# openxrlab/xrnerf

Measured on AMD Instinct MI355X. Metric: training rays/s, Instant-NGP Lego (configs/instant_ngp/nerf_blender_local01.py), synthetic 800x800 rays, higher is better.
Workload: dtype f32

## Files before the change

include/xrnerf_mi355.h:

```cpp
#ifndef XRNERF_MI355_H
#define XRNERF_MI355_H

#include <stddef.h>
#include <stdint.h>

#ifdef __cplusplus
extern "C" {
#endif

#define XR_OK 0
#define XR_EINVAL (-22)
#define XR_ENOMEM (-12)
#define XR_EHIP (-5)

#define XR_NERF_STEPS 1024u
#define XR_NERF_CASCADES 8u
#define XR_NERF_GRIDSIZE 128u
#define XR_GRID_CELLS (128u * 128u * 128u)

enum { XR_ACT_NONE = 0, XR_ACT_RELU = 1, XR_ACT_LOGISTIC = 2, XR_ACT_EXPONENTIAL = 3 };

const char* xr_last_error(void);
int xr_version(void);

void xr_pcg32_host_state(uint64_t seed, uint64_t ncalls, uint64_t* state_host, uint64_t* inc_host);

size_t xr_rays_sampler_workspace_bytes(uint32_t n_rays, uint32_t n_series );
int xr_rays_sampler(const float* rays_o, const float* rays_d, const uint8_t* bitfield, uint32_t n_rays,
                    float aabb0, float aabb1, float near_distance, float cone_angle, uint32_t max_samples,
                    uint64_t rng_state, uint64_t rng_inc, float* coords_out, int32_t* rays_index,
                    int32_t* rays_numsteps, uint32_t* counter2, float* xyz_planes, uint32_t plane_stride,
                    uint32_t rng_chunk, uint32_t rng_ray0, uint32_t flags, void* workspace, size_t workspace_bytes, void* stream);
#define XR_K1_WIDE 1u
int xr_rays_sampler_series(const float* rays_o, const float* rays_d, uint32_t ray_stride, const uint8_t* bitfield, uint32_t n_rays,
                           uint32_t n_series, float aabb0, float aabb1, float near_distance, float cone_angle, uint32_t max_samples,
                           uint64_t rng_state, uint64_t rng_inc, float* coords_out, size_t coords_stride, int32_t* rays_index,
                           int32_t* rays_numsteps, uint32_t* counter2, float* xyz_planes, uint32_t plane_stride, void* workspace,
                           size_t workspace_bytes, void* stream);

int xr_compacted_coord(const float* coords_in, const int32_t* numsteps_in, uint32_t n_rays,
                       uint32_t max_compacted, float* coords_out, int32_t* numsteps_out,
                       uint32_t* rays_counter, uint32_t* numstep_counter, void* workspace,
                       size_t workspace_bytes, void* stream);

int xr_clip_numsteps(const int32_t* numsteps_in, const uint32_t* counter2, uint32_t n_rays, uint32_t n_series, uint32_t ray_stride,
                     uint32_t max_compacted, int32_t* numsteps_out, uint32_t* n_valid_dev, void* stream);

int xr_calc_rgb_forward(const float* network_output , const float* coords ,
                        const int32_t* rays_numsteps, const int32_t* rays_numsteps_compacted,
                        const float* bg_color , uint32_t n_rays, int rgb_activation,
                        int density_activation, float* rgb_output , void* stream);
int xr_calc_rgb_backward(const float* network_output, const int32_t* rays_numsteps_compacted,
                         const float* coords, const float* grad_rgb ,
                         const float* rgb_output ,
                         const float* density_grid_mean , uint32_t n_rays,
                         int rgb_activation, int density_activation, float* dloss_doutput ,
                         void* stream);

int xr_composite_train(const float* network_output, const float* coords, const int32_t* rays_numsteps,
                       const int32_t* rays_numsteps_compacted, const float* bg_color, const float* target,
                       const float* alpha_mask, const float* density_grid_mean, uint32_t n_rays, int rgb_activation,
                       int density_activation, float delta, float scale, float* rgb_output, float* loss_mse_out,
                       float* dloss_doutput, uint32_t* live_seg_count, void* stream);
int xr_train_loss_scalars(const float* rgb, const float* target, const float* alpha_mask, uint32_t n_rays, float delta,
                          float scale, float* loss_mse_out, void* stream);
int xr_calc_rgb_inference(const float* network_output, const float* coords, const int32_t* rays_numsteps,
                          float bg_r, float bg_g, float bg_b, uint32_t n_rays, int rgb_activation,
                          int density_activation, float* rgb_output, float* alpha_output, void* stream);

int xr_render_slice_select(const int32_t* rays_numsteps, const float* T, uint32_t n_rays, uint32_t s0, uint32_t s1,
                           float eps, uint32_t* rows_out, int32_t* ray_offset_out, uint32_t* count_out, void* stream);
int xr_render_slice_composite(const float* raw_slice , const float* coords, const int32_t* rays_numsteps,
                              const int32_t* ray_offset, uint32_t n_rays, uint32_t s0, uint32_t s1, int rgb_activation,
                              int density_activation, float* T, float* rgb_acc, void* stream);

int xr_generate_grid_samples(const float* density_grid, uint32_t ema_step, uint32_t n_elements, uint32_t n_cascades ,
                             float thresh, float aabb0, float aabb1, uint64_t rng_state, uint64_t rng_inc,
                             float* positions, uint32_t pos_row_stride, uint32_t pos_comp_stride, int32_t* indices , void* stream);
int xr_mark_untrained_density_grid(const float* focal_lengths , const float* xforms ,
                                   uint32_t n_elements, uint32_t n_images, int resolution0, int resolution1,
                                   float* density_grid, void* stream);
int xr_splat_grid_samples(const float* mlp_out, const int32_t* indices, uint32_t padded_output_width,
                          uint32_t n_samples, float* density_grid_tmp, void* stream);
int xr_ema_grid_samples(const float* density_grid_tmp, uint32_t n_elements, float decay, float* density_grid,
                        void* stream);
size_t xr_update_bitfield_workspace_bytes(void);
int xr_update_bitfield(const float* density_grid, float* density_grid_mean, uint8_t* bitfield, void* workspace,
                       size_t workspace_bytes, void* stream);
int xr_ema_update_bitfield(const float* density_grid_tmp, uint32_t n_elements, float decay, float* density_grid,
                           float* density_grid_mean, uint8_t* bitfield, void* workspace, size_t workspace_bytes, void* stream);
int xr_bitfield_from_mean(const float* density_grid, const float* density_grid_mean, uint8_t* bitfield,
                          void* stream);

void xr_hashgrid_meta(int n_levels, int log2_hashmap_size, int base_resolution, double per_level_scale,
                      float* scale_host, uint32_t* resolution_host, uint32_t* offset_host );
int xr_hashgrid_fwd(const float* table, const float* x, uint32_t x_stride, uint32_t x_comp_stride, uint32_t n, const uint32_t* n_dev,
                    const uint32_t* rows, int n_levels, const float* scale_host, const uint32_t* resolution_host,
                    const uint32_t* offset_host, float* enc_t, uint32_t ld, void* stream);
size_t xr_hashgrid_bwd_workspace_bytes(uint32_t n, int n_levels, const uint32_t* resolution_host,
                                       const uint32_t* offset_host);
#define XR_SCATTER_OVERWRITE 1
int xr_hashgrid_bwd(const float* x, uint32_t x_stride, const float* denc_t, uint32_t ld, uint32_t n,
                    const uint32_t* n_dev, const uint32_t* rows, int n_levels, const float* scale_host, const uint32_t* resolution_host,
                    const uint32_t* offset_host, float* grad_table, void* workspace, size_t workspace_bytes, int flags,
                    void* stream);
int xr_set_helper_stream(void* stream, void* fork_event, void* join_event);
int xr_sh4(const float* dirs, uint32_t dir_stride, uint32_t n, float* out, void* stream);

#define XR_MLP_F32 0
#define XR_MLP_F16 1
#define XR_MLP_BF16X3 2
#define XR_MLP_F16X2 3
int xr_set_mlp_range_word(uint32_t* word);
int xr_nerf_mlp_fwd(int arithmetic, const float* enc_t, uint32_t ld, const float* dirs, uint32_t dir_stride, uint32_t n,
                    const uint32_t* n_dev, const uint32_t* rows , const float* w_density, const float* w_color, int n_hidden_density, int n_hidden_color,
                    float pad_value, float* raw , void* stream);
size_t xr_nerf_mlp_bwd_workspace_bytes(uint32_t n, int n_hidden_density, int n_hidden_color);
int xr_nerf_mlp_bwd(int arithmetic, const float* enc_t, uint32_t ld, const float* dirs, uint32_t dir_stride, uint32_t n,
                    const uint32_t* n_dev, const float* w_density, const float* w_color, int n_hidden_density, int n_hidden_color,
                    float pad_value, const float* draw , float* denc_t, float* grad_w_density,
                    float* grad_w_color, void* workspace, size_t workspace_bytes, const uint32_t* live_rows,
                    const uint32_t* n_live, void* stream);
#define XR_LIVE_SEGMENT_ROWS 1024u
#define XR_LIVE_ROWS_SEGMENTS(n) (((n) + XR_LIVE_SEGMENT_ROWS - 1u) / XR_LIVE_SEGMENT_ROWS)
int xr_nerf_mlp_bwd_list_slots(void* workspace, size_t workspace_bytes, uint32_t n, uint32_t** live_rows, uint32_t** seg_count,
                               uint32_t** n_live);
int xr_live_rows(const float* dloss_doutput, uint32_t n, const uint32_t* n_dev, uint32_t* seg_count, uint32_t* live_rows,
                 uint32_t* n_live, float* zero_denc_t, uint32_t ld, int seg_counts_ready, void* stream);

typedef struct xr_adam_fuse {
    float* param; float* m; float* v; float* ema;
    int step;
    float lr, beta1, beta2, eps, weight_decay, ema_momentum, grad_scale;
    uint64_t n;
} xr_adam_fuse;
int xr_hashgrid_bwd_adam(const float* x, uint32_t x_stride, const float* denc_t, uint32_t ld, uint32_t n, const uint32_t* n_dev,
                         const uint32_t* rows, int n_levels, const float* scale_host, const uint32_t* resolution_host,
                         const uint32_t* offset_host, void* workspace, size_t workspace_bytes, const xr_adam_fuse* adam,
                         void* stream);

int xr_nerf_density_splat(int mlp_mode, const float* enc_t, uint32_t ld, uint32_t n, const float* w_density, int n_hidden_density,
                          int n_hidden_color, const int32_t* indices, float* density_grid_tmp, void* stream);

int xr_ngp_train_step(const float* table, const float* w_density, const float* w_color, int n_hidden_density, int n_hidden_color,
                      float pad_value, int mlp_mode, int n_levels, const float* scale_host, const uint32_t* resolution_host,
                      const uint32_t* offset_host, const float* coords, uint32_t n_rows, const uint32_t* n_dev,
                      const int32_t* rays_numsteps, const int32_t* rays_numsteps_compacted, uint32_t n_rays, const float* bg_color,
                      const float* target, const float* alpha_mask, const float* density_grid_mean, int rgb_activation,
                      int density_activation, float huber_delta, float loss_scale, float* enc_t, uint32_t ld, float* raw,
                      float* draw, float* denc_t, float* rgb_out, float* zero_block, size_t zero_floats, float* grad_w_density,
                      float* grad_w_color, float* loss_mse, uint32_t* live_seg_count, float* grad_table, size_t table_floats, int zero_draw,
                      void* ws_mlp_bwd, size_t ws_mlp_bwd_bytes, void* ws_scatter, size_t ws_scatter_bytes, int scatter_level0,
                      const float* xyz_planes, uint32_t plane_stride, const xr_adam_fuse* table_adam, const xr_adam_fuse* w_density_adam,
                      const xr_adam_fuse* w_color_adam, const char* timed_entry, void* timing_begin, void* timing_end, void* stream);
void* xr_timing_event_create(void);
int xr_event_record(void* event, void* stream);
int xr_timing_event_destroy(void* event);
int xr_timing_event_elapsed_ms(void* begin, void* end, float* ms);

#define XR_NGP_WINDOW 16
typedef struct xr_ngp_window {
    float *rays_o, *rays_d, *target, *alpha, *bg; int32_t* img_ids;
    int32_t *rays_index, *rays_numsteps, *numsteps_clipped;
    uint32_t ray_stride;
    float* coords; size_t coords_stride;
    float* xyz_planes; uint32_t plane_stride;
    uint32_t *counter2, *n_valid;
} xr_ngp_window;
int xr_ngp_window_march(const xr_ngp_window* window, uint32_t first_chunk, uint32_t n_chunks, uint32_t batches_ready, uint32_t n_rays,
                        const float* rays_rgb_rows, uint64_t n_table_rays, uint64_t* cur_ray, uint64_t batch_seed, uint64_t batch_call_index,
                        const uint8_t* bitfield, float aabb0, float aabb1, float near_distance, float cone_angle, uint32_t max_samples,
                        uint64_t k1_call_index, uint32_t max_compacted, void* workspace, size_t workspace_bytes,
                        uint32_t* counter_host_pinned, void* stream);
int xr_make_batch_series(const float* rays_rgb_rows, const uint64_t* row0_host, uint32_t n, uint32_t n_series, uint32_t ray_stride,
                         uint64_t rng_state, uint64_t rng_inc, float* rays_o, float* rays_d, float* target, float* alpha, float* bg,
                         int32_t* img_ids, void* stream);

typedef struct xr_ngp_step_set {
    float *enc_t, *raw, *draw, *denc_t, *rgb_out, *zero_block; size_t zero_floats;
    float *grad_w_density, *grad_w_color, *loss_mse; uint32_t* live_seg_count;
    float* grad_table;
} xr_ngp_step_set;
typedef struct xr_grad_exchange {
    int (*all_reduce)(void* ctx, float* buf, size_t n, void* stream);
    int (*reduce_scatter)(void* ctx, const float* send, float* recv, size_t n_recv, void* stream);
    int (*all_gather)(void* ctx, const float* send, float* recv, size_t n_send, void* stream);
    int (*finish)(void* ctx, void* stream);
    void* ctx; int world_size, rank;
} xr_grad_exchange;
typedef struct xr_ngp_loop_desc {
    float *table, *w_density, *w_color; int n_hidden_density, n_hidden_color; float pad_value; int mlp_mode;
    int n_levels; const float* scale_host; const uint32_t *resolution_host, *offset_host;
    xr_adam_fuse adam_table, adam_w_density, adam_w_color;
    const float* density_grid_mean; int rgb_activation, density_activation; float huber_delta, loss_scale;
    uint32_t n_rows, ld;
    xr_ngp_window window; xr_ngp_step_set step[2];
    void* ws_mlp_bwd; size_t ws_mlp_bwd_bytes; void* ws_scatter; size_t ws_scatter_bytes;
    void* stream;
    const xr_grad_exchange* exchange; int dp_mode; int split_level;
    float *shard_grad, *table_padded; uint64_t shard_floats;
} xr_ngp_loop_desc;
typedef struct xr_ngp_loop_state {
    uint64_t iter;
    uint32_t step_turn;
    int32_t adam_step;
    uint32_t last_step_set;
} xr_ngp_loop_state;
int xr_ngp_loop_run(const xr_ngp_loop_desc* desc, xr_ngp_loop_state* state, uint32_t k, uint32_t n_rays, const float* lr,
                    const float* ema_momentum, const char* timed_entry, void* const* timing_events, void* const* iter_events);
int xr_rccl_unique_id(const char* librccl_path, void* id128);
void* xr_rccl_create(const char* librccl_path, const void* id128, int world_size, int rank);
int xr_rccl_destroy(void* handle);
int xr_rccl_exchange(void* handle, xr_grad_exchange* out);
int xr_rccl_exposed_ms(void* handle, int timing_on, float* mean_ms , float* max_ms, int* count);

int xr_mlp_fwd(const float* x, long row_stride, long col_stride, int n_in, float pad_value, uint32_t n, const float* w,
               int n_hidden, float* y, void* stream);
size_t xr_mlp_bwd_workspace_bytes(int n_hidden);
int xr_mlp_bwd(const float* x, long row_stride, long col_stride, int n_in, float pad_value, uint32_t n, const float* w,
               int n_hidden, const float* dy, float* dx, float* grad_w, void* workspace, size_t workspace_bytes,
               void* stream);

int xr_gen_rays(const float* pose43_host, int H, int W, float fx, float fy, float cx, float cy, int row0,
                int nrows, float* rays_o, float* rays_d, void* stream);
int xr_huber_loss_grad(const float* rgb, const float* target, const float* alpha, uint32_t n_elems, float delta, float scale,
                       float* grad, float* loss_out, void* stream);
int xr_scale_multi(int n_tensors, float* const* tensors, const size_t* n, const float* scale_dev, float host_factor,
                   void* stream);
int xr_adam_step_multi(int n_tensors, float* const* p_host, const float* const* g_host, float* const* m_host,
                       float* const* v_host, float* const* ema_host, const size_t* n_host, int step, float lr,
                       float beta1, float beta2, float eps, float weight_decay, float ema_momentum, float grad_scale,
                       void* stream);

int xr_mip_zvals(const float* near, const float* far, uint32_t n_rays, uint32_t n_z, int lindisp,
                 const float* z_rand, float* z_out, void* stream);
uint32_t xr_mip_encode_channels(int min_deg, int max_deg, int min_deg_view, int max_deg_view, int append_identity);
int xr_mip_encode(const float* rays_o, const float* rays_d, const float* viewdirs, const float* radii ,
                  const float* z_vals , uint32_t n_rays, uint32_t n_z, int min_deg, int max_deg,
                  int min_deg_view, int max_deg_view, int append_identity, int ray_shape, float* out, uint32_t ld,
                  void* stream);
int xr_mip_encode_gaussians(const float* means, const float* covs, const float* viewdirs, uint32_t n_rays,
                            uint32_t n_samples, int min_deg, int max_deg, int min_deg_view, int max_deg_view,
                            int append_identity, float* out, uint32_t ld, void* stream);
int xr_mip_render_forward(const float* raw, const float* z_vals, const float* rays_d, uint32_t n_rays, uint32_t n_z,
                          float density_bias, float rgb_padding, int white_bkgd, int density_activation, float* rgb,
                          float* distance, float* acc, float* weights, void* stream);
int xr_mip_render_backward(const float* raw, const float* z_vals, const float* rays_d, const float* grad_rgb,
                           uint32_t n_rays, uint32_t n_z, float density_bias, float rgb_padding, int white_bkgd,
                           int density_activation, float* grad_raw, void* stream);
int xr_mip_resample(const float* z_vals, const float* weights , const float* rand,
                    float resample_padding, uint32_t n_rays, uint32_t n_z, float* z_out, void* stream);

uint32_t xr_kilo_param_floats(int pos_freqs, int dir_freqs, int n_hidden);
size_t xr_kilo_workspace_bytes(uint64_t n_samples_total, uint32_t num_networks);
int xr_kilo_mlp_forward(const float* pts, const float* rays_o, const float* rays_d, const float* z_vals,
                        const float* viewdirs, uint32_t n_rays, uint32_t n_samples, const float* gmin_host,
                        const float* gmax_host, const int32_t* fixed_res_host, const int32_t* occ_res_host,
                        const uint8_t* occupancy, const float* domain_mins, const float* domain_maxs, const float* params,
                        uint32_t param_stride, uint32_t num_networks, int pos_freqs, int dir_freqs, int n_hidden,
                        float* raw, uint32_t* counts_out, void* workspace, size_t workspace_bytes, void* stream);
int xr_kilo_mlp_backward(const float* pts, const float* rays_o, const float* rays_d, const float* z_vals,
                         const float* viewdirs, uint32_t n_rays, uint32_t n_samples, const float* gmin_host,
                         const float* gmax_host, const int32_t* fixed_res_host, const int32_t* occ_res_host,
                         const uint8_t* occupancy, const float* domain_mins, const float* domain_maxs, const float* params,
                         uint32_t param_stride, uint32_t num_networks, int pos_freqs, int dir_freqs, int n_hidden,
                         const float* draw, float* grad_params, int reuse_assignment, void* workspace, size_t workspace_bytes, void* stream);
int xr_kilo_pack_params(const float* const* tensors_host, uint32_t num_networks, int pos_freqs, int dir_freqs, int n_hidden, float* blocks,
                        uint32_t param_stride, void* stream);
int xr_kilo_unpack_grads(float* blocks, uint32_t param_stride, uint32_t num_networks, int pos_freqs, int dir_freqs, int n_hidden,
                         float* const* grads_host, int clear_blocks, void* stream);
size_t xr_kilo_render_workspace_bytes(uint32_t n_rays, uint32_t n_samples, uint32_t num_networks);
int xr_kilo_render_rays(const float* rays_o, const float* rays_d, const float* viewdirs, const float* near,
                        const float* far, uint32_t n_rays, uint32_t n_samples, int lindisp, const float* gmin_host,
                        const float* gmax_host, const int32_t* fixed_res_host, const int32_t* occ_res_host,
                        const uint8_t* occupancy, const float* domain_mins, const float* domain_maxs, const float* params,
                        uint32_t param_stride, uint32_t num_networks, int pos_freqs, int dir_freqs, int n_hidden,
                        int white_bkgd, float* rgb, float* disp, float* acc, void* workspace, size_t workspace_bytes,
                        void* stream);
int xr_nerf_render_forward(const float* raw, const float* z_vals, const float* rays_d, uint32_t n_rays,
                           uint32_t n_samples, int white_bkgd, float* rgb, float* disp, float* acc, float* weights,
                           void* stream);

int xr_linear_forward(const float* x, uint32_t ldx, const float* w, const float* bias, uint32_t M, uint32_t N, uint32_t K, int relu,
                      float* y, uint32_t ldy, void* stream);
int xr_linear_backward_input(const float* dy, uint32_t lddy, const float* mask_src, const float* w, int w_transposed, uint32_t M, uint32_t N,
                             uint32_t K, float* dx, void* stream);
int xr_linear_arithmetic(int mode);
uint32_t xr_linear_backward_splits(uint32_t M, uint32_t N, uint32_t K);
int xr_linear_backward_weight(const float* dy, uint32_t lddy, const float* mask_src, const float* x, uint32_t ldx, uint32_t M, uint32_t N,
                              uint32_t K, uint32_t splits, float* dw_partials, float* db_partials, size_t part_stride, void* stream);
int xr_linear_backward_bias(const float* dy, const float* mask_src, uint32_t M, uint32_t N, uint32_t splits,
                            float* db_partials, void* stream);
int xr_sum_partials(const float* partials, uint32_t n_partials, size_t stride, uint32_t n, float* out, void* stream);

int xr_kilo_student_step(const float* examples, uint32_t ex_stride, const float* teacher_raw, const float* domain_mins,
                         const float* domain_maxs, float* params, uint32_t param_stride, uint32_t num_networks, uint32_t batch,
                         int pos_freqs, int dir_freqs, int n_hidden, float alpha_distance, float* loss, float* grad,
                         float* adam_m, float* adam_v, int adam_step, float lr, float beta1, float beta2, float eps, void* stream);
int xr_kilo_student_forward(const float* examples, uint32_t ex_stride, uint32_t n_examples, const float* domain_mins,
                            const float* domain_maxs, const float* params, uint32_t param_stride, uint32_t num_networks,
                            int pos_freqs, int dir_freqs, int n_hidden, int render, float alpha_distance, float* out, void* stream);
int xr_kilo_distill_examples(uint64_t seed, uint64_t iteration, uint64_t pool_size, const float* domain_mins, const float* domain_maxs,
                             uint32_t num_networks, uint32_t batch, uint32_t ex_stride, float* examples, void* stream);
int xr_kilo_occupancy_points(const float* gmin_host, const float* gmax_host, const int32_t* res_host, const int32_t* sub_host,
                             uint64_t voxel_begin, uint32_t n_voxels, float* points, void* stream);
int xr_kilo_occupancy_reduce(const float* raw, uint32_t raw_stride, uint32_t samples_per_voxel, float threshold, uint32_t n_voxels,
                             uint8_t* occupancy, void* stream);

#ifdef __cplusplus
}
#endif
#include "xrnerf_mi355_bungee.h"
#endif
```

xrnerf_amd/_lib.py:

```python
import ctypes as C
import os

HERE = os.path.dirname(os.path.abspath(__file__))
LIB_PATH = os.environ.get('XRNERF_LIB') or os.path.join(HERE, 'libxrnerf_mi355.so')

_vp, _u32, _i32, _f, _u64, _sz, _d = C.c_void_p, C.c_uint32, C.c_int, C.c_float, C.c_uint64, C.c_size_t, C.c_double

class AdamFuse(C.Structure):
    _fields_ = [('param', C.c_void_p), ('m', C.c_void_p), ('v', C.c_void_p), ('ema', C.c_void_p), ('step', C.c_int),
                ('lr', C.c_float), ('beta1', C.c_float), ('beta2', C.c_float), ('eps', C.c_float), ('weight_decay', C.c_float),
                ('ema_momentum', C.c_float), ('grad_scale', C.c_float), ('n', C.c_uint64)]


class Window(C.Structure):
    _fields_ = [(k, C.c_void_p) for k in ('rays_o', 'rays_d', 'target', 'alpha', 'bg', 'img_ids', 'rays_index', 'rays_numsteps',
                                          'numsteps_clipped')] + \
               [('ray_stride', C.c_uint32), ('coords', C.c_void_p), ('coords_stride', C.c_size_t), ('xyz_planes', C.c_void_p),
                ('plane_stride', C.c_uint32), ('counter2', C.c_void_p), ('n_valid', C.c_void_p)]


class StepSet(C.Structure):
    _fields_ = [(k, C.c_void_p) for k in ('enc_t', 'raw', 'draw', 'denc_t', 'rgb_out', 'zero_block')] + [('zero_floats', C.c_size_t)] + \
               [(k, C.c_void_p) for k in ('grad_w_density', 'grad_w_color', 'loss_mse', 'live_seg_count', 'grad_table')]


WINDOW = 16
LIVE_SEGMENT_ROWS = 1024

EX_ALL_REDUCE = C.CFUNCTYPE(C.c_int, C.c_void_p, C.c_void_p, C.c_size_t, C.c_void_p)
EX_SCATTER_GATHER = C.CFUNCTYPE(C.c_int, C.c_void_p, C.c_void_p, C.c_void_p, C.c_size_t, C.c_void_p)
EX_FINISH = C.CFUNCTYPE(C.c_int, C.c_void_p, C.c_void_p)


class GradExchange(C.Structure):
    _fields_ = [('all_reduce', EX_ALL_REDUCE), ('reduce_scatter', EX_SCATTER_GATHER), ('all_gather', EX_SCATTER_GATHER),
                ('finish', EX_FINISH), ('ctx', C.c_void_p), ('world_size', C.c_int), ('rank', C.c_int)]


class LoopDesc(C.Structure):
    _fields_ = [('table', C.c_void_p), ('w_density', C.c_void_p), ('w_color', C.c_void_p), ('n_hidden_density', C.c_int),
                ('n_hidden_color', C.c_int), ('pad_value', C.c_float), ('mlp_mode', C.c_int), ('n_levels', C.c_int),
                ('scale_host', C.c_void_p), ('resolution_host', C.c_void_p), ('offset_host', C.c_void_p),
                ('adam_table', AdamFuse), ('adam_w_density', AdamFuse), ('adam_w_color', AdamFuse),
                ('density_grid_mean', C.c_void_p), ('rgb_activation', C.c_int), ('density_activation', C.c_int),
                ('huber_delta', C.c_float), ('loss_scale', C.c_float), ('n_rows', C.c_uint32), ('ld', C.c_uint32),
                ('window', Window), ('step', StepSet * 2),
                ('ws_mlp_bwd', C.c_void_p), ('ws_mlp_bwd_bytes', C.c_size_t), ('ws_scatter', C.c_void_p), ('ws_scatter_bytes', C.c_size_t),
                ('stream', C.c_void_p),
                ('exchange', C.POINTER(GradExchange)), ('dp_mode', C.c_int), ('split_level', C.c_int),
                ('shard_grad', C.c_void_p), ('table_padded', C.c_void_p), ('shard_floats', C.c_uint64)]


class LoopState(C.Structure):
    _fields_ = [('iter', C.c_uint64), ('step_turn', C.c_uint32), ('adam_step', C.c_int32), ('last_step_set', C.c_uint32)]


SIGNATURES = {
    'xr_last_error': (C.c_char_p, []),
    'xr_version': (_i32, []),
    'xr_event_record': (_i32, [_vp, _vp]),
    'xr_timing_event_create': (_vp, []),
    'xr_timing_event_destroy': (_i32, [_vp]),
    'xr_timing_event_elapsed_ms': (_i32, [_vp, _vp, _vp]),
    'xr_pcg32_host_state': (None, [_u64, _u64, _vp, _vp]),
    'xr_rays_sampler': (_i32, [_vp, _vp, _vp, _u32, _f, _f, _f, _f, _u32, _u64, _u64, _vp, _vp, _vp, _vp, _vp, _u32, _u32, _u32, _u32, _vp, _sz, _vp]),
    'xr_compacted_coord': (_i32, [_vp, _vp, _u32, _u32, _vp, _vp, _vp, _vp, _vp, _sz, _vp]),
    'xr_rays_sampler_workspace_bytes': (_sz, [_u32, _u32]),
    'xr_rays_sampler_series': (_i32, [_vp, _vp, _u32, _vp, _u32, _u32, _f, _f, _f, _f, _u32, _u64, _u64, _vp, _sz, _vp, _vp, _vp, _vp, _u32, _vp,
                                      _sz, _vp]),
    'xr_clip_numsteps': (_i32, [_vp, _vp, _u32, _u32, _u32, _u32, _vp, _vp, _vp]),
    'xr_make_batch_series': (_i32, [_vp, _vp, _u32, _u32, _u32, _u64, _u64, _vp, _vp, _vp, _vp, _vp, _vp, _vp]),
    'xr_ngp_window_march': (_i32, [_vp, _u32, _u32, _u32, _u32, _vp, _u64, _vp, _u64, _u64, _vp, _f, _f, _f, _f, _u32, _u64, _u32, _vp, _sz,
                                   _vp, _vp]),
    'xr_render_slice_select': (_i32, [_vp, _vp, _u32, _u32, _u32, _f, _vp, _vp, _vp, _vp]),
    'xr_render_slice_composite': (_i32, [_vp, _vp, _vp, _vp, _u32, _u32, _u32, _i32, _i32, _vp, _vp, _vp]),
    'xr_calc_rgb_forward': (_i32, [_vp, _vp, _vp, _vp, _vp, _u32, _i32, _i32, _vp, _vp]),
    'xr_calc_rgb_backward': (_i32, [_vp, _vp, _vp, _vp, _vp, _vp, _u32, _i32, _i32, _vp, _vp]),
    'xr_hashgrid_bwd_adam': (_i32, [_vp, _u32, _vp, _u32, _u32, _vp, _vp, _i32, _vp, _vp, _vp, _vp, _sz, _vp, _vp]),
    'xr_train_loss_scalars': (_i32, [_vp, _vp, _vp, _u32, _f, _f, _vp, _vp]),
    'xr_composite_train': (_i32, [_vp, _vp, _vp, _vp, _vp, _vp, _vp, _vp, _u32, _i32, _i32, _f, _f, _vp, _vp, _vp, _vp, _vp]),
    'xr_calc_rgb_inference': (_i32, [_vp, _vp, _vp, _f, _f, _f, _u32, _i32, _i32, _vp, _vp, _vp]),
    'xr_generate_grid_samples': (_i32, [_vp, _u32, _u32, _u32, _f, _f, _f, _u64, _u64, _vp, _u32, _u32, _vp, _vp]),
    'xr_mark_untrained_density_grid': (_i32, [_vp, _vp, _u32, _u32, _i32, _i32, _vp, _vp]),
    'xr_splat_grid_samples': (_i32, [_vp, _vp, _u32, _u32, _vp, _vp]),
    'xr_ema_grid_samples': (_i32, [_vp, _u32, _f, _vp, _vp]),
    'xr_update_bitfield_workspace_bytes': (_sz, []),
    'xr_update_bitfield': (_i32, [_vp, _vp, _vp, _vp, _sz, _vp]),
    'xr_ema_update_bitfield': (_i32, [_vp, _u32, _f, _vp, _vp, _vp, _vp, _sz, _vp]),
    'xr_bitfield_from_mean': (_i32, [_vp, _vp, _vp, _vp]),
    'xr_hashgrid_meta': (None, [_i32, _i32, _i32, _d, _vp, _vp, _vp]),
    'xr_hashgrid_fwd': (_i32, [_vp, _vp, _u32, _u32, _u32, _vp, _vp, _i32, _vp, _vp, _vp, _vp, _u32, _vp]),
    'xr_hashgrid_bwd_workspace_bytes': (_sz, [_u32, _i32, _vp, _vp]),
    'xr_hashgrid_bwd': (_i32, [_vp, _u32, _vp, _u32, _u32, _vp, _vp, _i32, _vp, _vp, _vp, _vp, _vp, _sz, _i32, _vp]),
    'xr_set_helper_stream': (_i32, [_vp, _vp, _vp]),
    'xr_set_mlp_range_word': (_i32, [_vp]),
    'xr_sh4': (_i32, [_vp, _u32, _u32, _vp, _vp]),
    'xr_nerf_mlp_fwd': (_i32, [_i32, _vp, _u32, _vp, _u32, _u32, _vp, _vp, _vp, _vp, _i32, _i32, _f, _vp, _vp]),
    'xr_nerf_mlp_bwd_workspace_bytes': (_sz, [_u32, _i32, _i32]),
    'xr_ngp_train_step': (_i32, [_vp, _vp, _vp, _i32, _i32, _f, _i32, _i32, _vp, _vp, _vp, _vp, _u32, _vp, _vp, _vp, _u32, _vp, _vp, _vp,
                                 _vp, _i32, _i32, _f, _f, _vp, _u32, _vp, _vp, _vp, _vp, _vp, _sz, _vp, _vp, _vp, _vp, _vp, _sz, _i32, _vp, _sz,
                                 _vp, _sz, _i32, _vp, _u32, _vp, _vp, _vp, C.c_char_p, _vp, _vp, _vp]),
    'xr_ngp_loop_run': (_i32, [_vp, _vp, _u32, _u32, _vp, _vp, C.c_char_p, _vp, _vp]),
    'xr_rccl_unique_id': (_i32, [C.c_char_p, _vp]),
    'xr_rccl_create': (_vp, [C.c_char_p, _vp, _i32, _i32]),
    'xr_rccl_destroy': (_i32, [_vp]),
    'xr_rccl_exchange': (_i32, [_vp, _vp]),
    'xr_rccl_exposed_ms': (_i32, [_vp, _i32, _vp, _vp, _vp]),
    'xr_nerf_mlp_bwd': (_i32, [_i32, _vp, _u32, _vp, _u32, _u32, _vp, _vp, _vp, _i32, _i32, _f, _vp, _vp, _vp, _vp, _vp, _sz, _vp, _vp, _vp]),
    'xr_live_rows': (_i32, [_vp, _u32, _vp, _vp, _vp, _vp, _vp, _u32, _i32, _vp]),
    'xr_nerf_mlp_bwd_list_slots': (_i32, [_vp, _sz, _u32, _vp, _vp, _vp]),
    'xr_mlp_fwd': (_i32, [_vp, C.c_long, C.c_long, _i32, _f, _u32, _vp, _i32, _vp, _vp]),
    'xr_mlp_bwd_workspace_bytes': (_sz, [_i32]),
    'xr_mlp_bwd': (_i32, [_vp, C.c_long, C.c_long, _i32, _f, _u32, _vp, _i32, _vp, _vp, _vp, _vp, _sz, _vp]),
    'xr_gen_rays': (_i32, [_vp, _i32, _i32, _f, _f, _f, _f, _i32, _i32, _vp, _vp, _vp]),
    'xr_huber_loss_grad': (_i32, [_vp, _vp, _vp, _u32, _f, _f, _vp, _vp, _vp]),
    'xr_adam_step_multi': (_i32, [_i32, _vp, _vp, _vp, _vp, _vp, _vp, _i32, _f, _f, _f, _f, _f, _f, _f, _vp]),
    'xr_scale_multi': (_i32, [_i32, _vp, _vp, _vp, _f, _vp]),
    'xr_mip_zvals': (_i32, [_vp, _vp, _u32, _u32, _i32, _vp, _vp, _vp]),
    'xr_mip_encode_channels': (_u32, [_i32, _i32, _i32, _i32, _i32]),
    'xr_mip_encode': (_i32, [_vp, _vp, _vp, _vp, _vp, _u32, _u32, _i32, _i32, _i32, _i32, _i32, _i32, _vp, _u32, _vp]),
    'xr_mip_encode_gaussians': (_i32, [_vp, _vp, _vp, _u32, _u32, _i32, _i32, _i32, _i32, _i32, _vp, _u32, _vp]),
    'xr_mip_render_forward': (_i32, [_vp, _vp, _vp, _u32, _u32, _f, _f, _i32, _i32, _vp, _vp, _vp, _vp, _vp]),
    'xr_mip_render_backward': (_i32, [_vp, _vp, _vp, _vp, _u32, _u32, _f, _f, _i32, _i32, _vp, _vp]),
    'xr_mip_resample': (_i32, [_vp, _vp, _vp, _f, _u32, _u32, _vp, _vp]),
    'xr_kilo_param_floats': (_u32, [_i32, _i32, _i32]),
    'xr_kilo_workspace_bytes': (_sz, [_u64, _u32]),
    'xr_kilo_mlp_forward': (_i32, [_vp, _vp, _vp, _vp, _vp, _u32, _u32, _vp, _vp, _vp, _vp, _vp, _vp, _vp, _vp, _u32, _u32,
                                   _i32, _i32, _i32, _vp, _vp, _vp, _sz, _vp]),
    'xr_kilo_mlp_backward': (_i32, [_vp, _vp, _vp, _vp, _vp, _u32, _u32, _vp, _vp, _vp, _vp, _vp, _vp, _vp, _vp, _u32, _u32,
                                    _i32, _i32, _i32, _vp, _vp, _i32, _vp, _sz, _vp]),
    'xr_kilo_pack_params': (_i32, [_vp, _u32, _i32, _i32, _i32, _vp, _u32, _vp]),
    'xr_kilo_unpack_grads': (_i32, [_vp, _u32, _u32, _i32, _i32, _i32, _vp, _i32, _vp]),
    'xr_nerf_render_forward': (_i32, [_vp, _vp, _vp, _u32, _u32, _i32, _vp, _vp, _vp, _vp, _vp]),
    'xr_nerf_density_splat': (_i32, [_i32, _vp, _u32, _u32, _vp, _i32, _i32, _vp, _vp, _vp]),
    'xr_linear_forward': (_i32, [_vp, _u32, _vp, _vp, _u32, _u32, _u32, _i32, _vp, _u32, _vp]),
    'xr_linear_backward_input': (_i32, [_vp, _u32, _vp, _vp, _i32, _u32, _u32, _u32, _vp, _vp]),
    'xr_linear_backward_splits': (_u32, [_u32, _u32, _u32]),
    'xr_linear_arithmetic': (_i32, [_i32]),
    'xr_linear_backward_bias': (_i32, [_vp, _vp, _u32, _u32, _u32, _vp, _vp]),
    'xr_sum_partials': (_i32, [_vp, _u32, _sz, _u32, _vp, _vp]),
    'xr_linear_backward_weight': (_i32, [_vp, _u32, _vp, _vp, _u32, _u32, _u32, _u32, _u32, _vp, _vp, _sz, _vp]),
    'xr_kilo_render_workspace_bytes': (_sz, [_u32, _u32, _u32]),
    'xr_kilo_render_rays': (_i32, [_vp, _vp, _vp, _vp, _vp, _u32, _u32, _i32, _vp, _vp, _vp, _vp, _vp, _vp, _vp, _vp, _u32,
                                   _u32, _i32, _i32, _i32, _i32, _vp, _vp, _vp, _vp, _sz, _vp]),
    'xr_kilo_student_step': (_i32, [_vp, _u32, _vp, _vp, _vp, _vp, _u32, _u32, _u32, _i32, _i32, _i32, _f, _vp, _vp, _vp, _vp, _i32, _f, _f,
                                    _f, _f, _vp]),
    'xr_kilo_student_forward': (_i32, [_vp, _u32, _u32, _vp, _vp, _vp, _u32, _u32, _i32, _i32, _i32, _i32, _f, _vp, _vp]),
    'xr_kilo_distill_examples': (_i32, [_u64, _u64, _u64, _vp, _vp, _u32, _u32, _u32, _vp, _vp]),
    'xr_kilo_occupancy_points': (_i32, [_vp, _vp, _vp, _vp, _u64, _u32, _vp, _vp]),
    'xr_kilo_occupancy_reduce': (_i32, [_vp, _u32, _u32, _f, _u32, _vp, _vp]),
}

BUNGEE_SIGNATURES = {
    'xr_bungee_zvals': (_i32, [_vp, _vp, _vp, _vp, _u32, _u32, _i32, _vp, _f, _f, _f, _vp, _vp]),
    'xr_bungee_encode': (_i32, [_vp, _vp, _vp, _vp, _vp, _vp, _vp, _u32, _u32, _i32, _i32, _i32, _vp, _u32, _vp, _u32, _vp]),
    'xr_bungee_render_forward': (_i32, [_vp, _vp, _vp, _vp, _u32, _u32, _u32, _i32, _f, _f, _i32, _i32, _vp, _vp, _vp, _vp, _vp]),
    'xr_bungee_render_backward': (_i32, [_vp, _vp, _vp, _vp, _vp, _u32, _u32, _u32, _i32, _f, _f, _i32, _i32, _vp, _vp]),
}

VANILLA_SIGNATURES = {
    'xr_nerf_encode': (_i32, [_vp, _vp, _u64, _u32, _i32, _i32, _vp, _u32, _vp]),
    'xr_nerf_render_train_forward': (_i32, [_vp, _vp, _vp, _vp, _u32, _u32, _i32, _vp, _vp, _vp, _vp, _vp]),
    'xr_nerf_render_backward': (_i32, [_vp, _vp, _vp, _vp, _u32, _u32, _i32, _vp, _vp, _vp]),
    'xr_nerf_sample_pdf': (_i32, [_vp, _vp, _vp, _vp, _vp, _u32, _u32, _u32, _vp, _vp, _vp, _vp]),
}

ANINERF_SIGNATURES = {
    'xr_ani_closest': (_i32, [_vp, _vp, _vp, _vp, _u32, _u32, _f, _vp, _vp, _vp, _vp, _vp, _vp]),
    'xr_ani_select_workspace_bytes': (_sz, [_u32]),
    'xr_ani_select': (_i32, [_vp, _vp, _u32, _vp, _vp, _vp, _sz, _vp]),
    'xr_ani_blend_forward': (_i32, [_vp, _vp, _vp, _u32, _vp, _vp]),
    'xr_ani_blend_backward': (_i32, [_vp, _vp, _u32, _vp, _vp]),
    'xr_ani_skin_forward': (_i32, [_vp, _vp, _vp, _vp, _vp, _u32, _vp, _vp, _vp]),
    'xr_ani_skin_backward': (_i32, [_vp, _vp, _vp, _vp, _vp, _u32, _vp, _vp, _vp, _vp]),
    'xr_ani_encode_backward': (_i32, [_vp, _vp, _u32, _u32, _i32, _vp, _vp]),
}

NEURALBODY_SIGNATURES = {
    'xr_nb_layout': (_i32, [_u32, _i32, _i32, _i32, _vp]),
    'xr_nb_build_rows_workspace_bytes': (_sz, [_i32, _i32, _i32]),
    'xr_nb_build_rows': (_i32, [_vp, _u32, _i32, _i32, _i32, _vp, _vp, _vp, _vp, _vp, _sz, _vp]),
    'xr_nb_subm_table': (_i32, [_vp, _vp, _u32, _i32, _i32, _i32, _vp, _vp]),
    'xr_nb_down_tables': (_i32, [_vp, _vp, _u32, _vp, _vp, _u32, _i32, _i32, _i32, _vp, _vp, _vp]),
    'xr_nb_conv': (_i32, [_vp, _vp, _vp, _u32, _i32, _i32, _i32, _i32, _vp, _vp]),
    'xr_nb_conv_weight_grad_workspace_bytes': (_sz, [_u32, _i32, _i32]),
    'xr_nb_conv_weight_grad': (_i32, [_vp, _vp, _vp, _u32, _i32, _i32, _vp, _vp, _sz, _vp]),
    'xr_nb_sample_forward': (_i32, [_vp, _vp, _vp, _vp, _f, _i32, _i32, _i32, _vp, _vp, _u32, _vp, _u32, _vp]),
    'xr_nb_sample_backward_workspace_bytes': (_sz, [_vp]),
    'xr_nb_sample_backward': (_i32, [_vp, _vp, _vp, _vp, _f, _i32, _i32, _i32, _vp, _vp, _vp, _u32, _u32, _vp, _vp, _sz, _vp]),
}

_lib = None


class XrError(RuntimeError):
    pass


def load():
    global _lib
    if _lib is not None:
        return _lib
    from . import build as _build

    def is_stale():
        if not os.environ.get('XRNERF_LIB') and os.path.exists(LIB_PATH) and os.path.isdir(_build.CSRC):
            i = _build.info()
            return i.get('stamp') == 'missing' or not i.get('binary_is_the_stamped_build') or i.get('sources_match_the_stamped_build') is False
        return False

    stale = is_stale()
    if not os.path.exists(LIB_PATH) or stale:
        import fcntl
        import warnings

        def rebuild():
            try:
                _build.build(force=stale)
            except Exception as e:
                if not os.path.exists(LIB_PATH):
                    raise XrError('libxrnerf_mi355.so is missing and could not be built: %s. '
                                  'Run `python -m xrnerf_amd.build` (needs hipcc).' % e)
                warnings.warn('libxrnerf_mi355.so is not the stamped build of the sources beside it and could not be rebuilt (%s): '
                              'loading it as it is' % e)
        try:
            lock = open(LIB_PATH + '.lock', 'w')
        except OSError:
            lock = None
        if lock is None:
            rebuild()
        else:
            with lock:
                fcntl.flock(lock, fcntl.LOCK_EX)
                try:
                    stale = is_stale()
                    if not os.path.exists(LIB_PATH) or stale:
                        rebuild()
                finally:
                    fcntl.flock(lock, fcntl.LOCK_UN)
    lib = C.CDLL(LIB_PATH)
    for name, (res, args) in list(SIGNATURES.items()) + list(BUNGEE_SIGNATURES.items()) + list(VANILLA_SIGNATURES.items()) + \
            list(ANINERF_SIGNATURES.items()) + list(NEURALBODY_SIGNATURES.items()):
        fn = getattr(lib, name)
        fn.restype = res
        fn.argtypes = args
    _lib = lib
    return lib


def check(rc, what=''):
    if rc != 0:
        raise XrError('%s failed (%d): %s' % (what, rc, load().xr_last_error().decode()))
```

xrnerf_amd/csrc/xr_common.h:

```cpp
#pragma once
#include <hip/hip_runtime.h>
#include <cstdint>
#include <cstdio>
#include <cstring>
#include "../../include/xrnerf_mi355.h"
#ifndef XR_LDS_PTR
#define XR_LDS_PTR(T, p) ((T __attribute__((address_space(3)))*)(p))
#endif
extern "C" __attribute__((visibility("hidden"))) int xr_device_cus(void);

#define XR_WAVE 64

void xr_set_error(const char* fmt, ...);

#define XR_REQUIRE(cond, msg)                                   \
    do {                                                        \
        if (!(cond)) { xr_set_error("%s: %s", __func__, msg); return XR_EINVAL; } \
    } while (0)

#define XR_LAUNCH_CHECK()                                                            \
    do {                                                                             \
        hipError_t e_ = hipGetLastError();                                           \
        if (e_ != hipSuccess) { xr_set_error("%s: %s", __func__, hipGetErrorString(e_)); return XR_EHIP; } \
    } while (0)

#define XR_HIP(call)                                                                 \
    do {                                                                             \
        hipError_t e_ = (call);                                                      \
        if (e_ != hipSuccess) { xr_set_error("%s: %s", __func__, hipGetErrorString(e_)); return XR_EHIP; } \
    } while (0)

static inline uint32_t xr_div_up(uint64_t a, uint32_t b) { return (uint32_t)((a + b - 1) / b); }

#define XR_SQRT3 1.73205080757f
__host__ __device__ inline float xr_min_step() { return XR_SQRT3 / 1024.0f; }
__host__ __device__ inline float xr_max_step() { return XR_SQRT3 / 1024.0f * 128.0f * 1024.0f / 128.0f; }
__host__ __device__ inline float xr_max_warp_step() { return XR_SQRT3 / 1024.0f * 128.0f; }

struct xr_pcg32 {
    uint64_t state, inc;
    __host__ __device__ uint32_t next_uint() {
        uint64_t old = state;
        state = old * 0x5851f42d4c957f2dULL + inc;
        uint32_t xs = (uint32_t)(((old >> 18u) ^ old) >> 27u);
        uint32_t rot = (uint32_t)(old >> 59u);
        return (xs >> rot) | (xs << ((~rot + 1u) & 31));
    }
    __host__ __device__ float next_float() {
        uint32_t u = (next_uint() >> 9) | 0x3f800000u;
        float f;
#if defined(__HIP_DEVICE_COMPILE__)
        f = __uint_as_float(u);
#else
        memcpy(&f, &u, 4);
#endif
        return f - 1.0f;
    }
    __host__ __device__ void advance(uint64_t delta) {
        uint64_t cur_mult = 0x5851f42d4c957f2dULL, cur_plus = inc, acc_mult = 1u, acc_plus = 0u;
        while (delta > 0) {
            if (delta & 1) { acc_mult *= cur_mult; acc_plus = acc_plus * cur_mult + cur_plus; }
            cur_plus = (cur_mult + 1) * cur_plus;
            cur_mult *= cur_mult;
            delta >>= 1;
        }
        state = acc_mult * state + acc_plus;
    }
    __host__ __device__ void seed(uint64_t initstate, uint64_t initseq) {
        state = 0u; inc = (initseq << 1u) | 1u;
        next_uint(); state += initstate; next_uint();
    }
};

__host__ __device__ inline uint32_t xr_expand_bits(uint32_t v) {
    v = (v * 0x00010001u) & 0xFF0000FFu; v = (v * 0x00000101u) & 0x0F00F00Fu;
    v = (v * 0x00000011u) & 0xC30C30C3u; v = (v * 0x00000005u) & 0x49249249u;
    return v;
}
__host__ __device__ inline uint32_t xr_morton3d(uint32_t x, uint32_t y, uint32_t z) {
    return xr_expand_bits(x) | (xr_expand_bits(y) << 1) | (xr_expand_bits(z) << 2);
}
__host__ __device__ inline uint32_t xr_morton3d_invert(uint32_t x) {
    x = x & 0x49249249; x = (x | (x >> 2)) & 0xc30c30c3; x = (x | (x >> 4)) & 0x0f00f00f;
    x = (x | (x >> 8)) & 0xff0000ff; x = (x | (x >> 16)) & 0x0000ffff;
    return x;
}

__device__ inline float xr_clampf(float v, float lo, float hi) { return v < lo ? lo : (hi < v ? hi : v); }
__device__ inline float xr_logistic(float x) { return 1.0f / (1.0f + __expf(-x)); }
__device__ inline float xr_act_rgb(float v, int a) {
    switch (a) { case 0: return v; case 1: return v > 0.f ? v : 0.f; case 2: return xr_logistic(v);
                 default: return __expf(xr_clampf(v, -10.f, 10.f)); }
}
__device__ inline float xr_act_density(float v, int a) {
    switch (a) { case 0: return v; case 1: return v > 0.f ? v : 0.f; case 2: return xr_logistic(v);
                 default: return __expf(v); }
}
__device__ inline float xr_dact_rgb(float v, int a) {
    switch (a) { case 0: return 1.f; case 1: return v > 0.f ? 1.f : 0.f;
                 case 2: { float s = xr_logistic(v); return s * (1.f - s); }
                 default: return __expf(xr_clampf(v, -10.f, 10.f)); }
}
__device__ inline float xr_dact_density(float v, int a) {
    switch (a) { case 0: return 1.f; case 1: return v > 0.f ? 1.f : 0.f;
                 case 2: { float s = xr_logistic(v); return s * (1.f - s); }
                 default: return __expf(xr_clampf(v, -15.f, 15.f)); }
}
__host__ __device__ inline float xr_unwarp_dt(float dt) {
    return dt * (xr_max_warp_step() - xr_min_step()) + xr_min_step();
}

#define XR_LIVE_SEG 1024u

struct XrHelper { hipStream_t stream; hipEvent_t fork, join; };
const XrHelper* xr_internal_helper();
int xr_internal_hashgrid_bwd_adam_supported(uint32_t n, int n_levels, const float* scale_host, const uint32_t* resolution_host,
                                            const uint32_t* offset_host);
void xr_internal_defer_mlp_reduce(bool on);
int xr_internal_mlp_bwd_reduce(const void* workspace, uint32_t n, int n_hidden_density, int n_hidden_color, float* grad_w_density, float* grad_w_color, int overwrite, void* stream);
```

xrnerf_amd/csrc/xr_misc.hip:

```cpp
#include "xr_common.h"
#include "xr_adam.h"
#include <cstdlib>
#include <cstdarg>

static thread_local char g_err[512] = "";
void xr_set_error(const char* fmt, ...) {
    va_list ap; va_start(ap, fmt);
    vsnprintf(g_err, sizeof(g_err), fmt, ap);
    va_end(ap);
}
extern "C" const char* xr_last_error(void) { return g_err; }
extern "C" int xr_version(void) { return 123; }

extern "C" void xr_pcg32_host_state(uint64_t seed, uint64_t ncalls, uint64_t* state_host, uint64_t* inc_host) {
    xr_pcg32 r; r.seed(seed, 1u);
    r.advance(ncalls << 32);
    *state_host = r.state; *inc_host = r.inc;
}

struct Pose43 { float m[12]; };
__global__ __launch_bounds__(256) void k_gen_rays(Pose43 p, int W, float fx, float fy, float cx, float cy, int row0,
                                                   uint32_t n, float* __restrict__ rays_o, float* __restrict__ rays_d) {
    const uint32_t q = blockIdx.x * 256 + threadIdx.x;
    if (q >= n) return;
    const int r = q / W, c = q % W;
    const float i = (float)c + 0.5f, j = (float)(row0 + r) + 0.5f;
    const float dx = (i - cx) / fx, dy = (j - cy) / fy;
    float v[3];
#pragma unroll
    for (int k = 0; k < 3; ++k) {
        float a = __fmul_rn(p.m[k], dx);
        a = __fadd_rn(a, __fmul_rn(p.m[3 + k], dy));
        v[k] = __fadd_rn(a, p.m[6 + k]);
    }
    const float nrm = __fsqrt_rn(__fadd_rn(__fadd_rn(__fmul_rn(v[0], v[0]), __fmul_rn(v[1], v[1])), __fmul_rn(v[2], v[2])));
#pragma unroll
    for (int k = 0; k < 3; ++k) { rays_d[3 * (size_t)q + k] = v[k] / nrm; rays_o[3 * (size_t)q + k] = p.m[9 + k]; }
}
extern "C" int xr_gen_rays(const float* pose43_host, int H, int W, float fx, float fy, float cx, float cy, int row0,
                           int nrows, float* rays_o, float* rays_d, void* stream_) {
    XR_REQUIRE(pose43_host && rays_o && rays_d, "null pointer");
    XR_REQUIRE(H > 0 && W > 0 && row0 >= 0 && nrows > 0 && row0 + nrows <= H, "bad image window");
    Pose43 p; memcpy(p.m, pose43_host, sizeof(p.m));
    const uint32_t n = (uint32_t)nrows * (uint32_t)W;
    hipLaunchKernelGGL(k_gen_rays, dim3(xr_div_up(n, 256)), dim3(256), 0, (hipStream_t)stream_, p, W, fx, fy, cx, cy, row0, n,
                       rays_o, rays_d);
    XR_LAUNCH_CHECK();
    return XR_OK;
}

__global__ __launch_bounds__(256) void k_huber(const float* __restrict__ rgb, const float* __restrict__ target,
                                                const float* __restrict__ alpha, uint32_t n, float delta, float scale,
                                                float* __restrict__ grad, float* __restrict__ loss) {
    __shared__ float ws[4], ws2[4];
    float acc = 0.f, mse = 0.f;
    for (uint32_t i = blockIdx.x * 256 + threadIdx.x; i < n; i += gridDim.x * 256) {
        const float r = rgb[i] - target[i], a = fabsf(r);
        if (a > delta) { acc += a - 0.5f * delta; grad[i] = scale * (r > 0.f ? 1.f : -1.f); }
        else { acc += 0.5f / delta * a * a; grad[i] = scale * (r / delta); }
        if (alpha) { const float m = r * alpha[i / 3]; mse += m * m; }
    }
#pragma unroll
    for (int d = 32; d > 0; d >>= 1) { acc += __shfl_xor(acc, d, 64); mse += __shfl_xor(mse, d, 64); }
    if ((threadIdx.x & 63) == 0) { ws[threadIdx.x >> 6] = acc; ws2[threadIdx.x >> 6] = mse; }
    __syncthreads();
    if (threadIdx.x == 0) {
        atomicAdd(loss, scale * ((ws[0] + ws[1]) + (ws[2] + ws[3])));
        if (alpha) atomicAdd(loss + 1, (ws2[0] + ws2[1]) + (ws2[2] + ws2[3]));
    }
}
extern "C" int xr_huber_loss_grad(const float* rgb, const float* target, const float* alpha, uint32_t n_elems, float delta, float scale,
                                  float* grad, float* loss_out, void* stream_) {
    XR_REQUIRE(rgb && target && grad && loss_out && n_elems > 0, "bad argument");
    XR_REQUIRE(!alpha || n_elems % 3 == 0, "the masked error takes rgb triples");
    hipLaunchKernelGGL(k_huber, dim3(min(xr_div_up(n_elems, 256), 1024u)), dim3(256), 0, (hipStream_t)stream_, rgb, target, alpha, n_elems,
                       delta, scale, grad, loss_out);
    XR_LAUNCH_CHECK();
    return XR_OK;
}

struct XrBatchRows { uint64_t row0[XR_NGP_WINDOW]; };
__global__ __launch_bounds__(256) void k_make_batch(const float* __restrict__ rows, uint32_t n, xr_pcg32 rng,
                                                     float* __restrict__ rays_o, float* __restrict__ rays_d,
                                                     float* __restrict__ target, float* __restrict__ alpha,
                                                     float* __restrict__ bg, int32_t* __restrict__ img_ids, XrBatchRows at, uint32_t ray_stride) {
    const uint32_t i = blockIdx.x * 256 + threadIdx.x;
    if (i >= n) return;
    const float* r = rows + 11 * ((size_t)at.row0[blockIdx.y] + i);
    rng.advance(((uint64_t)blockIdx.y << 32) + 3ull * i);
    const size_t q = (size_t)blockIdx.y * ray_stride + i;
    const float a = r[9];
#pragma unroll
    for (int k = 0; k < 3; ++k) {
        rays_o[3 * q + k] = r[k];
        rays_d[3 * q + k] = r[3 + k];
        const float b = rng.next_float();
        bg[3 * q + k] = b;
        target[3 * q + k] = r[6 + k] * a + b * (1.f - a);
    }
    alpha[q] = a;
    img_ids[q] = (int32_t)r[10];
}
extern "C" int xr_make_batch_series(const float* rays_rgb_rows, const uint64_t* row0_host, uint32_t n, uint32_t n_series, uint32_t ray_stride,
                                    uint64_t rng_state, uint64_t rng_inc, float* rays_o, float* rays_d, float* target, float* alpha, float* bg,
                                    int32_t* img_ids, void* stream_) {
    XR_REQUIRE(rays_rgb_rows && row0_host && rays_o && rays_d && target && alpha && bg && img_ids && n > 0, "bad argument");
    XR_REQUIRE(n_series >= 1 && n_series <= (uint32_t)XR_NGP_WINDOW && ray_stride >= n, "bad series");
    xr_pcg32 rng{rng_state, rng_inc};
    XrBatchRows at = {};
    for (uint32_t c = 0; c < n_series; ++c) at.row0[c] = row0_host[c];
    hipLaunchKernelGGL(k_make_batch, dim3(xr_div_up(n, 256), n_series), dim3(256), 0, (hipStream_t)stream_, rays_rgb_rows, n, rng, rays_o,
                       rays_d, target, alpha, bg, img_ids, at, ray_stride);
    XR_LAUNCH_CHECK();
    return XR_OK;
}

struct AdamTensors { float* p[4]; const float* g[4]; float* m[4]; float* v[4]; float* ema[4]; unsigned long long n[4]; unsigned first_block[5]; };
typedef float am_f4 __attribute__((ext_vector_type(4)));
template <bool NT> __device__ __forceinline__ float4 am_ld(const float* p, size_t i) {
    if (NT) { const am_f4 r = __builtin_nontemporal_load(reinterpret_cast<const am_f4*>(p) + i); return make_float4(r.x, r.y, r.z, r.w); }
    return reinterpret_cast<const float4*>(p)[i];
}
template <bool NT> __device__ __forceinline__ void am_st(float* p, size_t i, const float4 v) {
    if (NT) { am_f4 r; r.x = v.x; r.y = v.y; r.z = v.z; r.w = v.w; __builtin_nontemporal_store(r, reinterpret_cast<am_f4*>(p) + i); }
    else reinterpret_cast<float4*>(p)[i] = v;
}
template <bool NT>
__global__ __launch_bounds__(256) void k_adam_multi(AdamTensors t, int nt, float b1, float b2, float step_size, float bc2s,
                                                     float eps, float wd, float mom, float gs) {
    int k = 0;
#pragma unroll
    for (int j = 1; j < 4; ++j) if (j < nt && blockIdx.x >= t.first_block[j]) k = j;
    const unsigned nblk = t.first_block[k + 1] - t.first_block[k], blk = blockIdx.x - t.first_block[k];
    float* __restrict__ p = t.p[k]; const float* __restrict__ g = t.g[k];
    float* __restrict__ m = t.m[k]; float* __restrict__ v = t.v[k]; float* __restrict__ ema = t.ema[k];
    const size_t n = t.n[k], n4 = n / 4;
    for (size_t i = blk * 256ull + threadIdx.x; i < n4; i += (size_t)nblk * 256) {
        float4 pp = ((float4*)p)[i], mm = am_ld<NT>(m, i), vv = am_ld<NT>(v, i);
        const float4 gg = am_ld<NT>(g, i);
        adam1(pp.x, gg.x, mm.x, vv.x, b1, b2, step_size, bc2s, eps, wd, gs);
        adam1(pp.y, gg.y, mm.y, vv.y, b1, b2, step_size, bc2s, eps, wd, gs);
        adam1(pp.z, gg.z, mm.z, vv.z, b1, b2, step_size, bc2s, eps, wd, gs);
        adam1(pp.w, gg.w, mm.w, vv.w, b1, b2, step_size, bc2s, eps, wd, gs);
        ((float4*)p)[i] = pp; am_st<NT>(m, i, mm); am_st<NT>(v, i, vv);
        if (ema) {
            float4 e = am_ld<NT>(ema, i);
            e.x = (1.f - mom) * e.x + mom * pp.x; e.y = (1.f - mom) * e.y + mom * pp.y;
            e.z = (1.f - mom) * e.z + mom * pp.z; e.w = (1.f - mom) * e.w + mom * pp.w;
            am_st<NT>(ema, i, e);
        }
    }
    if (blk == 0 && threadIdx.x < (n & 3)) {
        const size_t i = n4 * 4 + threadIdx.x;
        float pp = p[i], mm = m[i], vv = v[i];
        adam1(pp, g[i], mm, vv, b1, b2, step_size, bc2s, eps, wd, gs);
        p[i] = pp; m[i] = mm; v[i] = vv;
        if (ema) ema[i] = (1.f - mom) * ema[i] + mom * pp;
    }
}
extern "C" int xr_adam_step_multi(int n_tensors, float* const* p, const float* const* g, float* const* m, float* const* v,
                                  float* const* ema, const size_t* n, int step, float lr, float beta1, float beta2, float eps,
                                  float weight_decay, float ema_momentum, float grad_scale, void* stream_) {
    XR_REQUIRE(n_tensors >= 1 && n_tensors <= 4 && p && g && m && v && n && step >= 1, "bad argument");
    AdamTensors t; memset(&t, 0, sizeof(t));
    unsigned blocks = 0;
    for (int k = 0; k < n_tensors; ++k) {
        XR_REQUIRE(p[k] && g[k] && m[k] && v[k] && n[k] > 0, "null tensor");
        XR_REQUIRE((((uintptr_t)p[k] | (uintptr_t)g[k] | (uintptr_t)m[k] | (uintptr_t)v[k] | (uintptr_t)(ema ? ema[k] : nullptr)) & 15) == 0,
                   "buffers must be 16-byte aligned");
        t.p[k] = p[k]; t.g[k] = g[k]; t.m[k] = m[k]; t.v[k] = v[k]; t.ema[k] = ema ? ema[k] : nullptr; t.n[k] = n[k];
        t.first_block[k] = blocks;
        blocks += min(xr_div_up(n[k] / 4 + 1, 256), 2048u);
    }
    for (int k = n_tensors; k <= 4; ++k) t.first_block[k] = blocks;
    const float bc1 = 1.f - powf(beta1, (float)step), bc2 = 1.f - powf(beta2, (float)step);
#ifndef XR_ADAM_NT
#define XR_ADAM_NT 1
#endif
    hipLaunchKernelGGL(k_adam_multi<XR_ADAM_NT != 0>, dim3(blocks), dim3(256), 0, (hipStream_t)stream_, t, n_tensors, beta1, beta2, lr / bc1,
                       sqrtf(bc2), eps, weight_decay, ema_momentum, grad_scale);
    XR_LAUNCH_CHECK();
    return XR_OK;
}

struct ScaleTensors { float* p[4]; unsigned long long n[4]; };
__global__ __launch_bounds__(256) void k_scale_multi(ScaleTensors t, int nt, const float* __restrict__ scale_dev, float host_factor) {
    const float f = (scale_dev ? *scale_dev : 1.f) * host_factor;
    if (f == 1.f) return;
    for (int k = 0; k < nt; ++k) {
        float* __restrict__ p = t.p[k];
        const size_t n = t.n[k], n4 = n / 4;
        for (size_t i = blockIdx.x * 256ull + threadIdx.x; i < n4; i += (size_t)gridDim.x * 256) {
            float4 v = ((float4*)p)[i];
            v.x *= f; v.y *= f; v.z *= f; v.w *= f;
            ((float4*)p)[i] = v;
        }
        if (blockIdx.x == 0 && threadIdx.x < (n & 3)) p[n4 * 4 + threadIdx.x] *= f;
    }
}
extern "C" int xr_scale_multi(int n_tensors, float* const* p, const size_t* n, const float* scale_dev, float host_factor, void* stream_) {
    XR_REQUIRE(n_tensors >= 1 && n_tensors <= 4 && p && n, "bad argument");
    ScaleTensors t; memset(&t, 0, sizeof(t));
    for (int k = 0; k < n_tensors; ++k) {
        XR_REQUIRE(p[k] && ((uintptr_t)p[k] & 15) == 0, "tensors must be 16-byte aligned");
        t.p[k] = p[k]; t.n[k] = n[k];
    }
    hipLaunchKernelGGL(k_scale_multi, dim3(2048), dim3(256), 0, (hipStream_t)stream_, t, n_tensors, scale_dev, host_factor);
    XR_LAUNCH_CHECK();
    return XR_OK;
}
```

xrnerf_amd/csrc/xr_raymarch.hip:

```cpp
#include "xr_common.h"
#include "xr_aux.h"
#include <cfloat>
#include <cstdlib>

#define RM_BLOCK 256
#ifndef K1W_MAX_RAYS
#define K1W_MAX_RAYS 32768
#endif
#define K1_TL 128

__device__ inline uint32_t block_excl_scan(uint32_t v, uint32_t* total, uint32_t* lds4) {
    const int lane = threadIdx.x & 63, wid = threadIdx.x >> 6;
    uint32_t inc = v;
#pragma unroll
    for (int d = 1; d < 64; d <<= 1) {
        uint32_t o = __shfl_up(inc, d, 64);
        if (lane >= d) inc += o;
    }
    if (lane == 63) lds4[wid] = inc;
    __syncthreads();
    uint32_t woff = 0, tot = 0;
#pragma unroll
    for (int w = 0; w < RM_BLOCK / 64; ++w) {
        uint32_t t = lds4[w];
// ... 162 lines not shown
            }
        }
        if (done) break;
        const float tl = __shfl(t, K1W - 1, K1W);
        t0 = tl + rm_calc_dt(tl, cone);
    }
    if (li == 0) { cnt[ray] = j; start_t[ray] = startt; }
}
__global__ __launch_bounds__(RM_BLOCK) void k1_block_scan(uint32_t n_rays, const uint32_t* __restrict__ cnt, uint32_t* __restrict__ local_off,
                                                          uint32_t* __restrict__ block_tot) {
    __shared__ uint32_t lds4[4];
    const uint32_t i = blockIdx.x * RM_BLOCK + threadIdx.x;
    uint32_t tot;
    const uint32_t off = block_excl_scan(i < n_rays ? cnt[i] : 0u, &tot, lds4);
    if (i < n_rays) local_off[i] = off;
    if (threadIdx.x == 0) block_tot[blockIdx.x] = tot;
}

__global__ __launch_bounds__(1024) void k_scan_blocks(uint32_t nb, const uint32_t* __restrict__ block_tot,
                                                      uint32_t limit, uint32_t* __restrict__ block_base,
                                                      uint32_t* __restrict__ info) {
    __shared__ uint32_t wsum[16];
    __shared__ uint32_t s_running, s_cross;
    const int lane = threadIdx.x & 63, wid = threadIdx.x >> 6;
    if (threadIdx.x == 0) { s_running = 0; s_cross = nb; }
    __syncthreads();
    for (uint32_t c0 = 0; c0 < nb; c0 += 1024) {
        uint32_t b = c0 + threadIdx.x;
        uint32_t v = b < nb ? block_tot[b] : 0, inc = v;
#pragma unroll
        for (int d = 1; d < 64; d <<= 1) { uint32_t o = __shfl_up(inc, d, 64); if (lane >= d) inc += o; }
        if (lane == 63) wsum[wid] = inc;
        __syncthreads();
        uint32_t woff = 0, ctot = 0;
        for (int w = 0; w < 16; ++w) { uint32_t t = wsum[w]; if (w < wid) woff += t; ctot += t; }
        uint32_t base = s_running + woff + inc - v;
        if (b < nb) {
            block_base[b] = base;
            if ((uint64_t)base + v > (uint64_t)limit) atomicMin(&s_cross, b);
        }
        __syncthreads();
        if (threadIdx.x == 0) s_running += ctot;
        __syncthreads();
    }
    if (threadIdx.x == 0) { info[0] = s_running; info[1] = s_cross; }
}

__global__ __launch_bounds__(RM_BLOCK) void k1_write(
    uint32_t n_rays, float lo, float hi, const float* __restrict__ rays_o, const float* __restrict__ rays_d,
    const uint8_t* __restrict__ bitfield, float cone, uint32_t max_samples, const uint32_t* __restrict__ cnt,
    const uint32_t* __restrict__ local_off, const float* __restrict__ start_t,
    const uint32_t* __restrict__ block_base, const uint32_t* __restrict__ info, const uint32_t* __restrict__ block_tot,
    float* __restrict__ coords_out,
    int32_t* __restrict__ rays_index, int32_t* __restrict__ numsteps_out, uint32_t* __restrict__ counter2,
    const float* __restrict__ tlist, float* __restrict__ xyz_planes, uint32_t plane_stride, uint32_t ray_stride, size_t coords_stride) {
    __shared__ uint32_t lds4[4];
    const uint32_t b = blockIdx.x, i = b * RM_BLOCK + threadIdx.x;
    const uint32_t nb = gridDim.x;
    {
        const size_t c = blockIdx.y;
        rays_o += 3 * c * ray_stride; rays_d += 3 * c * ray_stride;
        rays_index += c * ray_stride; numsteps_out += 2 * c * ray_stride; counter2 += 2 * c;
        coords_out += 7 * c * coords_stride;
        if (xyz_planes) xyz_planes += 3 * c * (size_t)plane_stride;
        if (block_tot) block_tot += c * nb;
        cnt += c * nb * RM_BLOCK; local_off += c * nb * RM_BLOCK; start_t += c * nb * RM_BLOCK; tlist += c * nb * RM_BLOCK * (size_t)K1_TL;
    }
    uint32_t cross, bbase, grand;
    if (block_tot) {
        __shared__ uint32_t s_cross, s_bbase;
        if (threadIdx.x == 0) s_cross = nb;
        const uint32_t v = threadIdx.x < nb ? block_tot[threadIdx.x] : 0u;
        const uint32_t ex = block_excl_scan(v, &grand, lds4);
        if (threadIdx.x < nb && (uint64_t)ex + v > (uint64_t)max_samples) atomicMin(&s_cross, threadIdx.x);
        if (threadIdx.x == b) s_bbase = ex;
        __syncthreads();
        cross = s_cross; bbase = s_bbase;
    } else { cross = info[1]; bbase = block_base[b]; grand = info[0]; }
    uint32_t n = 0, base = 0; bool in = i < n_rays;
    if (in) { n = cnt[i]; base = bbase + local_off[i]; }
    bool valid = in && !((uint64_t)base + n > (uint64_t)max_samples);
    uint32_t vtot;
    uint32_t voff = block_excl_scan(valid ? 1u : 0u, &vtot, lds4);
    uint32_t valid_before = (b <= cross) ? b * RM_BLOCK : 0u;
    if (in) {
        if (!valid) {
            numsteps_out[2 * i] = 0; numsteps_out[2 * i + 1] = (int32_t)base; rays_index[i] = 0;
        } else {
            numsteps_out[2 * i] = (int32_t)n; numsteps_out[2 * i + 1] = (int32_t)base;
            rays_index[i] = n == 0 ? -1 : (int32_t)(valid_before + voff);
        }
    }
    if (threadIdx.x == 0) {
        if (b == 0) counter2[1] = grand;
        if (b == cross || (cross == nb && b == nb - 1)) counter2[0] = valid_before + vtot;
    }
    __shared__ uint32_t s_off[RM_BLOCK], s_n[RM_BLOCK];
    __shared__ float s_ray[RM_BLOCK][6];
    s_off[threadIdx.x] = in ? local_off[i] : 0xffffffffu;
    s_n[threadIdx.x] = valid ? n : 0u;
    if (in) {
#pragma unroll
        for (int k = 0; k < 3; ++k) { s_ray[threadIdx.x][k] = rays_o[3 * i + k]; s_ray[threadIdx.x][3 + k] = rays_d[3 * i + k]; }
    }
    __syncthreads();
    const uint32_t last = min((uint32_t)RM_BLOCK, n_rays - b * RM_BLOCK) - 1;
    const uint32_t btot = s_off[last] + cnt[b * RM_BLOCK + last];
    const float diag = hi - lo;
    for (uint32_t e = threadIdx.x; e < btot; e += RM_BLOCK) {
        uint32_t lo_r = 0, hi_r = last;
        while (lo_r < hi_r) {
            const uint32_t mid = (lo_r + hi_r + 1) >> 1;
            if (s_off[mid] <= e) lo_r = mid; else hi_r = mid - 1;
        }
        const uint32_t j = e - s_off[lo_r];
        if (j >= s_n[lo_r] || j >= K1_TL) continue;
        const float t = tlist[((size_t)b * RM_BLOCK + lo_r) * K1_TL + j];
        const float ox = s_ray[lo_r][0], oy = s_ray[lo_r][1], oz = s_ray[lo_r][2];
        const float dx = s_ray[lo_r][3], dy = s_ray[lo_r][4], dz = s_ray[lo_r][5];
        const float px = ox + t * dx, py = oy + t * dy, pz = oz + t * dz;
        const float dt = rm_calc_dt(t, cone);
        float* c = coords_out + 7 * ((size_t)bbase + e);
        c[0] = (px - lo) / diag; c[1] = (py - lo) / diag; c[2] = (pz - lo) / diag;
        c[3] = (dt - xr_min_step()) / (xr_max_warp_step() - xr_min_step());
        c[4] = (dx + 1.0f) * 0.5f; c[5] = (dy + 1.0f) * 0.5f; c[6] = (dz + 1.0f) * 0.5f;
        if (xyz_planes) {
            const size_t q = (size_t)bbase + e;
            xyz_planes[q] = c[0]; xyz_planes[plane_stride + q] = c[1]; xyz_planes[2 * (size_t)plane_stride + q] = c[2];
        }
    }
    if (!valid || n <= K1_TL) return;
    Ray r = rm_load_ray(rays_o, rays_d, i);
    const float wdx = (r.dx + 1.0f) * 0.5f, wdy = (r.dy + 1.0f) * 0.5f, wdz = (r.dz + 1.0f) * 0.5f;
    float t = tlist[(size_t)i * K1_TL + (K1_TL - 1)];
    t += rm_calc_dt(t, cone);
    uint32_t j = K1_TL;
    float* __restrict__ out = coords_out + 7 * (size_t)base;
    for (;;) {
        float px = r.ox + t * r.dx, py = r.oy + t * r.dy, pz = r.oz + t * r.dz;
        if (!(rm_contains(lo, hi, px, py, pz) && j < n)) break;
        float dt = rm_calc_dt(t, cone);
        int mip = rm_mip_from_dt(dt, px, py, pz);
        if (rm_occupied(px, py, pz, bitfield, mip)) {
            float* c = out + 7 * (size_t)j;
            c[0] = (px - lo) / diag; c[1] = (py - lo) / diag; c[2] = (pz - lo) / diag;
            c[3] = (dt - xr_min_step()) / (xr_max_warp_step() - xr_min_step());
            c[4] = wdx; c[5] = wdy; c[6] = wdz;
            if (xyz_planes) {
                const size_t q = (size_t)base + j;
                xyz_planes[q] = c[0]; xyz_planes[plane_stride + q] = c[1]; xyz_planes[2 * (size_t)plane_stride + q] = c[2];
            }
            ++j; t += dt;
        } else t = rm_advance(t, cone, px, py, pz, r, XR_NERF_GRIDSIZE >> mip);
    }
}

struct RmWorkspace { uint32_t *cnt, *local_off, *block_tot, *block_base, *info; float *start_t, *tlist; };
static size_t rm_ws_layout(uint32_t n_rays, char* base, RmWorkspace* w, uint32_t n_series = 1) {
    const size_t nb = (size_t)xr_div_up(n_rays, RM_BLOCK) * n_series;
    const size_t slots = n_series > 1 ? nb * RM_BLOCK : (size_t)n_rays;
    size_t off = 0;
    auto take = [&](size_t bytes) { size_t o = off; off += (bytes + 255) / 256 * 256; return base ? base + o : (char*)nullptr; };
    char* p0 = take(4ull * slots); char* p1 = take(4ull * slots); char* p2 = take(4ull * slots);
    char* p3 = take(4 * nb); char* p4 = take(4 * nb); char* p5 = take(16);
    char* p6 = take(4ull * slots * K1_TL);
    if (w) { w->tlist = (float*)p6; w->cnt = (uint32_t*)p0; w->local_off = (uint32_t*)p1; w->start_t = (float*)p2;
             w->block_tot = (uint32_t*)p3; w->block_base = (uint32_t*)p4; w->info = (uint32_t*)p5; }
    return off;
}

extern "C" size_t xr_rays_sampler_workspace_bytes(uint32_t n_rays, uint32_t n_series) {
    return rm_ws_layout(n_rays, nullptr, nullptr, n_series ? n_series : 1);
}

static int rm_launch(const float* rays_o, const float* rays_d, const uint8_t* bitfield, uint32_t n_rays, uint32_t n_series, uint32_t ray_stride,
                     float aabb0, float aabb1, float near_distance, float cone_angle, uint32_t max_samples, xr_pcg32 rng,
                     float* coords_out, size_t coords_stride, int32_t* rays_index, int32_t* rays_numsteps, uint32_t* counter2, float* xyz_planes,
                     uint32_t plane_stride, uint32_t rng_chunk, uint32_t rng_ray0, uint32_t flags, void* workspace, hipStream_t stream) {
    RmWorkspace w; rm_ws_layout(n_rays, (char*)workspace, &w, n_series);
    const uint32_t nb = xr_div_up(n_rays, RM_BLOCK);
#ifndef K1W_ALWAYS
#define K1W_ALWAYS 0
#endif
    if (n_series == 1 && ((flags & XR_K1_WIDE) != 0u || K1W_ALWAYS != 0) && (uint32_t)K1W_MAX_RAYS != 0u && n_rays <= (uint32_t)K1W_MAX_RAYS) {
        hipLaunchKernelGGL(k1_count_w, dim3(xr_div_up(n_rays * K1W, RM_BLOCK)), dim3(RM_BLOCK), 0, stream, n_rays, aabb0, aabb1, rays_o, rays_d,
                           bitfield, cone_angle, near_distance, rng, rng_chunk, rng_ray0, w.cnt, w.start_t, w.tlist);
        hipLaunchKernelGGL(k1_block_scan, dim3(nb), dim3(RM_BLOCK), 0, stream, n_rays, (const uint32_t*)w.cnt, w.local_off, w.block_tot);
    } else
        hipLaunchKernelGGL(k1_count, dim3(nb, n_series), dim3(RM_BLOCK), 0, stream, n_rays, aabb0, aabb1, rays_o, rays_d, bitfield,
                           cone_angle, near_distance, rng, rng_chunk, rng_ray0, w.cnt, w.local_off, w.start_t, w.block_tot, w.tlist, ray_stride);
#ifndef K1_INLINE_SCAN
#define K1_INLINE_SCAN 1
#endif
    const bool inline_scan = (K1_INLINE_SCAN || n_series > 1) && nb <= (uint32_t)RM_BLOCK;
    if (!inline_scan) hipLaunchKernelGGL(k_scan_blocks, dim3(1), dim3(1024), 0, stream, nb, w.block_tot, max_samples, w.block_base, w.info);
    hipLaunchKernelGGL(k1_write, dim3(nb, n_series), dim3(RM_BLOCK), 0, stream, n_rays, aabb0, aabb1, rays_o, rays_d, bitfield,
                       cone_angle, max_samples, w.cnt, w.local_off, w.start_t, w.block_base, w.info,
                       inline_scan ? (const uint32_t*)w.block_tot : (const uint32_t*)nullptr, coords_out,
                       rays_index, rays_numsteps, counter2, w.tlist, xyz_planes, plane_stride, ray_stride, coords_stride);
    XR_LAUNCH_CHECK();
    return XR_OK;
}

extern "C" int xr_rays_sampler(const float* rays_o, const float* rays_d, const uint8_t* bitfield, uint32_t n_rays,
                                float aabb0, float aabb1, float near_distance, float cone_angle, uint32_t max_samples,
                                uint64_t rng_state, uint64_t rng_inc, float* coords_out, int32_t* rays_index,
                                int32_t* rays_numsteps, uint32_t* counter2, float* xyz_planes, uint32_t plane_stride,
                                uint32_t rng_chunk, uint32_t rng_ray0, uint32_t flags, void* workspace, size_t workspace_bytes, void* stream_) {
    XR_REQUIRE((flags & ~XR_K1_WIDE) == 0, "unknown flag");
    XR_REQUIRE(rays_o && rays_d && bitfield && coords_out && rays_index && rays_numsteps && counter2, "null pointer");
    XR_REQUIRE(!xyz_planes || plane_stride >= max_samples, "a position plane holds max_samples values");
    XR_REQUIRE(n_rays > 0 && n_rays <= (1u << 28), "n_rays out of range");
    XR_REQUIRE(workspace && workspace_bytes >= xr_rays_sampler_workspace_bytes(n_rays, 1), "workspace too small");
    return rm_launch(rays_o, rays_d, bitfield, n_rays, 1, 0, aabb0, aabb1, near_distance, cone_angle, max_samples, xr_pcg32{rng_state, rng_inc},
                     coords_out, 0, rays_index, rays_numsteps, counter2, xyz_planes, plane_stride, rng_chunk, rng_ray0, flags, workspace,
                     (hipStream_t)stream_);
}

extern "C" int xr_rays_sampler_series(const float* rays_o, const float* rays_d, uint32_t ray_stride, const uint8_t* bitfield, uint32_t n_rays,
                                      uint32_t n_series, float aabb0, float aabb1, float near_distance, float cone_angle, uint32_t max_samples,
                                      uint64_t rng_state, uint64_t rng_inc, float* coords_out, size_t coords_stride, int32_t* rays_index,
                                      int32_t* rays_numsteps, uint32_t* counter2, float* xyz_planes, uint32_t plane_stride, void* workspace,
                                      size_t workspace_bytes, void* stream_) {
    XR_REQUIRE(rays_o && rays_d && bitfield && coords_out && rays_index && rays_numsteps && counter2, "null pointer");
    XR_REQUIRE(n_series >= 1 && n_series <= 65535u && n_rays > 0 && n_rays <= (1u << 28) && ray_stride >= n_rays, "bad series");
    XR_REQUIRE(coords_stride >= max_samples && (!xyz_planes || plane_stride >= max_samples), "a launch's buffers hold max_samples rows");
    XR_REQUIRE(workspace && workspace_bytes >= xr_rays_sampler_workspace_bytes(n_rays, n_series), "workspace too small");
    const uint32_t nb = xr_div_up(n_rays, RM_BLOCK);
    if (nb <= (uint32_t)RM_BLOCK || n_series == 1)
        return rm_launch(rays_o, rays_d, bitfield, n_rays, n_series, ray_stride, aabb0, aabb1, near_distance, cone_angle, max_samples,
                         xr_pcg32{rng_state, rng_inc}, coords_out, coords_stride, rays_index, rays_numsteps, counter2, xyz_planes, plane_stride,
                         0, 0, 0, workspace, (hipStream_t)stream_);
    xr_pcg32 rng{rng_state, rng_inc};
    for (uint32_t c = 0; c < n_series; ++c) {
        int rc = rm_launch(rays_o + 3 * (size_t)c * ray_stride, rays_d + 3 * (size_t)c * ray_stride, bitfield, n_rays, 1, 0, aabb0, aabb1, near_distance,
                           cone_angle, max_samples, rng, coords_out + 7 * c * coords_stride, 0, rays_index + (size_t)c * ray_stride,
                           rays_numsteps + 2 * (size_t)c * ray_stride, counter2 + 2 * c, xyz_planes ? xyz_planes + 3 * (size_t)c * plane_stride : nullptr,
                           plane_stride, 0, 0, 0, workspace, (hipStream_t)stream_);
        if (rc != XR_OK) return rc;
        rng.advance(1ull << 32);
    }
    return XR_OK;
}

__global__ __launch_bounds__(RM_BLOCK) void k2_count(uint32_t n_rays, const int32_t* __restrict__ numsteps_in,
                                                      uint32_t* __restrict__ local_off, uint32_t* __restrict__ block_tot) {
    __shared__ uint32_t lds4[4];
    const uint32_t i = blockIdx.x * RM_BLOCK + threadIdx.x;
    uint32_t n = i < n_rays ? (uint32_t)numsteps_in[2 * i] : 0u, tot;
    uint32_t off = block_excl_scan(n, &tot, lds4);
    if (i < n_rays) local_off[i] = off;
    if (threadIdx.x == 0) block_tot[blockIdx.x] = tot;
}
__global__ __launch_bounds__(RM_BLOCK) void k2_copy(uint32_t n_rays, uint32_t max_compacted,
                                                     const float* __restrict__ coords_in, const int32_t* __restrict__ numsteps_in,
                                                     const uint32_t* __restrict__ local_off, const uint32_t* __restrict__ block_base,
                                                     const uint32_t* __restrict__ info, float* __restrict__ coords_out,
                                                     int32_t* __restrict__ numsteps_out, uint32_t* __restrict__ rays_counter,
                                                     uint32_t* __restrict__ numstep_counter) {
    const uint32_t i = blockIdx.x * RM_BLOCK + threadIdx.x;
    const int lane = threadIdx.x & 63;
    uint32_t n = 0, base = 0, cbase = 0, nc = 0;
    if (i < n_rays) {
        n = (uint32_t)numsteps_in[2 * i]; base = (uint32_t)numsteps_in[2 * i + 1];
        cbase = block_base[blockIdx.x] + local_off[i];
        nc = min(max_compacted - min(max_compacted, cbase), n);
        numsteps_out[2 * i] = (int32_t)nc; numsteps_out[2 * i + 1] = (int32_t)cbase;
    }
    unsigned long long m = __ballot(nc > 0);
    if (lane == 0 && m) atomicAdd(rays_counter, (uint32_t)__popcll(m));
    if (i == 0) *numstep_counter = info[0];
    for (int s = 0; s < 64; ++s) {
        uint32_t rn = __shfl(nc, s, 64);
        if (rn == 0) continue;
        uint32_t rb = __shfl(base, s, 64), rc = __shfl(cbase, s, 64);
        const float* __restrict__ src = coords_in + 7 * (size_t)rb;
        float* __restrict__ dst = coords_out + 7 * (size_t)rc;
        for (uint32_t e = lane; e < 7 * rn; e += 64) dst[e] = src[e];
    }
}

extern "C" int xr_compacted_coord(const float* coords_in, const int32_t* numsteps_in, uint32_t n_rays,
                                  uint32_t max_compacted, float* coords_out, int32_t* numsteps_out,
                                  uint32_t* rays_counter, uint32_t* numstep_counter, void* workspace,
                                  size_t workspace_bytes, void* stream_) {
    hipStream_t stream = (hipStream_t)stream_;
    XR_REQUIRE(coords_in && numsteps_in && coords_out && numsteps_out && rays_counter && numstep_counter, "null pointer");
    XR_REQUIRE(n_rays > 0, "n_rays == 0");
    XR_REQUIRE(workspace && workspace_bytes >= xr_rays_sampler_workspace_bytes(n_rays, 1), "workspace too small");
    RmWorkspace w; rm_ws_layout(n_rays, (char*)workspace, &w);
    const uint32_t nb = xr_div_up(n_rays, RM_BLOCK);
    XR_HIP(hipMemsetAsync(rays_counter, 0, 4, stream));
    hipLaunchKernelGGL(k2_count, dim3(nb), dim3(RM_BLOCK), 0, stream, n_rays, numsteps_in, w.local_off, w.block_tot);
    hipLaunchKernelGGL(k_scan_blocks, dim3(1), dim3(1024), 0, stream, nb, w.block_tot, 0xffffffffu, w.block_base, w.info);
    hipLaunchKernelGGL(k2_copy, dim3(nb), dim3(RM_BLOCK), 0, stream, n_rays, max_compacted, coords_in, numsteps_in,
                       w.local_off, w.block_base, w.info, coords_out, numsteps_out, rays_counter, numstep_counter);
    XR_LAUNCH_CHECK();
    return XR_OK;
}

__global__ __launch_bounds__(RM_BLOCK) void k2_clip(uint32_t n_rays, uint32_t max_compacted, const int32_t* __restrict__ in,
                                                     const uint32_t* __restrict__ counter2, int32_t* __restrict__ out,
                                                     uint32_t* __restrict__ n_valid, uint32_t chunk_rows, uint32_t n_chunks,
                                                     uint32_t ray_stride) {
    const uint32_t i = blockIdx.x * RM_BLOCK + threadIdx.x;
    in += 2 * (size_t)blockIdx.y * ray_stride; out += 2 * (size_t)blockIdx.y * ray_stride;
    counter2 += 2 * blockIdx.y; n_valid += (size_t)(1 + n_chunks) * blockIdx.y;
    if (i == 0) {
        const uint32_t total = min(counter2[1], max_compacted);
        n_valid[0] = total;
        for (uint32_t c = 0; c < n_chunks; ++c)
            n_valid[1 + c] = min(chunk_rows, total - min(total, c * chunk_rows));
    }
    if (i >= n_rays) return;
    const uint32_t n = (uint32_t)in[2 * i], base = (uint32_t)in[2 * i + 1];
    out[2 * i] = (int32_t)min(max_compacted - min(max_compacted, base), n);
    out[2 * i + 1] = (int32_t)base;
}
extern "C" int xr_clip_numsteps(const int32_t* numsteps_in, const uint32_t* counter2, uint32_t n_rays, uint32_t n_series, uint32_t ray_stride,
                                       uint32_t max_compacted, int32_t* numsteps_out, uint32_t* n_valid_dev, void* stream_) {
    XR_REQUIRE(numsteps_in && counter2 && numsteps_out && n_valid_dev && n_rays > 0 && n_series >= 1 && n_series <= 65535u && ray_stride >= n_rays, "bad argument");
    hipLaunchKernelGGL(k2_clip, dim3(xr_div_up(n_rays, RM_BLOCK), n_series), dim3(RM_BLOCK), 0, (hipStream_t)stream_, n_rays, max_compacted,
                       numsteps_in, counter2, numsteps_out, n_valid_dev, max_compacted, 1u, ray_stride);
    XR_LAUNCH_CHECK();
    return XR_OK;
}

#define CG 16
#define CG_RC 4
__device__ inline void cg_chunk(uint32_t n, uint32_t sub, uint32_t* k0, uint32_t* k1) {
    const uint32_t chunk = (n + CG - 1) / CG;
    *k0 = min(n, sub * chunk); *k1 = min(n, (sub + 1) * chunk);
}
__device__ inline void cg_stitch(uint32_t sub, float T_loc, float cr, float cg, float cb, float* Tb, float* Cbr, float* Cbg,
                                 float* Cbb, float* Ttot, float* Cr, float* Cg, float* Cb) {
    float tb = 1.f, ar = 0.f, ag = 0.f, ab = 0.f, tt = 1.f, tr = 0.f, tg = 0.f, tbb = 0.f;
#pragma unroll
    for (int m = 0; m < CG; ++m) {
        const float tm = __shfl(T_loc, m, CG), rm = __shfl(cr, m, CG), gm = __shfl(cg, m, CG), bm = __shfl(cb, m, CG);
        if ((uint32_t)m == sub) { tb = tt; ar = tr; ag = tg; ab = tbb; }
        tr += tt * rm; tg += tt * gm; tbb += tt * bm;
        tt *= tm;
    }
    *Tb = tb; *Cbr = ar; *Cbg = ag; *Cbb = ab; *Ttot = tt; *Cr = tr; *Cg = tg; *Cb = tbb;
}

#define CG_LB 8
template <class F>
__device__ __forceinline__ void cg_long(const float4* __restrict__ raw, const float* __restrict__ coords, uint32_t base, uint32_t k0,
                                        uint32_t k1, F&& f) {
    for (uint32_t b = k0; b < k1; b += CG_LB) {
        float4 o[CG_LB]; float d[CG_LB];
        const uint32_t mm = min((uint32_t)CG_LB, k1 - b);
#pragma unroll
        for (uint32_t u = 0; u < CG_LB; ++u)
            if (u < mm) { o[u] = raw[base + b + u]; d[u] = coords[7 * (size_t)(base + b + u) + 3]; }
#pragma unroll
        for (uint32_t u = 0; u < CG_LB; ++u) if (u < mm) f(o[u], d[u], b + u);
    }
}

template <bool INFERENCE>
__global__ __launch_bounds__(RM_BLOCK) void k_composite_fwd(
    uint32_t n_rays, const float4* __restrict__ raw, const float* __restrict__ coords,
    const int32_t* __restrict__ numsteps, const int32_t* __restrict__ numsteps_c, const float* __restrict__ bg,
    float bg_r, float bg_g, float bg_b, int rgb_act, int density_act, float* __restrict__ rgb_out,
    float* __restrict__ alpha_out) {
    const uint32_t t = blockIdx.x * RM_BLOCK + threadIdx.x;
    const uint32_t i = t / CG, sub = t % CG;
    const bool in = i < n_rays;
    uint32_t n = 0, base = 0;
    if (in) { n = (uint32_t)numsteps_c[2 * i]; base = (uint32_t)numsteps_c[2 * i + 1]; }
    uint32_t k0, k1;
    cg_chunk(n, sub, &k0, &k1);
    float T = 1.f, cr = 0.f, cg = 0.f, cb = 0.f;
    const uint32_t m = k1 - k0;
    float4 oc[CG_RC]; float dc[CG_RC];
    if (m <= CG_RC) {
#pragma unroll
        for (uint32_t u = 0; u < CG_RC; ++u)
            if (u < m) { oc[u] = raw[base + k0 + u]; dc[u] = coords[7 * (size_t)(base + k0 + u) + 3]; }
    }
    auto step = [&](const float4 o, float dtw) {
        const float dt = xr_unwarp_dt(dtw);
        const float density = xr_act_density(o.w, density_act);
        const float alpha = 1.f - __expf(-density * dt);
        const float w = alpha * T;
        cr += w * xr_act_rgb(o.x, rgb_act); cg += w * xr_act_rgb(o.y, rgb_act); cb += w * xr_act_rgb(o.z, rgb_act);
        T *= (1.f - alpha);
    };
    if (m <= CG_RC) {
#pragma unroll
        for (uint32_t u = 0; u < CG_RC; ++u) if (u < m) step(oc[u], dc[u]);
    } else {
        cg_long(raw, coords, base, k0, k1, [&](const float4 o, float dtw, uint32_t) { step(o, dtw); });
    }
    float Tb, ar, ag, ab, Tt, Cr, Cg, Cb;
    cg_stitch(sub, T, cr, cg, cb, &Tb, &ar, &ag, &ab, &Tt, &Cr, &Cg, &Cb);
    if (!in || sub != 0) return;
    float br, bgc, bb;
    if (INFERENCE) { br = bg_r; bgc = bg_g; bb = bg_b; }
    else { br = bg[3 * i]; bgc = bg[3 * i + 1]; bb = bg[3 * i + 2]; }
    if (n == 0) {
        rgb_out[3 * i] = br; rgb_out[3 * i + 1] = bgc; rgb_out[3 * i + 2] = bb;
        if (INFERENCE) alpha_out[i] = 0.f;
        return;
    }
    const bool add_bg = INFERENCE ? true : (n == (uint32_t)numsteps[2 * i]);
    if (add_bg) { Cr += Tt * br; Cg += Tt * bgc; Cb += Tt * bb; }
    rgb_out[3 * i] = Cr; rgb_out[3 * i + 1] = Cg; rgb_out[3 * i + 2] = Cb;
    if (INFERENCE) alpha_out[i] = 1.f - Tt;
}

extern "C" int xr_calc_rgb_forward(const float* network_output, const float* coords, const int32_t* rays_numsteps,
                                   const int32_t* rays_numsteps_compacted, const float* bg_color, uint32_t n_rays,
                                   int rgb_activation, int density_activation, float* rgb_output, void* stream_) {
    XR_REQUIRE(network_output && coords && rays_numsteps && rays_numsteps_compacted && bg_color && rgb_output, "null pointer");
    XR_REQUIRE(((uintptr_t)network_output & 15) == 0, "network_output must be 16-byte aligned");
    XR_REQUIRE(n_rays > 0, "n_rays == 0");
    hipLaunchKernelGGL(k_composite_fwd<false>, dim3(xr_div_up((uint64_t)n_rays * CG, RM_BLOCK)), dim3(RM_BLOCK), 0, (hipStream_t)stream_,
                       n_rays, (const float4*)network_output, coords, rays_numsteps, rays_numsteps_compacted, bg_color,
                       0.f, 0.f, 0.f, rgb_activation, density_activation, rgb_output, (float*)nullptr);
    XR_LAUNCH_CHECK();
    return XR_OK;
}

extern "C" int xr_calc_rgb_inference(const float* network_output, const float* coords, const int32_t* rays_numsteps,
                                     float bg_r, float bg_g, float bg_b, uint32_t n_rays, int rgb_activation,
                                     int density_activation, float* rgb_output, float* alpha_output, void* stream_) {
    XR_REQUIRE(network_output && coords && rays_numsteps && rgb_output && alpha_output, "null pointer");
    XR_REQUIRE(((uintptr_t)network_output & 15) == 0, "network_output must be 16-byte aligned");
    XR_REQUIRE(n_rays > 0, "n_rays == 0");
    hipLaunchKernelGGL(k_composite_fwd<true>, dim3(xr_div_up((uint64_t)n_rays * CG, RM_BLOCK)), dim3(RM_BLOCK), 0, (hipStream_t)stream_,
                       n_rays, (const float4*)network_output, coords, rays_numsteps, rays_numsteps, (const float*)nullptr,
                       bg_r, bg_g, bg_b, rgb_activation, density_activation, rgb_output, alpha_output);
    XR_LAUNCH_CHECK();
    return XR_OK;
}

__global__ __launch_bounds__(RM_BLOCK) void k_slice_select(uint32_t n_rays, const int32_t* __restrict__ numsteps,
                                                            const float* __restrict__ T, float eps, uint32_t s0, uint32_t s1,
                                                            uint32_t* __restrict__ rows, int32_t* __restrict__ ray_off,
                                                            uint32_t* __restrict__ count) {
    const uint32_t i = blockIdx.x * RM_BLOCK + threadIdx.x;
    const int lane = threadIdx.x & 63;
    uint32_t cnt = 0, base = 0;
    if (i < n_rays) {
        const uint32_t n = (uint32_t)numsteps[2 * i];
        base = (uint32_t)numsteps[2 * i + 1];
        if (n > s0 && T[i] > eps) cnt = min(n, s1) - s0;
    }
    uint32_t inc = cnt;
#pragma unroll
    for (int d = 1; d < 64; d <<= 1) { uint32_t o = __shfl_up(inc, d, 64); if (lane >= d) inc += o; }
    const uint32_t wave_total = __shfl(inc, 63, 64);
    uint32_t wave_base = 0;
    if (lane == 63 && wave_total) wave_base = atomicAdd(count, wave_total);
    wave_base = __shfl(wave_base, 63, 64);
    if (i >= n_rays) return;
    if (cnt == 0) { ray_off[i] = -1; return; }
    const uint32_t off = wave_base + inc - cnt;
    ray_off[i] = (int32_t)off;
    for (uint32_t j = 0; j < cnt; ++j) rows[off + j] = base + s0 + j;
}
__global__ __launch_bounds__(RM_BLOCK) void k_slice_composite(uint32_t n_rays, const float4* __restrict__ raw_s,
                                                               const float* __restrict__ coords, const int32_t* __restrict__ numsteps,
                                                               const int32_t* __restrict__ ray_off, uint32_t s0, uint32_t s1,
                                                               int rgb_act, int density_act, float* __restrict__ T,
                                                               float* __restrict__ rgb_acc) {
    const uint32_t i = blockIdx.x * RM_BLOCK + threadIdx.x;
    if (i >= n_rays) return;
    const int32_t off = ray_off[i];
    if (off < 0) return;
    const uint32_t n = (uint32_t)numsteps[2 * i], base = (uint32_t)numsteps[2 * i + 1];
    const uint32_t cnt = min(n, s1) - s0;
    float t = T[i], cr = rgb_acc[3 * i], cg = rgb_acc[3 * i + 1], cb = rgb_acc[3 * i + 2];
    for (uint32_t j = 0; j < cnt; ++j) {
        const float4 o = raw_s[(uint32_t)off + j];
        const float dt = xr_unwarp_dt(coords[7 * (size_t)(base + s0 + j) + 3]);
        const float alpha = 1.f - __expf(-xr_act_density(o.w, density_act) * dt);
        const float w = alpha * t;
        cr += w * xr_act_rgb(o.x, rgb_act); cg += w * xr_act_rgb(o.y, rgb_act); cb += w * xr_act_rgb(o.z, rgb_act);
        t *= (1.f - alpha);
    }
    T[i] = t; rgb_acc[3 * i] = cr; rgb_acc[3 * i + 1] = cg; rgb_acc[3 * i + 2] = cb;
}
extern "C" int xr_render_slice_select(const int32_t* rays_numsteps, const float* T, uint32_t n_rays, uint32_t s0, uint32_t s1,
                                      float eps, uint32_t* rows_out, int32_t* ray_offset_out, uint32_t* count_out, void* stream_) {
    XR_REQUIRE(rays_numsteps && T && rows_out && ray_offset_out && count_out && n_rays > 0 && s1 > s0, "bad argument");
    XR_HIP(hipMemsetAsync(count_out, 0, 4, (hipStream_t)stream_));
    hipLaunchKernelGGL(k_slice_select, dim3(xr_div_up(n_rays, RM_BLOCK)), dim3(RM_BLOCK), 0, (hipStream_t)stream_, n_rays,
                       rays_numsteps, T, eps, s0, s1, rows_out, ray_offset_out, count_out);
    XR_LAUNCH_CHECK();
    return XR_OK;
}
extern "C" int xr_render_slice_composite(const float* raw_slice, const float* coords, const int32_t* rays_numsteps,
                                         const int32_t* ray_offset, uint32_t n_rays, uint32_t s0, uint32_t s1, int rgb_activation,
                                         int density_activation, float* T, float* rgb_acc, void* stream_) {
    XR_REQUIRE(raw_slice && coords && rays_numsteps && ray_offset && T && rgb_acc && n_rays > 0, "bad argument");
    XR_REQUIRE(((uintptr_t)raw_slice & 15) == 0, "raw must be 16-byte aligned");
    hipLaunchKernelGGL(k_slice_composite, dim3(xr_div_up(n_rays, RM_BLOCK)), dim3(RM_BLOCK), 0, (hipStream_t)stream_, n_rays,
                       (const float4*)raw_slice, coords, rays_numsteps, ray_offset, s0, s1, rgb_activation, density_activation,
                       T, rgb_acc);
    XR_LAUNCH_CHECK();
    return XR_OK;
}

__global__ __launch_bounds__(RM_BLOCK) void k_composite_bwd(
    uint32_t n_rays, const float4* __restrict__ raw, const int32_t* __restrict__ numsteps_c,
    const float* __restrict__ coords, const float* __restrict__ grad_rgb, const float* __restrict__ rgb_final,
    const float* __restrict__ density_grid_mean, int rgb_act, int density_act, float4* __restrict__ dout) {
    const uint32_t t = blockIdx.x * RM_BLOCK + threadIdx.x;
    const uint32_t i = t / CG, sub = t % CG;
    const bool in = i < n_rays;
    float loss_scale = 128.f; loss_scale /= (float)n_rays;
    const float l2 = rgb_act == XR_ACT_EXPONENTIAL ? 1e-4f : 0.0f;
    const float l1 = density_grid_mean[0] < 0.01f ? 1e-4f : 0.0f;
    uint32_t n = 0, base = 0;
    if (in) { n = (uint32_t)numsteps_c[2 * i]; base = (uint32_t)numsteps_c[2 * i + 1]; }
    uint32_t k0, k1;
    cg_chunk(n, sub, &k0, &k1);
    float T = 1.f, cr = 0.f, cg = 0.f, cb = 0.f;
    const uint32_t m = k1 - k0;
    float4 oc[CG_RC]; float dc[CG_RC];
    float gr = 0.f, gg = 0.f, gb = 0.f, fr = 0.f, fg = 0.f, fb = 0.f;
    if (in) {
        gr = grad_rgb[3 * i]; gg = grad_rgb[3 * i + 1]; gb = grad_rgb[3 * i + 2];
        fr = rgb_final[3 * i]; fg = rgb_final[3 * i + 1]; fb = rgb_final[3 * i + 2];
    }
    if (m <= CG_RC) {
#pragma unroll
        for (uint32_t u = 0; u < CG_RC; ++u)
            if (u < m) { oc[u] = raw[base + k0 + u]; dc[u] = coords[7 * (size_t)(base + k0 + u) + 3]; }
    }
    auto pass1 = [&](const float4 o, float dtw) {
        const float dt = xr_unwarp_dt(dtw);
        const float alpha = 1.f - __expf(-xr_act_density(o.w, density_act) * dt);
        const float w = alpha * T;
        cr += w * xr_act_rgb(o.x, rgb_act); cg += w * xr_act_rgb(o.y, rgb_act); cb += w * xr_act_rgb(o.z, rgb_act);
        T *= (1.f - alpha);
    };
    if (m <= CG_RC) {
#pragma unroll
        for (uint32_t u = 0; u < CG_RC; ++u) if (u < m) pass1(oc[u], dc[u]);
    } else {
        cg_long(raw, coords, base, k0, k1, [&](const float4 o, float dtw, uint32_t) { pass1(o, dtw); });
    }
    float Tb, ar, ag, ab, Tt, Cr, Cg, Cb;
    cg_stitch(sub, T, cr, cg, cb, &Tb, &ar, &ag, &ab, &Tt, &Cr, &Cg, &Cb);
    if (!in || k0 >= k1) return;
    T = Tb; cr = ar; cg = ag; cb = ab;
    auto pass2 = [&](const float4 o, float dtw, uint32_t k) {
        const float r = xr_act_rgb(o.x, rgb_act), g = xr_act_rgb(o.y, rgb_act), b = xr_act_rgb(o.z, rgb_act);
        const float dt = xr_unwarp_dt(dtw);
        const float density = xr_act_density(o.w, density_act);
        const float alpha = 1.f - __expf(-density * dt);
        const float w = alpha * T;
        cr += w * r; cg += w * g; cb += w * b;
        T *= (1.f - alpha);
        const float sr = fr - cr, sg = fg - cg, sb = fb - cb;
        float4 d;
        d.x = loss_scale * ((w * gr) * xr_dact_rgb(o.x, rgb_act) + fmaxf(0.0f, l2 * o.x));
        d.y = loss_scale * ((w * gg) * xr_dact_rgb(o.y, rgb_act) + fmaxf(0.0f, l2 * o.y));
        d.z = loss_scale * ((w * gb) * xr_dact_rgb(o.z, rgb_act) + fmaxf(0.0f, l2 * o.z));
        const float dot = gr * (T * r - sr) + gg * (T * g - sg) + gb * (T * b - sb);
        d.w = loss_scale * (xr_dact_density(o.w, density_act) * (dt * dot)) + (o.w < 0.f ? -l1 : 0.0f);
        dout[base + k] = d;
    };
    if (m <= CG_RC) {
#pragma unroll
        for (uint32_t u = 0; u < CG_RC; ++u) if (u < m) pass2(oc[u], dc[u], k0 + u);
    } else {
        cg_long(raw, coords, base, k0, k1, pass2);
    }
}

extern "C" int xr_calc_rgb_backward(const float* network_output, const int32_t* rays_numsteps_compacted,
                                    const float* coords, const float* grad_rgb, const float* rgb_output,
                                    const float* density_grid_mean, uint32_t n_rays, int rgb_activation,
                                    int density_activation, float* dloss_doutput, void* stream_) {
    XR_REQUIRE(network_output && rays_numsteps_compacted && coords && grad_rgb && rgb_output && density_grid_mean &&
               dloss_doutput, "null pointer");
    XR_REQUIRE((((uintptr_t)network_output | (uintptr_t)dloss_doutput) & 15) == 0, "raw/grad buffers must be 16-byte aligned");
    XR_REQUIRE(n_rays > 0, "n_rays == 0");
    hipLaunchKernelGGL(k_composite_bwd, dim3(xr_div_up((uint64_t)n_rays * CG, RM_BLOCK)), dim3(RM_BLOCK), 0, (hipStream_t)stream_,
                       n_rays, (const float4*)network_output, rays_numsteps_compacted, coords, grad_rgb, rgb_output,
                       density_grid_mean, rgb_activation, density_activation, (float4*)dloss_doutput);
    XR_LAUNCH_CHECK();
    return XR_OK;
}

#define CT_BLOCK 1024
#define CT_SEGS 68
#define CT_CAP 6144u
#define CT_MARK 0x7fc0a5a5u
#define CT_LDS_BYTES (CT_CAP * 20u)
__global__ __launch_bounds__(CT_BLOCK) void k_composite_train(
    uint32_t n_rays, const float4* __restrict__ raw, const float* __restrict__ coords, const int32_t* __restrict__ numsteps,
    const int32_t* __restrict__ numsteps_c, const float* __restrict__ bg, const float* __restrict__ target,
    const float* __restrict__ alpha_mask, const float* __restrict__ density_grid_mean, int rgb_act, int density_act, float delta,
    float scale, float* __restrict__ rgb_out, float* __restrict__ loss_mse, float4* __restrict__ dout,
    uint32_t* __restrict__ live_seg_count, int stage) {
    extern __shared__ __attribute__((aligned(16))) float4 ct_rows[];
    __shared__ float ws[CT_BLOCK / 64], ws2[CT_BLOCK / 64];
    __shared__ uint32_t seg_hist[CT_SEGS], seg_first, row_lo, row_hi;
    if (live_seg_count && threadIdx.x < CT_SEGS) seg_hist[threadIdx.x] = 0;
    if (threadIdx.x == 0) { row_lo = 0xffffffffu; row_hi = 0u; }
    const uint32_t t = blockIdx.x * CT_BLOCK + threadIdx.x;
    const uint32_t i = t / CG, sub = t % CG;
    const bool in = i < n_rays;
    float loss_scale = 128.f; loss_scale /= (float)n_rays;
    const float l2 = rgb_act == XR_ACT_EXPONENTIAL ? 1e-4f : 0.0f;
    const float l1 = density_grid_mean[0] < 0.01f ? 1e-4f : 0.0f;
    uint32_t n = 0, base = 0, n_full = 0;
    float br = 0.f, bgc = 0.f, bb = 0.f, tr = 0.f, tg = 0.f, tb = 0.f, am = 0.f;
    if (in) {
        n = (uint32_t)numsteps_c[2 * i]; base = (uint32_t)numsteps_c[2 * i + 1]; n_full = (uint32_t)numsteps[2 * i];
        br = bg[3 * i]; bgc = bg[3 * i + 1]; bb = bg[3 * i + 2];
        tr = target[3 * i]; tg = target[3 * i + 1]; tb = target[3 * i + 2];
        am = alpha_mask[i];
    }
    __syncthreads();
    if (stage && in && sub == 0 && n > 0) { atomicMin(&row_lo, base); atomicMax(&row_hi, base + n); }
    __syncthreads();
    const uint32_t lo = row_lo, hi = row_hi;
    const bool staged = stage && hi > lo && hi - lo <= CT_CAP;
    float* const ct_dt = reinterpret_cast<float*>(ct_rows + CT_CAP);
    if (staged) {
        for (uint32_t r = threadIdx.x; r < hi - lo; r += CT_BLOCK) {
            ct_rows[r] = raw[lo + r];
            ct_dt[r] = coords[7 * (size_t)(lo + r) + 3];
        }
        __syncthreads();
    }
    uint32_t k0, k1;
    cg_chunk(n, sub, &k0, &k1);
    float T = 1.f, cr = 0.f, cg = 0.f, cb = 0.f;
    const uint32_t m = k1 - k0;
    const uint32_t slot0 = base - lo;
    float4 oc[CG_RC]; float dc[CG_RC];
    if (m <= CG_RC) {
#pragma unroll
        for (uint32_t u = 0; u < CG_RC; ++u)
            if (u < m) {
                if (staged) { oc[u] = ct_rows[slot0 + k0 + u]; dc[u] = ct_dt[slot0 + k0 + u]; }
                else { oc[u] = raw[base + k0 + u]; dc[u] = coords[7 * (size_t)(base + k0 + u) + 3]; }
            }
    }
    auto long_chunk = [&](auto&& f) {
        if (staged) { for (uint32_t k = k0; k < k1; ++k) f(ct_rows[slot0 + k], ct_dt[slot0 + k], k); }
        else cg_long(raw, coords, base, k0, k1, f);
    };
    auto pass1 = [&](const float4 o, float dtw, uint32_t) {
        const float dt = xr_unwarp_dt(dtw);
        const float alpha = 1.f - __expf(-xr_act_density(o.w, density_act) * dt);
        const float w = alpha * T;
        cr += w * xr_act_rgb(o.x, rgb_act); cg += w * xr_act_rgb(o.y, rgb_act); cb += w * xr_act_rgb(o.z, rgb_act);
        T *= (1.f - alpha);
    };
    if (m <= CG_RC) {
#pragma unroll
        for (uint32_t u = 0; u < CG_RC; ++u) if (u < m) pass1(oc[u], dc[u], 0u);
    } else {
        long_chunk(pass1);
    }
    float Tb, ar, ag, ab, Tt, Cr, Cg, Cb;
    cg_stitch(sub, T, cr, cg, cb, &Tb, &ar, &ag, &ab, &Tt, &Cr, &Cg, &Cb);
    float fr, fg, fb;
    if (n == 0) { fr = br; fg = bgc; fb = bb; }
    else { fr = Cr; fg = Cg; fb = Cb; if (n == n_full) { fr += Tt * br; fg += Tt * bgc; fb += Tt * bb; } }
    float gr, gg, gb, acc = 0.f, mse = 0.f;
    {
        const float d3[3] = {fr - tr, fg - tg, fb - tb};
        float g3[3];
#pragma unroll
        for (int c = 0; c < 3; ++c) {
            const float a = fabsf(d3[c]);
            if (a > delta) { acc += a - 0.5f * delta; g3[c] = scale * (d3[c] > 0.f ? 1.f : -1.f); }
            else { acc += 0.5f / delta * a * a; g3[c] = scale * (d3[c] / delta); }
            const float mm = d3[c] * am; mse += mm * mm;
        }
        gr = g3[0]; gg = g3[1]; gb = g3[2];
    }
    if (!(in && sub == 0)) { acc = 0.f; mse = 0.f; }
    else { rgb_out[3 * i] = fr; rgb_out[3 * i + 1] = fg; rgb_out[3 * i + 2] = fb; }
#pragma unroll
    for (int d = 32; d > 0; d >>= 1) { acc += __shfl_xor(acc, d, 64); mse += __shfl_xor(mse, d, 64); }
    if ((threadIdx.x & 63) == 0) { ws[threadIdx.x >> 6] = acc; ws2[threadIdx.x >> 6] = mse; }
    if (threadIdx.x == 0) seg_first = base / XR_LIVE_SEG;
    __syncthreads();
    if (threadIdx.x == 0) {
        float a = 0.f, b = 0.f;
#pragma unroll
        for (int w = 0; w < CT_BLOCK / 64; ++w) { a += ws[w]; b += ws2[w]; }
        if (loss_mse && a != 0.f) atomicAdd(loss_mse, scale * a);
        if (loss_mse && b != 0.f) atomicAdd(loss_mse + 1, b);
    }
    if (in && k0 < k1) {
        T = Tb; cr = ar; cg = ag; cb = ab;
        auto pass2 = [&](const float4 o, float dtw, uint32_t k) {
            const float r = xr_act_rgb(o.x, rgb_act), g = xr_act_rgb(o.y, rgb_act), b = xr_act_rgb(o.z, rgb_act);
            const float dt = xr_unwarp_dt(dtw);
            const float density = xr_act_density(o.w, density_act);
            const float alpha = 1.f - __expf(-density * dt);
            const float w = alpha * T;
            cr += w * r; cg += w * g; cb += w * b;
            T *= (1.f - alpha);
            const float sr = fr - cr, sg = fg - cg, sb = fb - cb;
            float4 d;
            d.x = loss_scale * ((w * gr) * xr_dact_rgb(o.x, rgb_act) + fmaxf(0.0f, l2 * o.x));
            d.y = loss_scale * ((w * gg) * xr_dact_rgb(o.y, rgb_act) + fmaxf(0.0f, l2 * o.y));
            d.z = loss_scale * ((w * gb) * xr_dact_rgb(o.z, rgb_act) + fmaxf(0.0f, l2 * o.z));
            const float dot = gr * (T * r - sr) + gg * (T * g - sg) + gb * (T * b - sb);
            d.w = loss_scale * (xr_dact_density(o.w, density_act) * (dt * dot)) + (o.w < 0.f ? -l1 : 0.0f);
            if (staged) { ct_rows[slot0 + k] = d; ct_dt[slot0 + k] = __uint_as_float(CT_MARK); }
            else dout[base + k] = d;
            if (live_seg_count && (d.x != 0.f || d.y != 0.f || d.z != 0.f || d.w != 0.f)) {
                const uint32_t sg_ = (base + k) / XR_LIVE_SEG, rel = sg_ - seg_first;
                if (rel < CT_SEGS) atomicAdd(&seg_hist[rel], 1u); else atomicAdd(&live_seg_count[sg_], 1u);
            }
        };
        if (m <= CG_RC) {
#pragma unroll
            for (uint32_t u = 0; u < CG_RC; ++u) if (u < m) pass2(oc[u], dc[u], k0 + u);
        } else {
            long_chunk(pass2);
        }
    }
    if (!live_seg_count && !staged) return;
    __syncthreads();
    if (live_seg_count && threadIdx.x < CT_SEGS && seg_hist[threadIdx.x])
        atomicAdd(&live_seg_count[seg_first + threadIdx.x], seg_hist[threadIdx.x]);
    if (staged)
        for (uint32_t r = threadIdx.x; r < hi - lo; r += CT_BLOCK)
            if (__float_as_uint(ct_dt[r]) == CT_MARK) dout[lo + r] = ct_rows[r];
}

#define CW_RAYS 4
#define CW_RC 2
#define CW_SEGS 8
__global__ __launch_bounds__(64 * CW_RAYS) void k_composite_train_w(
    uint32_t n_rays, const float4* __restrict__ raw, const float* __restrict__ coords, const int32_t* __restrict__ numsteps,
    const int32_t* __restrict__ numsteps_c, const float* __restrict__ bg, const float* __restrict__ target,
    const float* __restrict__ density_grid_mean, int rgb_act, int density_act, float delta, float scale,
    float* __restrict__ rgb_out, float4* __restrict__ dout, uint32_t* __restrict__ live_seg_count) {
    __shared__ uint32_t seg_hist[CW_SEGS], seg_first;
    const uint32_t lane = threadIdx.x & 63, i = blockIdx.x * CW_RAYS + (threadIdx.x >> 6);
    const bool in = i < n_rays;
    if (live_seg_count) {
        if (threadIdx.x < CW_SEGS) seg_hist[threadIdx.x] = 0;
        if (threadIdx.x == 0) seg_first = (uint32_t)numsteps_c[2 * i + 1] / XR_LIVE_SEG;
        __syncthreads();
    }
    float loss_scale = 128.f; loss_scale /= (float)n_rays;
    const float l2 = rgb_act == XR_ACT_EXPONENTIAL ? 1e-4f : 0.0f;
    const float l1 = density_grid_mean[0] < 0.01f ? 1e-4f : 0.0f;
    uint32_t n = 0, base = 0, n_full = 0;
    if (in) { n = (uint32_t)numsteps_c[2 * i]; base = (uint32_t)numsteps_c[2 * i + 1]; n_full = (uint32_t)numsteps[2 * i]; }
    if (n > 0) {
        const uint32_t chunk = (n + 63) / 64;
        const uint32_t k0 = min(n, lane * chunk), k1 = min(n, (lane + 1) * chunk), m = k1 - k0;
        float4 oc[CW_RC]; float dc[CW_RC];
        if (chunk <= CW_RC) {
#pragma unroll
            for (uint32_t u = 0; u < CW_RC; ++u)
                if (u < m) { oc[u] = raw[base + k0 + u]; dc[u] = coords[7 * (size_t)(base + k0 + u) + 3]; }
        }
        const float br = bg[3 * i], bgc = bg[3 * i + 1], bb = bg[3 * i + 2];
        const float tr = target[3 * i], tg = target[3 * i + 1], tb = target[3 * i + 2];
        float T = 1.f, cr = 0.f, cg = 0.f, cb = 0.f;
        auto pass1 = [&](const float4 o, float dtw, uint32_t) {
            const float dt = xr_unwarp_dt(dtw);
            const float alpha = 1.f - __expf(-xr_act_density(o.w, density_act) * dt);
            const float w = alpha * T;
            cr += w * xr_act_rgb(o.x, rgb_act); cg += w * xr_act_rgb(o.y, rgb_act); cb += w * xr_act_rgb(o.z, rgb_act);
            T *= (1.f - alpha);
        };
        if (chunk <= CW_RC) {
#pragma unroll
            for (uint32_t u = 0; u < CW_RC; ++u) if (u < m) pass1(oc[u], dc[u], 0u);
        } else {
            cg_long(raw, coords, base, k0, k1, pass1);
        }
        float Tb1, ar1, ag1, ab1, Tg, Cgr, Cgg, Cgb;
        cg_stitch(lane & 15, T, cr, cg, cb, &Tb1, &ar1, &ag1, &ab1, &Tg, &Cgr, &Cgg, &Cgb);
        float GT = 1.f, Gr = 0.f, Gg = 0.f, Gb = 0.f, Tb = 1.f, ar = 0.f, ag = 0.f, ab = 0.f;
#pragma unroll
        for (int h = 0; h < 4; ++h) {
            const float th = __shfl(Tg, 16 * h, 64), rh = __shfl(Cgr, 16 * h, 64), gh = __shfl(Cgg, 16 * h, 64), bh = __shfl(Cgb, 16 * h, 64);
            if ((int)(lane >> 4) == h) { Tb = GT * Tb1; ar = Gr + GT * ar1; ag = Gg + GT * ag1; ab = Gb + GT * ab1; }
            Gr += GT * rh; Gg += GT * gh; Gb += GT * bh;
            GT *= th;
        }
        const float Tt = GT;
        float fr = Gr, fg = Gg, fb = Gb;
        if (n == n_full) { fr += Tt * br; fg += Tt * bgc; fb += Tt * bb; }
        if (lane == 0) { rgb_out[3 * i] = fr; rgb_out[3 * i + 1] = fg; rgb_out[3 * i + 2] = fb; }
        float g3[3];
        {
            const float d3[3] = {fr - tr, fg - tg, fb - tb};
#pragma unroll
            for (int c = 0; c < 3; ++c) g3[c] = fabsf(d3[c]) > delta ? scale * (d3[c] > 0.f ? 1.f : -1.f) : scale * (d3[c] / delta);
        }
        const float gr = g3[0], gg = g3[1], gb = g3[2];
        if (k0 < k1) {
            T = Tb; cr = ar; cg = ag; cb = ab;
            uint32_t live_lo = 0, live_hi = 0;
            const uint32_t seg_lo = (base + k0) / XR_LIVE_SEG;
            auto pass2 = [&](const float4 o, float dtw, uint32_t k) {
                const float r = xr_act_rgb(o.x, rgb_act), g = xr_act_rgb(o.y, rgb_act), b = xr_act_rgb(o.z, rgb_act);
                const float dt = xr_unwarp_dt(dtw);
                const float density = xr_act_density(o.w, density_act);
                const float alpha = 1.f - __expf(-density * dt);
                const float w = alpha * T;
                cr += w * r; cg += w * g; cb += w * b;
                T *= (1.f - alpha);
                const float ur = fr - cr, ug = fg - cg, ub = fb - cb;
                float4 d;
                d.x = loss_scale * ((w * gr) * xr_dact_rgb(o.x, rgb_act) + fmaxf(0.0f, l2 * o.x));
                d.y = loss_scale * ((w * gg) * xr_dact_rgb(o.y, rgb_act) + fmaxf(0.0f, l2 * o.y));
                d.z = loss_scale * ((w * gb) * xr_dact_rgb(o.z, rgb_act) + fmaxf(0.0f, l2 * o.z));
                const float dot = gr * (T * r - ur) + gg * (T * g - ug) + gb * (T * b - ub);
                d.w = loss_scale * (xr_dact_density(o.w, density_act) * (dt * dot)) + (o.w < 0.f ? -l1 : 0.0f);
                dout[base + k] = d;
                if (d.x != 0.f || d.y != 0.f || d.z != 0.f || d.w != 0.f) {
                    if ((base + k) / XR_LIVE_SEG == seg_lo) ++live_lo; else ++live_hi;
                }
            };
            if (chunk <= CW_RC) {
#pragma unroll
                for (uint32_t u = 0; u < CW_RC; ++u) if (u < m) pass2(oc[u], dc[u], k0 + u);
            } else {
                cg_long(raw, coords, base, k0, k1, pass2);
            }
            if (live_seg_count) {
                const uint32_t rel = seg_lo - seg_first;
                if (live_lo) { if (rel < CW_SEGS) atomicAdd(&seg_hist[rel], live_lo); else atomicAdd(&live_seg_count[seg_lo], live_lo); }
                if (live_hi) { if (rel + 1 < CW_SEGS) atomicAdd(&seg_hist[rel + 1], live_hi); else atomicAdd(&live_seg_count[seg_lo + 1], live_hi); }
            }
        }
    } else if (in && lane == 0) {
        rgb_out[3 * i] = bg[3 * i]; rgb_out[3 * i + 1] = bg[3 * i + 1]; rgb_out[3 * i + 2] = bg[3 * i + 2];
    }
    if (!live_seg_count) return;
    __syncthreads();
    if (threadIdx.x < CW_SEGS && seg_hist[threadIdx.x]) atomicAdd(&live_seg_count[seg_first + threadIdx.x], seg_hist[threadIdx.x]);
}

#define LS_THREADS XR_AUX_LS_VTHREADS
__global__ __launch_bounds__(LS_THREADS) void k_train_loss_scalars(const float* __restrict__ rgb, const float* __restrict__ target,
                                                                  const float* __restrict__ alpha_mask, uint32_t n_rays, float delta,
                                                                  float scale, float* __restrict__ out) {
    __shared__ float ws[LS_THREADS / 64], ws2[LS_THREADS / 64];
    xr_aux_loss_block<LS_THREADS>(rgb, target, alpha_mask, n_rays, delta, scale, out, ws, ws2);
}
extern "C" int xr_train_loss_scalars(const float* rgb, const float* target, const float* alpha_mask, uint32_t n_rays, float delta,
                                     float scale, float* loss_mse_out, void* stream_) {
    XR_REQUIRE(rgb && target && alpha_mask && loss_mse_out && n_rays > 0, "bad argument");
    hipLaunchKernelGGL(k_train_loss_scalars, dim3(1), dim3(LS_THREADS), 0, (hipStream_t)stream_, rgb, target, alpha_mask, n_rays, delta,
                       scale, loss_mse_out);
    XR_LAUNCH_CHECK();
    return XR_OK;
}

extern "C" int xr_composite_train(const float* network_output, const float* coords, const int32_t* rays_numsteps,
                                   const int32_t* rays_numsteps_compacted, const float* bg_color, const float* target,
                                   const float* alpha_mask, const float* density_grid_mean, uint32_t n_rays, int rgb_activation,
                                   int density_activation, float delta, float scale, float* rgb_output, float* loss_mse_out,
                                   float* dloss_doutput, uint32_t* live_seg_count, void* stream_) {
    XR_REQUIRE(network_output && coords && rays_numsteps && rays_numsteps_compacted && bg_color && target && alpha_mask &&
               density_grid_mean && rgb_output && dloss_doutput, "null pointer");
    XR_REQUIRE((((uintptr_t)network_output | (uintptr_t)dloss_doutput) & 15) == 0, "raw/grad buffers must be 16-byte aligned");
    XR_REQUIRE(n_rays > 0, "n_rays == 0");
#ifndef XR_CT_WAVE
#define XR_CT_WAVE 1
#endif
#ifndef XR_CT_STAGE
#define XR_CT_STAGE 1
#endif
    if (!loss_mse_out && XR_CT_WAVE) {
        hipLaunchKernelGGL(k_composite_train_w, dim3(xr_div_up(n_rays, CW_RAYS)), dim3(64 * CW_RAYS), 0, (hipStream_t)stream_, n_rays,
                           (const float4*)network_output, coords, rays_numsteps, rays_numsteps_compacted, bg_color, target,
                           density_grid_mean, rgb_activation, density_activation, delta, scale, rgb_output, (float4*)dloss_doutput,
                           live_seg_count);
        XR_LAUNCH_CHECK();
        return XR_OK;
    }
    const int stage = XR_CT_STAGE;
    static thread_local bool attr_set = false;
    if (!attr_set) {
        XR_HIP(hipFuncSetAttribute((const void*)k_composite_train, hipFuncAttributeMaxDynamicSharedMemorySize, (int)CT_LDS_BYTES));
        attr_set = true;
    }
    hipLaunchKernelGGL(k_composite_train, dim3(xr_div_up((uint64_t)n_rays * CG, CT_BLOCK)), dim3(CT_BLOCK), CT_LDS_BYTES, (hipStream_t)stream_,
                       n_rays, (const float4*)network_output, coords, rays_numsteps, rays_numsteps_compacted, bg_color, target,
                       alpha_mask, density_grid_mean, rgb_activation, density_activation, delta, scale, rgb_output, loss_mse_out,
                       (float4*)dloss_doutput, live_seg_count, stage);
    XR_LAUNCH_CHECK();
    return XR_OK;
}
```

xrnerf_amd/csrc/xr_step.hip:

```cpp
#include "xr_common.h"
#include "xr_aux.h"
#include <cstdlib>
#include <initializer_list>

extern "C" void* xr_timing_event_create(void) {
    hipEvent_t e = nullptr;
    return hipEventCreate(&e) == hipSuccess ? (void*)e : nullptr;
}
extern "C" int xr_timing_event_destroy(void* e) { return e && hipEventDestroy((hipEvent_t)e) != hipSuccess ? XR_EHIP : XR_OK; }
extern "C" int xr_timing_event_elapsed_ms(void* a, void* b, float* ms) {
    XR_REQUIRE(a && b && ms, "null pointer");
    XR_HIP(hipEventElapsedTime(ms, (hipEvent_t)a, (hipEvent_t)b));
    return XR_OK;
}
extern "C" int xr_event_record(void* event, void* stream) {
    XR_REQUIRE(event, "null event");
    XR_HIP(hipEventRecord((hipEvent_t)event, (hipStream_t)stream));
    return XR_OK;
}

static bool stage_is(const char* timed, const char* name) { return timed && strcmp(timed, name) == 0; }

extern "C" int xr_ngp_train_step(
    const float* table, const float* w_density, const float* w_color, int n_hidden_density, int n_hidden_color, float pad_value,
    int mlp_mode, int n_levels, const float* scale_host, const uint32_t* resolution_host, const uint32_t* offset_host,
    const float* coords, uint32_t n_rows, const uint32_t* n_dev, const int32_t* rays_numsteps, const int32_t* rays_numsteps_compacted,
    uint32_t n_rays, const float* bg_color, const float* target, const float* alpha_mask, const float* density_grid_mean,
    int rgb_activation, int density_activation, float huber_delta, float loss_scale,
    float* enc_t, uint32_t ld, float* raw, float* draw, float* denc_t, float* rgb_out,
    float* zero_block, size_t zero_floats, float* grad_w_density, float* grad_w_color, float* loss_mse, uint32_t* live_seg_count,
    float* grad_table, size_t table_floats, int zero_draw,
    void* ws_mlp_bwd, size_t ws_mlp_bwd_bytes, void* ws_scatter, size_t ws_scatter_bytes, int scatter_level0,
    const float* xyz_planes, uint32_t plane_stride, const xr_adam_fuse* table_adam, const xr_adam_fuse* w_density_adam,
    const xr_adam_fuse* w_color_adam, const char* timed_entry, void* timing_begin, void* timing_end, void* stream_) {
    XR_REQUIRE(table && w_density && w_color && coords && rays_numsteps && rays_numsteps_compacted && bg_color && target &&
               alpha_mask && density_grid_mean && enc_t && raw && draw && denc_t && rgb_out && zero_block && grad_w_density &&
               grad_w_color && loss_mse && (grad_table || table_adam), "null pointer");
    XR_REQUIRE(!table_adam || (scatter_level0 == 0 && table_adam->param == table), "the fused table update takes the whole table of this step");
    XR_REQUIRE(!w_density_adam == !w_color_adam, "the two MLP tensors' updates come together");
    XR_REQUIRE(!w_density_adam || (w_density_adam->param == w_density && w_color_adam->param == w_color && w_density_adam->step == w_color_adam->step &&
                                   w_density_adam->n > 0 && w_color_adam->n > 0),
               "mlp_adam: the step's own weight tensors, one step count");
    XR_REQUIRE(!table_adam || xr_internal_hashgrid_bwd_adam_supported(n_rows, n_levels, scale_host, resolution_host, offset_host),
               "the fused table update needs a non-atomic scatter path for every level at this row capacity");
    XR_REQUIRE(n_rows > 0 && n_rays > 0 && ld >= n_rows, "bad sizes");
    XR_REQUIRE(mlp_mode >= 0 && mlp_mode <= 3, "mlp_mode is 0 (fp32 MFMA), 1 (fp16), 2 (fp32 forward on 3-way split bf16 operands) or 3 (on 2-way split fp16 operands)");
    XR_REQUIRE(scatter_level0 >= 0 && scatter_level0 < n_levels, "scatter_level0 outside [0, n_levels)");
    XR_REQUIRE(!timed_entry || (timing_begin && timing_end), "a timed entry point needs its two events");
    hipStream_t stream = (hipStream_t)stream_;
#ifndef XR_STEP_REDUCE_AUX
#define XR_STEP_REDUCE_AUX 1
#endif
    const bool reduce_aux = XR_STEP_REDUCE_AUX != 0;
    auto begin = [&](const char* name) -> int { if (stage_is(timed_entry, name)) XR_HIP(hipEventRecord((hipEvent_t)timing_begin, stream)); return XR_OK; };
    auto end = [&](const char* name) -> int {
        if (stage_is(timed_entry, name)) XR_HIP(hipEventRecord((hipEvent_t)timing_end, stream));
        return XR_OK;
    };
    int rc;
    if ((rc = begin("xr_hashgrid_fwd")) != XR_OK) return rc;
    if (xyz_planes) rc = xr_hashgrid_fwd(table, xyz_planes, 1, plane_stride, n_rows, n_dev, nullptr, n_levels, scale_host, resolution_host, offset_host, enc_t, ld, stream_);
    else rc = xr_hashgrid_fwd(table, coords, 7, 1, n_rows, n_dev, nullptr, n_levels, scale_host, resolution_host, offset_host, enc_t, ld, stream_);
    if (rc != XR_OK) return rc;
    if ((rc = end("xr_hashgrid_fwd")) != XR_OK || (rc = begin("xr_nerf_mlp_fwd")) != XR_OK) return rc;
    rc = xr_nerf_mlp_fwd(mlp_mode, enc_t, ld, coords + 4, 7, n_rows, n_dev, nullptr, w_density, w_color, n_hidden_density, n_hidden_color, pad_value,
                         raw, stream_);
    if (rc != XR_OK) return rc;
    if ((rc = end("xr_nerf_mlp_fwd")) != XR_OK) return rc;
    (void)zero_block; (void)zero_floats;
    if (zero_draw) XR_HIP(hipMemsetAsync(draw, 0, (size_t)n_rows * 4 * sizeof(float), stream));
    static const bool live_on = []() { const char* e = getenv("XR_MLP_LIVE"); return !(e && e[0] == '0'); }();
    uint32_t *rows = nullptr, *seg = nullptr, *n_live = nullptr;
    if (live_on) {
        rc = xr_nerf_mlp_bwd_list_slots(ws_mlp_bwd, ws_mlp_bwd_bytes, n_rows, &rows, &seg, &n_live);
        if (rc != XR_OK) return rc;
        if (live_seg_count) seg = live_seg_count;
        else XR_HIP(hipMemsetAsync(seg, 0, XR_LIVE_ROWS_SEGMENTS(n_rows) * sizeof(uint32_t), stream));
    }
    if ((rc = begin("xr_composite_train")) != XR_OK) return rc;
    rc = xr_composite_train(raw, coords, rays_numsteps, rays_numsteps_compacted, bg_color, target, alpha_mask, density_grid_mean,
                             n_rays, rgb_activation, density_activation, huber_delta, loss_scale, rgb_out, nullptr, draw, seg, stream_);
    if (rc != XR_OK) return rc;
    if ((rc = end("xr_composite_train")) != XR_OK) return rc;
    if ((rc = begin("xr_live_rows")) != XR_OK) return rc;
    if (live_on) {
        rc = xr_live_rows(draw, n_rows, n_dev, seg, rows, n_live, nullptr, ld, 1, stream_);
        if (rc != XR_OK) return rc;
    }
    if ((rc = end("xr_live_rows")) != XR_OK || (rc = begin("xr_nerf_mlp_bwd")) != XR_OK) return rc;
    xr_internal_defer_mlp_reduce(true);
    rc = xr_nerf_mlp_bwd(mlp_mode, enc_t, ld, coords + 4, 7, n_rows, n_dev, w_density, w_color, n_hidden_density, n_hidden_color, pad_value, draw, denc_t,
                         grad_w_density, grad_w_color, ws_mlp_bwd, ws_mlp_bwd_bytes, rows, n_live, stream_);
    xr_internal_defer_mlp_reduce(false);
    if (rc != XR_OK) return rc;
    if ((rc = end("xr_nerf_mlp_bwd")) != XR_OK) return rc;
    XrAuxWork aux; memset(&aux, 0, sizeof(aux));
    if ((rc = xr_internal_mlp_bwd_reduce_desc(ws_mlp_bwd, n_rows, n_hidden_density, n_hidden_color, &aux)) != XR_OK) return rc;
    aux.g0 = grad_w_density; aux.g1 = grad_w_color; aux.overwrite = 1;
    const bool aux_adam = w_density_adam && w_color_adam && (uint32_t)w_density_adam->n == aux.split && (uint32_t)w_color_adam->n == aux.gw - aux.split;
    if (aux_adam) {
        const xr_adam_fuse* ad[2] = {w_density_adam, w_color_adam};
        XrAdamArgs* A[2] = {&aux.a0, &aux.a1};
        const xr_adam_fuse& H = *w_density_adam;
        const float bc1 = 1.f - powf(H.beta1, (float)H.step), bc2 = 1.f - powf(H.beta2, (float)H.step);
        const bool ema = ad[0]->ema && ad[1]->ema;
        for (int k = 0; k < 2; ++k)
            *A[k] = XrAdamArgs{ad[k]->param, ad[k]->m, ad[k]->v, ema ? ad[k]->ema : nullptr, H.beta1, H.beta2, H.lr / bc1, sqrtf(bc2), H.eps,
                               H.weight_decay, H.ema_momentum, H.grad_scale};
        aux.adam = 1;
    }
    aux.rgb = rgb_out; aux.target = target; aux.alpha = alpha_mask; aux.n_rays = n_rays; aux.delta = huber_delta; aux.scale = loss_scale; aux.loss = loss_mse;
    if (live_on && live_seg_count) { aux.clear = live_seg_count; aux.clear_words = XR_LIVE_ROWS_SEGMENTS(n_rows); }
    if (reduce_aux) xr_internal_scatter_aux_work(&aux);
    if ((rc = begin("xr_hashgrid_bwd")) != XR_OK) return rc;
    if (table_adam)
        rc = xr_hashgrid_bwd_adam(coords, 7, denc_t, ld, n_rows, live_on ? n_live : n_dev, rows, n_levels, scale_host, resolution_host, offset_host,
                                  ws_scatter, ws_scatter_bytes, table_adam, stream_);
    else
        rc = xr_hashgrid_bwd(coords, 7, denc_t + (size_t)2 * scatter_level0 * ld, ld, n_rows, live_on ? n_live : n_dev, rows, n_levels - scatter_level0,
                              scale_host + scatter_level0, resolution_host + scatter_level0, offset_host + scatter_level0, grad_table,
                              ws_scatter, ws_scatter_bytes, XR_SCATTER_OVERWRITE, stream_);
    xr_internal_scatter_aux_work(nullptr);
    if (rc != XR_OK) return rc;
    if (!aux.done) {
        if ((rc = xr_internal_mlp_bwd_reduce(ws_mlp_bwd, n_rows, n_hidden_density, n_hidden_color, grad_w_density, grad_w_color, 1, stream_)) != XR_OK) return rc;
        if (aux.clear) XR_HIP(hipMemsetAsync(aux.clear, 0, (size_t)aux.clear_words * sizeof(uint32_t), stream));
        if (w_density_adam) {
            float* p[2] = {w_density_adam->param, w_color_adam->param}; const float* g[2] = {grad_w_density, grad_w_color};
            float* m[2] = {w_density_adam->m, w_color_adam->m}; float* v[2] = {w_density_adam->v, w_color_adam->v};
            float* e[2] = {w_density_adam->ema, w_color_adam->ema};
            const size_t nn[2] = {(size_t)w_density_adam->n, (size_t)w_color_adam->n};
            rc = xr_adam_step_multi(2, p, g, m, v, (e[0] && e[1]) ? e : nullptr, nn, w_density_adam->step, w_density_adam->lr, w_density_adam->beta1,
                                    w_density_adam->beta2, w_density_adam->eps, w_density_adam->weight_decay, w_density_adam->ema_momentum,
                                    w_density_adam->grad_scale, stream_);
            if (rc != XR_OK) return rc;
        }
        if ((rc = xr_train_loss_scalars(rgb_out, target, alpha_mask, n_rays, huber_delta, loss_scale, loss_mse, stream_)) != XR_OK) return rc;
    } else if (w_density_adam && !aux_adam) {
        float* p[2] = {w_density_adam->param, w_color_adam->param}; const float* g[2] = {grad_w_density, grad_w_color};
        float* m[2] = {w_density_adam->m, w_color_adam->m}; float* v[2] = {w_density_adam->v, w_color_adam->v};
        float* e[2] = {w_density_adam->ema, w_color_adam->ema};
        const size_t nn[2] = {(size_t)w_density_adam->n, (size_t)w_color_adam->n};
        rc = xr_adam_step_multi(2, p, g, m, v, (e[0] && e[1]) ? e : nullptr, nn, w_density_adam->step, w_density_adam->lr, w_density_adam->beta1,
                                w_density_adam->beta2, w_density_adam->eps, w_density_adam->weight_decay, w_density_adam->ema_momentum,
                                w_density_adam->grad_scale, stream_);
        if (rc != XR_OK) return rc;
    }
    if ((rc = end("xr_hashgrid_bwd")) != XR_OK) return rc;
    return XR_OK;
}

extern "C" int xr_ngp_window_march(const xr_ngp_window* W, uint32_t first_chunk, uint32_t n_chunks, uint32_t batches_ready, uint32_t n_rays,
                                   const float* rays_rgb_rows, uint64_t n_table_rays, uint64_t* cur_ray, uint64_t batch_seed,
                                   uint64_t batch_call_index, const uint8_t* bitfield, float aabb0, float aabb1, float near_distance,
                                   float cone_angle, uint32_t max_samples, uint64_t k1_call_index, uint32_t max_compacted, void* workspace,
                                   size_t workspace_bytes, uint32_t* counter_host_pinned, void* stream_) {
    XR_REQUIRE(W && cur_ray && bitfield && W->rays_o && W->rays_d && W->target && W->alpha && W->bg && W->img_ids && W->rays_index &&
               W->rays_numsteps && W->numsteps_clipped && W->coords && W->counter2 && W->n_valid, "null pointer");
    XR_REQUIRE(n_chunks >= 1 && first_chunk + n_chunks <= (uint32_t)XR_NGP_WINDOW && batches_ready <= n_chunks, "chunks outside the window");
    XR_REQUIRE(n_rays >= 1 && n_rays <= W->ray_stride && W->coords_stride >= max_samples, "the window's buffers are too small");
    XR_REQUIRE(batches_ready == n_chunks || (rays_rgb_rows && n_rays <= n_table_rays), "no ray table to draw the batches from");
    const size_t r0 = (size_t)first_chunk * W->ray_stride;
    uint64_t st, inc;
    int rc;
    if (batches_ready < n_chunks) {
        uint64_t row0[XR_NGP_WINDOW];
        uint64_t cur = *cur_ray;
        for (uint32_t c = batches_ready; c < n_chunks; ++c) {
            if (cur + n_rays > n_table_rays) cur = 0;
            row0[c - batches_ready] = cur;
            cur += n_rays;
        }
        *cur_ray = cur;
        const size_t rb = r0 + (size_t)batches_ready * W->ray_stride;
        xr_pcg32_host_state(batch_seed, batch_call_index, &st, &inc);
        rc = xr_make_batch_series(rays_rgb_rows, row0, n_rays, n_chunks - batches_ready, W->ray_stride, st, inc, W->rays_o + 3 * rb, W->rays_d + 3 * rb,
                                  W->target + 3 * rb, W->alpha + rb, W->bg + 3 * rb, W->img_ids + rb, stream_);
        if (rc != XR_OK) return rc;
    }
    xr_pcg32_host_state(9121, k1_call_index, &st, &inc);
    rc = xr_rays_sampler_series(W->rays_o + 3 * r0, W->rays_d + 3 * r0, W->ray_stride, bitfield, n_rays, n_chunks, aabb0, aabb1, near_distance, cone_angle,
                                max_samples, st, inc, W->coords + 7 * (size_t)first_chunk * W->coords_stride, W->coords_stride, W->rays_index + r0,
                                W->rays_numsteps + 2 * r0, W->counter2 + 2 * first_chunk,
                                W->xyz_planes ? W->xyz_planes + 3 * (size_t)first_chunk * W->plane_stride : nullptr, W->plane_stride, workspace,
                                workspace_bytes, stream_);
    if (rc != XR_OK) return rc;
    rc = xr_clip_numsteps(W->rays_numsteps + 2 * r0, W->counter2 + 2 * first_chunk, n_rays, n_chunks, W->ray_stride, max_compacted,
                                 W->numsteps_clipped + 2 * r0, W->n_valid + 2 * first_chunk, stream_);
    if (rc != XR_OK) return rc;
    if (counter_host_pinned)
        XR_HIP(hipMemcpyAsync(counter_host_pinned + 2 * first_chunk, W->counter2 + 2 * first_chunk, (size_t)n_chunks * 2 * sizeof(uint32_t),
                              hipMemcpyDeviceToHost, (hipStream_t)stream_));
    return XR_OK;
}

extern "C" int xr_ngp_loop_run(const xr_ngp_loop_desc* desc, xr_ngp_loop_state* state, uint32_t k, uint32_t n_rays, const float* lr,
                               const float* ema_momentum, const char* timed_entry, void* const* timing_events, void* const* iter_events) {
    XR_REQUIRE(desc && state && lr && ema_momentum, "null pointer");
    const xr_ngp_loop_desc& D = *desc;
    xr_ngp_loop_state& S = *state;
    const xr_ngp_window& W = D.window;
    XR_REQUIRE(k >= 1 && k <= (uint32_t)XR_NGP_WINDOW && n_rays >= 1 && n_rays <= W.ray_stride, "bad sizes");
    XR_REQUIRE(!timed_entry || timing_events, "a timed entry point needs its events");
    const xr_grad_exchange* X = D.exchange;
    XR_REQUIRE(D.adam_w_density.param == D.w_density && D.adam_w_color.param == D.w_color, "the updates name the step's tensors");
    XR_REQUIRE(X ? (D.dp_mode == 1 ? (D.shard_grad && D.table_padded && D.shard_floats > 0 && D.adam_table.n == D.shard_floats &&
                                        D.adam_table.param == D.table_padded + (uint64_t)X->rank * D.shard_floats && X->reduce_scatter && X->all_gather)
                                    : (D.dp_mode == 0 && D.adam_table.param == D.table))
                 : D.adam_table.param == D.table, "the table update names the step's table (zero1: this rank's shard of it)");
    XR_REQUIRE(!X || (X->all_reduce && X->finish && X->world_size >= 1 && D.step[0].grad_table && D.step[1].grad_table &&
                      D.split_level >= 0 && D.split_level < D.n_levels && (D.dp_mode == 0 || D.split_level == 0)), "bad exchange");
    XR_REQUIRE(W.coords && W.rays_numsteps && W.numsteps_clipped && W.n_valid && W.bg && W.target && W.alpha && W.coords_stride >= D.n_rows, "bad window");
    hipStream_t stream = (hipStream_t)D.stream;
    int rc;
    xr_adam_fuse at = D.adam_table, ad = D.adam_w_density, ac = D.adam_w_color;
    for (uint32_t j = 0; j < k; ++j) {
        const uint64_t it = S.iter;
        if (iter_events) XR_HIP(hipEventRecord((hipEvent_t)iter_events[j], stream));
        const size_t c = (size_t)(it % (uint64_t)XR_NGP_WINDOW), r0 = c * W.ray_stride;
        S.step_turn ^= 1u;
        const xr_ngp_step_set& B = D.step[S.step_turn & 1u];
        S.adam_step += 1;
        at.step = ad.step = ac.step = S.adam_step;
        at.lr = ad.lr = ac.lr = lr[j];
        at.ema_momentum = ad.ema_momentum = ac.ema_momentum = ema_momentum[j];
        const float* coords = W.coords + 7 * c * W.coords_stride;
        const size_t table_floats = 2 * (size_t)D.offset_host[D.n_levels];
        rc = xr_ngp_train_step(D.table, D.w_density, D.w_color, D.n_hidden_density, D.n_hidden_color, D.pad_value, D.mlp_mode, D.n_levels, D.scale_host,
                               D.resolution_host, D.offset_host, coords, D.n_rows, W.n_valid + 2 * c, W.rays_numsteps + 2 * r0,
                               W.numsteps_clipped + 2 * r0, n_rays, W.bg + 3 * r0, W.target + 3 * r0, W.alpha + r0, D.density_grid_mean, D.rgb_activation,
                               D.density_activation, D.huber_delta, D.loss_scale, B.enc_t, D.ld, B.raw, B.draw, B.denc_t, B.rgb_out, B.zero_block,
                               B.zero_floats, B.grad_w_density, B.grad_w_color, B.loss_mse, B.live_seg_count, X ? B.grad_table : nullptr,
                               X ? table_floats : 0, 0, D.ws_mlp_bwd, D.ws_mlp_bwd_bytes, D.ws_scatter, D.ws_scatter_bytes, X ? D.split_level : 0,
                               W.xyz_planes ? W.xyz_planes + 3 * c * W.plane_stride : nullptr, W.plane_stride, X ? nullptr : &at, X ? nullptr : &ad,
                               X ? nullptr : &ac, timed_entry, timed_entry ? timing_events[2 * j] : nullptr,
                               timed_entry ? timing_events[2 * j + 1] : nullptr, D.stream);
        if (rc != XR_OK) return rc;
        if (X) {
            XR_REQUIRE(B.grad_w_color == B.grad_w_density + D.adam_w_density.n, "the two MLP gradients form one bucket");
            if ((rc = X->all_reduce(X->ctx, B.grad_w_density, (size_t)(D.adam_w_density.n + D.adam_w_color.n), D.stream)) != XR_OK) return rc;
            if (D.dp_mode == 1) {
                if ((rc = X->reduce_scatter(X->ctx, B.grad_table, D.shard_grad, (size_t)D.shard_floats, D.stream)) != XR_OK) return rc;
            } else if (D.split_level > 0) {
                const size_t cut = 2 * (size_t)D.offset_host[D.split_level];
                if ((rc = X->all_reduce(X->ctx, B.grad_table + cut, table_floats - cut, D.stream)) != XR_OK) return rc;
                uint32_t *rows = nullptr, *seg = nullptr, *n_live = nullptr;
                static const bool live_on = []() { const char* e = getenv("XR_MLP_LIVE"); return !(e && e[0] == '0'); }();
                if (live_on && (rc = xr_nerf_mlp_bwd_list_slots(D.ws_mlp_bwd, D.ws_mlp_bwd_bytes, D.n_rows, &rows, &seg, &n_live)) != XR_OK) return rc;
                rc = xr_hashgrid_bwd(coords, 7, B.denc_t, D.ld, D.n_rows, live_on ? n_live : W.n_valid + 2 * c, live_on ? rows : nullptr, D.split_level,
                                      D.scale_host, D.resolution_host, D.offset_host, B.grad_table, D.ws_scatter, D.ws_scatter_bytes, XR_SCATTER_OVERWRITE, D.stream);
                if (rc != XR_OK) return rc;
                if ((rc = X->all_reduce(X->ctx, B.grad_table, cut, D.stream)) != XR_OK) return rc;
            } else if ((rc = X->all_reduce(X->ctx, B.grad_table, table_floats, D.stream)) != XR_OK) return rc;
            if ((rc = X->finish(X->ctx, D.stream)) != XR_OK) return rc;
            float* p[3] = {at.param, ad.param, ac.param};
            const float* g[3] = {D.dp_mode == 1 ? D.shard_grad : B.grad_table, B.grad_w_density, B.grad_w_color};
            float* m[3] = {at.m, ad.m, ac.m}; float* v[3] = {at.v, ad.v, ac.v}; float* e[3] = {at.ema, ad.ema, ac.ema};
            const size_t nn[3] = {(size_t)at.n, (size_t)ad.n, (size_t)ac.n};
            rc = xr_adam_step_multi(3, p, g, m, v, (e[0] && e[1] && e[2]) ? e : nullptr, nn, at.step, at.lr, at.beta1, at.beta2, at.eps, at.weight_decay,
                                    at.ema_momentum, 1.0f / (float)X->world_size, D.stream);
            if (rc != XR_OK) return rc;
            if (D.dp_mode == 1) {
                if ((rc = X->all_gather(X->ctx, at.param, D.table_padded, (size_t)D.shard_floats, D.stream)) != XR_OK) return rc;
                if ((rc = X->finish(X->ctx, D.stream)) != XR_OK) return rc;
            }
        }
        S.last_step_set = S.step_turn & 1u;
        S.iter = it + 1;
    }
    if (iter_events) XR_HIP(hipEventRecord((hipEvent_t)iter_events[k], stream));
    return XR_OK;
}
```

xrnerf_amd/ops.py:

```python
import ctypes as C
import os

import numpy as np
import torch

from . import _lib

G3 = 128 ** 3
N_GRID = 8 * G3

_workspaces = {}


class KernelTimer:

    def __init__(self, only=None, train_only=False):
        self.events = {}
        self.only = only
        self.train_only = train_only

    def span(self, name, units=0, train=True):
        if self.only is not None and name not in self.only:
            return _NOSPAN
        if self.train_only and not train:
            return _NOSPAN
        return _Span(self, name, units)

    STEP_STAGES = ('xr_hashgrid_fwd', 'xr_nerf_mlp_fwd', 'xr_composite_train', 'xr_live_rows', 'xr_nerf_mlp_bwd', 'xr_hashgrid_bwd')

    def native_stage(self):
        if self.only is None:
            return False, None
        inside = [k for k in self.only if k in self.STEP_STAGES]
        return len(inside) <= 1, (inside[0] if inside else None)

    def summary(self):
        return {k: (len(v), sum(a.elapsed_time(b) for a, b, _ in v), sum(u for _, _, u in v))
                for k, v in self.events.items()}


class _Span:
    def __init__(self, timer, name, units):
        self.timer, self.name, self.units = timer, name, units

    def __enter__(self):
        self.a = torch.cuda.Event(enable_timing=True)
        self.b = torch.cuda.Event(enable_timing=True)
        self.a.record()

    def __exit__(self, *exc):
        self.b.record()
        self.timer.events.setdefault(self.name, []).append((self.a, self.b, self.units))


class _CEvent:

    def __init__(self):
        self.h = _lib.load().xr_timing_event_create()
        if not self.h:
            raise _lib.XrError('cannot create a timing event')

    def elapsed_time(self, other):
        ms = C.c_float()
        _lib.check(_lib.load().xr_timing_event_elapsed_ms(self.h, other.h, C.byref(ms)), 'xr_timing_event_elapsed_ms')
        return float(ms.value)

    def __del__(self):
        try:
            _lib.load().xr_timing_event_destroy(self.h)
        except Exception:
            pass


class _NoSpan:
    def __enter__(self):
        return None

    def __exit__(self, *exc):
        return False


TIMER = None
_NOSPAN = _NoSpan()


def _span(name, units=0, train=True):
    return TIMER.span(name, units, train) if TIMER is not None else _NOSPAN


_PRECISION = os.environ.get('XRNERF_MLP_PRECISION', 'f32')
if _PRECISION not in ('f32', 'f16'):
    raise ValueError("XRNERF_MLP_PRECISION must be 'f32' or 'f16' (got %r)" % _PRECISION)


_F32_FORWARD = os.environ.get('XRNERF_F32_FORWARD', 'f16x2')
if _F32_FORWARD not in ('f16x2', 'bf16x3', 'mfma'):
    raise ValueError("XRNERF_F32_FORWARD must be 'f16x2', 'bf16x3' or 'mfma' (got %r)" % _F32_FORWARD)


def f32_forward():
    return _F32_FORWARD


def set_f32_forward(kind):
    global _F32_FORWARD
    if kind not in ('f16x2', 'bf16x3', 'mfma'):
        raise ValueError("the fp32 forward is 'f16x2', 'bf16x3' or 'mfma'")
    _F32_FORWARD = kind


def _mlp_mode(nhd=1, nhc=2):
    if nhd == 1 and nhc == 2:
        if _PRECISION == 'f16':
            return 1
        if _F32_FORWARD == 'bf16x3':
            return 2
    return 3 if _F32_FORWARD == 'f16x2' else 0


def precision():
    return _PRECISION


def set_precision(p):
    global _PRECISION
    if p not in ('f32', 'f16'):
        raise ValueError("precision must be 'f32' or 'f16'")
    _PRECISION = p


def _stream():
    return C.c_void_p(torch._C._cuda_getCurrentRawStream(torch.cuda.current_device()))


def _on_device(t):
    return t.is_cuda


def _ptr(t):
    if t is None:
        return None
    if not _on_device(t):
        raise _lib.XrError('xrnerf_amd ops need ROCm device tensors (got a %s tensor): there is no CPU fallback' % t.device)
    if not t.is_contiguous():
        raise _lib.XrError('tensor must be contiguous')
    return C.c_void_p(t.data_ptr())


def _ws(device, nbytes, tag):
    key = (str(device), tag)
    w = _workspaces.get(key)
    if w is None or w.numel() < nbytes:
        w = torch.empty(max(int(nbytes), 256), dtype=torch.uint8, device=device)
        if tag == 'mlpbwd':
            w.zero_()
        _workspaces[key] = w
    return w


def _buf(device, shape, tag):
    n = 1
    for v in shape:
        n *= int(v)
    key = (str(device), tag)
    have = _workspaces.get(key)
    need = 4 * max(n, 1) + 256
    w = _ws(device, need if (have is not None and have.numel() >= need) else need + need // 4, tag)
    off = (-w.data_ptr()) % 16
    return w[off:off + 4 * n].view(torch.float32).view(*shape)


_helpers = {}
_helper_current = {}


def _ensure_helper(device):
    import threading
    if device.type != 'cuda':
        return
    tid = threading.get_ident()
    key = (str(device), tid)
    if _helper_current.get(tid) == key:
        return
    h = _helpers.get(key)
    if h is None:
        with torch.cuda.device(device):
            st = torch.cuda.Stream(device=device)
            evs = (torch.cuda.Event(), torch.cuda.Event())
            for e in evs:
                e.record(st)
        h = _helpers[key] = (st, evs)
    st, evs = h
    _lib.check(_lib.load().xr_set_helper_stream(C.c_void_p(st.cuda_stream), C.c_void_p(evs[0].cuda_event), C.c_void_p(evs[1].cuda_event)),
               'xr_set_helper_stream')
    _helper_current[tid] = key


_range_words = {}
_range_current = {}
_range_off = set()


def mlp_range_word(device):
    import threading
    if device.type != 'cuda':
        return None
    w = _range_words.get(str(device))
    if w is None:
        w = _range_words[str(device)] = torch.zeros((1,), dtype=torch.int32, device=device)
    tid = threading.get_ident()
    want = None if tid in _range_off else str(device)
    if _range_current.get(tid, 0) != want:
        _lib.check(_lib.load().xr_set_mlp_range_word(C.c_void_p(w.data_ptr()) if want is not None else None), 'xr_set_mlp_range_word')
        _range_current[tid] = want
    return w


def mlp_range_tracking(device, on):
    import threading
    tid = threading.get_ident()
    if on:
        _range_off.discard(tid)
    else:
        _range_off.add(tid)
    mlp_range_word(device)


def mlp_range_events(device, reset=False):
    w = mlp_range_word(device)
    if w is None:
        return 0
    v = int(w.item())
    if reset and v:
        w.zero_()
    return v


def pcg32_host_state(ncalls, seed=9121):
    s, i = C.c_uint64(), C.c_uint64()
    _lib.load().xr_pcg32_host_state(seed, ncalls, C.byref(s), C.byref(i))
    return s.value, i.value


def rays_sampler(rays_o, rays_d, bitfield, aabb, near_distance, cone_angle, max_samples, rng_calls,
                 coords_out=None, ws_tag='k1', small_out=None, xyz_out=None, rng_chunk=0, rng_ray0=0, wide=False):
    L = _lib.load()
    n = rays_o.shape[0]
    dev = rays_o.device
    if coords_out is None:
        coords_out = torch.empty((max_samples, 7), dtype=torch.float32, device=dev)
    if small_out is not None:
        rays_index, numsteps, counter = small_out
    else:
        rays_index = torch.empty((n, 1), dtype=torch.int32, device=dev)
        numsteps = torch.empty((n, 2), dtype=torch.int32, device=dev)
        counter = torch.empty((2,), dtype=torch.int32, device=dev)
    nb = L.xr_rays_sampler_workspace_bytes(n, 1)
    ws = _ws(dev, nb, ws_tag)
    st, inc = pcg32_host_state(rng_calls)
    with _span('xr_rays_sampler', n):
        _lib.check(L.xr_rays_sampler(_ptr(rays_o), _ptr(rays_d), _ptr(bitfield), n, aabb[0], aabb[1], near_distance,
                                      cone_angle, max_samples, st, inc, _ptr(coords_out), _ptr(rays_index),
                                      _ptr(numsteps), _ptr(counter), _ptr(xyz_out), xyz_out.shape[1] if xyz_out is not None else 0,
                                      int(rng_chunk), int(rng_ray0), 1 if wide else 0, _ptr(ws), ws.numel(), _stream()), 'xr_rays_sampler')
    return coords_out, rays_index, numsteps, counter


def compacted_coord(coords_in, numsteps, max_compacted, coords_out=None):
    L = _lib.load()
    n = numsteps.shape[0]
    dev = coords_in.device
    if coords_out is None:
        coords_out = torch.zeros((max_compacted, 7), dtype=torch.float32, device=dev)
    nc = torch.empty((n, 2), dtype=torch.int32, device=dev)
    rc = torch.empty((1,), dtype=torch.int32, device=dev)
    sc = torch.empty((1,), dtype=torch.int32, device=dev)
    ws = _ws(dev, L.xr_rays_sampler_workspace_bytes(n, 1), 'k1')
    _lib.check(L.xr_compacted_coord(_ptr(coords_in), _ptr(numsteps), n, max_compacted, _ptr(coords_out), _ptr(nc),
                                    _ptr(rc), _ptr(sc), _ptr(ws), ws.numel(), _stream()), 'xr_compacted_coord')
    return coords_out, nc, rc, sc


def calc_rgb_forward(raw, coords, numsteps, numsteps_c, bg, rgb_act, density_act, out=None):
    L = _lib.load()
    n = numsteps.shape[0]
    if out is None:
        out = torch.empty((n, 3), dtype=torch.float32, device=raw.device)
    with _span('xr_calc_rgb_forward', 0):
        _lib.check(L.xr_calc_rgb_forward(_ptr(raw), _ptr(coords), _ptr(numsteps), _ptr(numsteps_c), _ptr(bg), n,
                                         int(rgb_act), int(density_act), _ptr(out), _stream()), 'xr_calc_rgb_forward')
    return out


def calc_rgb_backward(raw, numsteps_c, coords, grad_rgb, rgb_out, density_grid_mean, rgb_act, density_act, out=None):
    L = _lib.load()
    n = numsteps_c.shape[0]
    if out is None:
        out = torch.zeros_like(raw)
    with _span('xr_calc_rgb_backward', 0):
        _lib.check(L.xr_calc_rgb_backward(_ptr(raw), _ptr(numsteps_c), _ptr(coords), _ptr(grad_rgb), _ptr(rgb_out),
                                          _ptr(density_grid_mean), n, int(rgb_act), int(density_act), _ptr(out),
                                          _stream()), 'xr_calc_rgb_backward')
    return out


def composite_train(raw, coords, numsteps, numsteps_c, bg, target, alpha, density_grid_mean, rgb_act, density_act, loss_mse, draw,
                    delta=0.1, scale=5.0, rgb=None, live_seg=None):
    n = numsteps.shape[0]
    if rgb is None:
        rgb = torch.empty((n, 3), dtype=torch.float32, device=raw.device)
    p_seg = _ptr(live_seg)
    with _span('xr_composite_train', 0):
        _lib.check(_lib.load().xr_composite_train(_ptr(raw), _ptr(coords), _ptr(numsteps), _ptr(numsteps_c), _ptr(bg), _ptr(target),
                                                   _ptr(alpha), _ptr(density_grid_mean), n, int(rgb_act), int(density_act),
                                                   float(delta), float(scale), _ptr(rgb), _ptr(loss_mse), _ptr(draw), p_seg, _stream()),
                   'xr_composite_train')
    return rgb


class MarchWindow:

    N = _lib.WINDOW

    def __init__(self, device, ray_stride, coords_stride, planes=True):
        W = self.N
        f = lambda *shape: torch.empty(shape, dtype=torch.float32, device=device)
        i = lambda *shape: torch.empty(shape, dtype=torch.int32, device=device)
        self.device, self.ray_stride, self.coords_stride = device, int(ray_stride), int(coords_stride)
        self.rays_o, self.rays_d, self.target, self.bg = f(W, ray_stride, 3), f(W, ray_stride, 3), f(W, ray_stride, 3), f(W, ray_stride, 3)
        self.alpha, self.img_ids = f(W, ray_stride, 1), i(W, ray_stride, 1)
        self.rays_index, self.numsteps, self.clipped = i(W, ray_stride, 1), i(W, ray_stride, 2), i(W, ray_stride, 2)
        self.coords = f(W, coords_stride, 7)
        self.xyz = f(W, 3, coords_stride) if planes else None
        self.counter2, self.n_valid = i(W, 2), i(W, 2)
        self.pinned = torch.zeros((W, 2), dtype=torch.int32).pin_memory() if device.type == 'cuda' else None
        c = _lib.Window()
        vp = lambda t: t.data_ptr() if t is not None else None
        c.rays_o, c.rays_d, c.target, c.alpha, c.bg, c.img_ids = vp(self.rays_o), vp(self.rays_d), vp(self.target), vp(self.alpha), vp(self.bg), vp(self.img_ids)
        c.rays_index, c.rays_numsteps, c.numsteps_clipped = vp(self.rays_index), vp(self.numsteps), vp(self.clipped)
        c.ray_stride, c.coords, c.coords_stride = self.ray_stride, vp(self.coords), self.coords_stride
        c.xyz_planes, c.plane_stride = vp(self.xyz), (self.coords_stride if planes else 0)
        c.counter2, c.n_valid = vp(self.counter2), vp(self.n_valid)
        self.c = c

    def batch(self, c, n):
        return {'rays_o': self.rays_o[c, :n], 'rays_d': self.rays_d[c, :n], 'target_s': self.target[c, :n], 'alpha': self.alpha[c, :n],
                'img_ids': self.img_ids[c, :n], 'bg_color': self.bg[c, :n]}

    def batch_out(self, c):
        return {'rays_o': self.rays_o[c], 'rays_d': self.rays_d[c], 'target_s': self.target[c], 'alpha': self.alpha[c],
                'img_ids': self.img_ids[c], 'bg_color': self.bg[c]}


def ngp_window_march(win, first_chunk, n_chunks, batches_ready, n, rows_table, cur_ray, batch_call_index, bitfield, aabb, near_distance,
                     cone_angle, max_samples, k1_call_index, max_compacted, batch_seed=20220901, ws_tag='k1_window'):
    L = _lib.load()
    ws = _ws(win.device, L.xr_rays_sampler_workspace_bytes(n, n_chunks), ws_tag)
    try:
        native = L.xr_ngp_window_march
    except AttributeError:
        native = None
    if native is not None:
        cur = C.c_uint64(int(cur_ray))
        with _span('xr_rays_sampler', n * n_chunks):
            _lib.check(native(C.byref(win.c), first_chunk, n_chunks, batches_ready, n, _ptr(rows_table),
                              rows_table.shape[0] if rows_table is not None else 0, C.byref(cur), batch_seed, batch_call_index,
                              _ptr(bitfield), aabb[0], aabb[1], near_distance, cone_angle, max_samples, k1_call_index, max_compacted,
                              _ptr(ws), ws.numel(), C.c_void_p(win.pinned.data_ptr()) if win.pinned is not None else None, _stream()),
                       'xr_ngp_window_march')
        return int(cur.value)
    c0, c1, cur = first_chunk, first_chunk + n_chunks, int(cur_ray)
    if batches_ready < n_chunks:
        row0 = []
        for _ in range(batches_ready, n_chunks):
            if cur + n > rows_table.shape[0]:
                cur = 0
            row0.append(cur)
            cur += n
        b0 = c0 + batches_ready
        st, inc = pcg32_host_state(batch_call_index, batch_seed)
        _lib.check(L.xr_make_batch_series(_ptr(rows_table), (C.c_uint64 * len(row0))(*row0), n, len(row0), win.ray_stride, st, inc, _ptr(win.rays_o[b0:c1]),
                                          _ptr(win.rays_d[b0:c1]), _ptr(win.target[b0:c1]), _ptr(win.alpha[b0:c1]), _ptr(win.bg[b0:c1]),
                                          _ptr(win.img_ids[b0:c1]), _stream()), 'xr_make_batch_series')
    st, inc = pcg32_host_state(k1_call_index)
    _lib.check(L.xr_rays_sampler_series(_ptr(win.rays_o[c0:c1]), _ptr(win.rays_d[c0:c1]), win.ray_stride, _ptr(bitfield), n, n_chunks, aabb[0], aabb[1],
                                        near_distance, cone_angle, max_samples, st, inc, _ptr(win.coords[c0:c1]), win.coords_stride,
                                        _ptr(win.rays_index[c0:c1]), _ptr(win.numsteps[c0:c1]), _ptr(win.counter2[c0:c1]),
                                        _ptr(win.xyz[c0:c1]) if win.xyz is not None else None, win.coords_stride if win.xyz is not None else 0,
                                        _ptr(ws), ws.numel(), _stream()), 'xr_rays_sampler_series')
    _lib.check(L.xr_clip_numsteps(_ptr(win.numsteps[c0:c1]), _ptr(win.counter2[c0:c1]), n, n_chunks, win.ray_stride, max_compacted,
                                         _ptr(win.clipped[c0:c1]), _ptr(win.n_valid[c0:c1]), _stream()), 'xr_clip_numsteps')
    return cur


class TrainStepBuffers:

    def __init__(self, device, n_rows, ray_cap, table_floats, wd_floats, wc_floats, meta, table_grad_storage=None):
        f = lambda *shape: torch.empty(shape, dtype=torch.float32, device=device)
        self.n_rows, self.ray_cap, self.ld = n_rows, ray_cap, (n_rows + 63) // 64 * 64
        self.enc_t, self.denc_t = f(meta.n_output_dims, self.ld), f(meta.n_output_dims, self.ld)
        self.raw, self.draw, self.rgb = f(n_rows, 4), f(n_rows, 4), f(ray_cap, 3)
        n_seg = live_segments(n_rows)
        self.zero_block = torch.zeros((wd_floats + wc_floats + 4 + n_seg,), dtype=torch.float32, device=device)
        self.live_seg = self.zero_block[wd_floats + wc_floats + 4:]
        self.g_wd, self.g_wc = self.zero_block[:wd_floats], self.zero_block[wd_floats:wd_floats + wc_floats]
        self.g_mlp = self.zero_block[:wd_floats + wc_floats]
        self.loss_mse = self.zero_block[wd_floats + wc_floats:wd_floats + wc_floats + 2]
        self.g_table = table_grad_storage(device)[1] if table_grad_storage is not None else f(table_floats)


def ngp_train_step(table, wd, wc, nhd, nhc, pad_value, meta, coords, n_dev, numsteps, numsteps_c, bg, target, alpha,
                   density_grid_mean, rgb_act, density_act, bufs, huber_delta=0.1, loss_scale=5.0, scatter_level0=0, xyz=None,
                   adam=None, mlp_adam=None):
    global LIVE_STATS
    L = _lib.load()
    n_rays = numsteps.shape[0]
    mode = _mlp_mode(nhd, nhc)
    mlp_range_word(coords.device)
    key = (table.data_ptr(), wd.data_ptr(), wc.data_ptr(), coords.data_ptr(), coords.shape[0], n_dev.data_ptr() if n_dev is not None else 0,
           numsteps.data_ptr(), numsteps_c.data_ptr(), bg.data_ptr(), target.data_ptr(), alpha.data_ptr(), density_grid_mean.data_ptr(),
           xyz.data_ptr() if xyz is not None else 0, xyz.shape[1] if xyz is not None else 0, nhd, nhc, pad_value, mode, id(meta),
           int(rgb_act), int(density_act), huber_delta, loss_scale, int(scatter_level0))
    cache = bufs.__dict__.setdefault('_step_args', {})
    ent = cache.get(key)
    if ent is None:
        n_rows = bufs.n_rows
        if coords.shape[0] < n_rows or coords.shape[1] != 7 or not coords.is_contiguous():
            raise _lib.XrError('coords must be contiguous [>= n_rows, 7] rows')
        s, r, o = meta._args()
        _ensure_helper(coords.device)
        _ws(coords.device, L.xr_nerf_mlp_bwd_workspace_bytes(n_rows, nhd, nhc), 'mlpbwd')
        ws_sc = _ws(coords.device, L.xr_hashgrid_bwd_workspace_bytes(n_rows, meta.n_levels, r, o), 'hgb')
        ws_mlp, live_list, _, live_stats = _list_slots(coords.device, n_rows, nhd, nhc)
        live = (live_list, live_stats) if os.environ.get('XR_MLP_LIVE') != '0' else None
        head = (_ptr(table), _ptr(wd), _ptr(wc), nhd, nhc, pad_value, mode, meta.n_levels, s, r, o,
                _ptr(coords), n_rows, _ptr(n_dev), _ptr(numsteps), _ptr(numsteps_c))
        mid = (_ptr(bg), _ptr(target), _ptr(alpha),
               _ptr(density_grid_mean), int(rgb_act), int(density_act), float(huber_delta), float(loss_scale),
               _ptr(bufs.enc_t), bufs.ld, _ptr(bufs.raw), _ptr(bufs.draw), _ptr(bufs.denc_t), _ptr(bufs.rgb),
               _ptr(bufs.zero_block), bufs.zero_block.numel(), _ptr(bufs.g_wd), _ptr(bufs.g_wc), _ptr(bufs.loss_mse), _ptr(bufs.live_seg),
               _ptr(bufs.g_table), bufs.g_table.numel(), 0 if n_dev is not None else 1,
               _ptr(ws_mlp), ws_mlp.numel(), _ptr(ws_sc), ws_sc.numel(), int(scatter_level0),
               _ptr(xyz), xyz.shape[1] if xyz is not None else 0)
        if len(cache) > 16:
            cache.clear()
        ent = cache[key] = (head, mid, live, live_stats, (ws_mlp, ws_sc, meta, table, wd, wc))
    head, mid, live, LIVE_STATS = ent[0], ent[1], ent[2], ent[3]
    bufs.live = live
    stage, ev = None, (None, None)
    if TIMER is not None:
        ok, stage = TIMER.native_stage()
        if not ok:
            raise _lib.XrError('this KernelTimer needs the per-entry-point launch sequence (XRNERF_STEP=py)')
        if stage is not None:
            ev = (_CEvent(), _CEvent())
            TIMER.events.setdefault(stage, []).append((ev[0], ev[1], 0))
    rc = L.xr_ngp_train_step(*head, n_rays, *mid, C.byref(adam) if adam is not None else None,
                             C.byref(mlp_adam[0]) if mlp_adam else None, C.byref(mlp_adam[1]) if mlp_adam else None,
                             stage.encode() if stage else None, ev[0].h if stage else None, ev[1].h if stage else None, _stream())
    if rc != 0:
        _lib.check(rc, 'xr_ngp_train_step')
    return bufs.rgb[:n_rays]


def record_event(cevent):
    _lib.check(_lib.load().xr_event_record(cevent.h, _stream()), 'xr_event_record')


def calc_rgb_inference(raw, coords, numsteps, bg3, rgb_act, density_act):
    L = _lib.load()
    n = numsteps.shape[0]
    rgb = torch.empty((n, 3), dtype=torch.float32, device=raw.device)
    alpha = torch.empty((n, 1), dtype=torch.float32, device=raw.device)
    if raw.shape[0] == 0 or coords.shape[0] == 0:
        raw = torch.zeros((1, 4), dtype=torch.float32, device=numsteps.device)
        coords = torch.zeros((1, 7), dtype=torch.float32, device=numsteps.device)
    _lib.check(L.xr_calc_rgb_inference(_ptr(raw), _ptr(coords), _ptr(numsteps), float(bg3[0]), float(bg3[1]),
                                       float(bg3[2]), n, int(rgb_act), int(density_act), _ptr(rgb), _ptr(alpha),
                                       _stream()), 'xr_calc_rgb_inference')
    return rgb, alpha


def render_slice_select(numsteps, T, s0, s1, eps, rows, ray_off, count):
    _lib.check(_lib.load().xr_render_slice_select(_ptr(numsteps), _ptr(T), numsteps.shape[0], s0, s1, eps, _ptr(rows),
                                                  _ptr(ray_off), _ptr(count), _stream()), 'xr_render_slice_select')


def render_slice_composite(raw_s, coords, numsteps, ray_off, s0, s1, rgb_act, density_act, T, rgb_acc):
    _lib.check(_lib.load().xr_render_slice_composite(_ptr(raw_s), _ptr(coords), _ptr(numsteps), _ptr(ray_off),
                                                     numsteps.shape[0], s0, s1, int(rgb_act), int(density_act), _ptr(T),
                                                     _ptr(rgb_acc), _stream()), 'xr_render_slice_composite')


def generate_grid_samples(grid, ema_step, n_elements, n_cascades, thresh, aabb, rng_calls, planes_out=None, idx_out=None, offset=0):
    L = _lib.load()
    dev = grid.device
    st, inc = pcg32_host_state(rng_calls)
    if planes_out is not None:
        if n_elements:
            _ptr(planes_out); _ptr(idx_out)
            _lib.check(L.xr_generate_grid_samples(_ptr(grid), ema_step, n_elements, n_cascades, thresh, aabb[0], aabb[1], st, inc,
                                                   C.c_void_p(planes_out.data_ptr() + 4 * offset), 1, planes_out.stride(0),
                                                   C.c_void_p(idx_out.data_ptr() + 4 * offset), _stream()), 'xr_generate_grid_samples')
        return planes_out[:, offset:offset + n_elements], idx_out[offset:offset + n_elements]
    pos = torch.empty((n_elements, 3), dtype=torch.float32, device=dev)
    idx = torch.empty((n_elements,), dtype=torch.int32, device=dev)
    _lib.check(L.xr_generate_grid_samples(_ptr(grid), ema_step, n_elements, n_cascades, thresh, aabb[0], aabb[1],
                                          st, inc, _ptr(pos), 3, 1, _ptr(idx), _stream()), 'xr_generate_grid_samples')
    return pos, idx


def mark_untrained_density_grid(focal, xforms, n_elements, resolutions, grid=None):
    L = _lib.load()
    if grid is None:
        grid = torch.empty((n_elements,), dtype=torch.float32, device=focal.device)
    _lib.check(L.xr_mark_untrained_density_grid(_ptr(focal), _ptr(xforms), n_elements, xforms.shape[0],
                                                int(resolutions[0]), int(resolutions[1]), _ptr(grid), _stream()),
               'xr_mark_untrained_density_grid')
    return grid


def splat_grid_samples(mlp_out, indices, padded_width, n_samples, grid_tmp):
    if not _on_device(mlp_out):
        raise _lib.XrError('xrnerf_amd ops need ROCm device tensors: there is no CPU fallback')
    _lib.check(_lib.load().xr_splat_grid_samples(C.c_void_p(mlp_out.data_ptr()), _ptr(indices), padded_width, n_samples,
                                                 _ptr(grid_tmp), _stream()), 'xr_splat_grid_samples')
    return grid_tmp


def ema_grid_samples(grid_tmp, n_elements, decay, grid):
    _lib.check(_lib.load().xr_ema_grid_samples(_ptr(grid_tmp), n_elements, decay, _ptr(grid), _stream()),
               'xr_ema_grid_samples')
    return grid


def update_bitfield(grid, mean, bitfield):
    L = _lib.load()
    ws = _ws(grid.device, L.xr_update_bitfield_workspace_bytes(), 'k10')
    _lib.check(L.xr_update_bitfield(_ptr(grid), _ptr(mean), _ptr(bitfield), _ptr(ws), ws.numel(), _stream()),
               'xr_update_bitfield')
    return bitfield, mean


def ema_update_bitfield(grid_tmp, n_elements, decay, grid, mean, bitfield):
    L = _lib.load()
    ws = _ws(grid.device, L.xr_update_bitfield_workspace_bytes(), 'k10')
    _lib.check(L.xr_ema_update_bitfield(_ptr(grid_tmp), n_elements, decay, _ptr(grid), _ptr(mean), _ptr(bitfield), _ptr(ws), ws.numel(), _stream()),
               'xr_ema_update_bitfield')
    return grid


def bitfield_from_mean(grid, mean, bitfield):
    _lib.check(_lib.load().xr_bitfield_from_mean(_ptr(grid), _ptr(mean), _ptr(bitfield), _stream()),
               'xr_bitfield_from_mean')
    return bitfield


class GridMeta:

    def __init__(self, n_levels=16, log2_hashmap_size=19, base_resolution=16, per_level_scale=None):
        if per_level_scale is None:
            per_level_scale = float(np.exp2(np.log2(2048 * 1 / 16) / (16 - 1)))
        self.n_levels = int(n_levels)
        self.log2_hashmap_size = int(log2_hashmap_size)
        self.n_features = 2
        self.scale = np.zeros(n_levels, np.float32)
        self.resolution = np.zeros(n_levels, np.uint32)
        self.offset = np.zeros(n_levels + 1, np.uint32)
        _lib.load().xr_hashgrid_meta(n_levels, log2_hashmap_size, base_resolution, per_level_scale,
                                     self.scale.ctypes.data, self.resolution.ctypes.data, self.offset.ctypes.data)
        self.n_params = int(self.offset[-1]) * 2
        self.n_output_dims = 2 * self.n_levels

    def _args(self):
        return self.scale.ctypes.data, self.resolution.ctypes.data, self.offset.ctypes.data


def _pos_view(x):
    if x.dim() != 2 or x.shape[1] < 3 or x.dtype != torch.float32:
        raise _lib.XrError('positions must be a 2-D float32 tensor with >= 3 columns')
    if x.stride(1) != 1:
        raise _lib.XrError('positions must have unit column stride')
    if not _on_device(x):
        raise _lib.XrError('xrnerf_amd ops need ROCm device tensors (got a %s tensor): there is no CPU fallback' % x.device)
    return x, int(x.stride(0))


def clip_numsteps(numsteps, counter, max_compacted, out=None):
    n = numsteps.shape[0]
    if out is not None:
        out, n_valid = out
    else:
        out = torch.empty_like(numsteps)
        n_valid = torch.empty((2,), dtype=torch.int32, device=numsteps.device)
    _lib.check(_lib.load().xr_clip_numsteps(_ptr(numsteps), _ptr(counter), n, 1, n, max_compacted, _ptr(out), _ptr(n_valid),
                                            _stream()), 'xr_clip_numsteps')
    return out, n_valid


def hashgrid_fwd(table, x, meta, enc_t=None, ld=None, n_dev=None, rows=None, row0=0, count=None, levels=None):
    L = _lib.load()
    if x.dim() == 2 and x.shape[0] == 3 and x.shape[1] != 3 and x.stride(1) == 1:
        if x.dtype != torch.float32 or not _on_device(x):
            raise _lib.XrError('positions must be float32 device tensors')
        xs, xcs, n_x = 1, int(x.stride(0)), x.shape[1]
    else:
        x, xs = _pos_view(x)
        xcs, n_x = 1, x.shape[0]
    n = n_x if rows is None else rows.shape[0]
    if ld is None:
        ld = (n + 63) // 64 * 64
    if enc_t is None:
        enc_t = torch.empty((meta.n_output_dims, ld), dtype=torch.float32, device=x.device)
    s, r, o = meta._args()
    l0, l1 = (0, meta.n_levels) if levels is None else levels
    if not 0 <= l0 < l1 <= meta.n_levels:
        raise _lib.XrError('bad level range %r' % (levels,))
    if count is not None:
        n = count
    xp = x.data_ptr() + 4 * xs * row0
    ep = enc_t.data_ptr() + 4 * (row0 + 2 * l0 * ld)
    with _span('xr_hashgrid_fwd', 0 if n_dev is not None else n, train=n_dev is not None):
        _ptr(enc_t)
        _lib.check(L.xr_hashgrid_fwd(_ptr(table), C.c_void_p(xp), xs, xcs, n, _ptr(n_dev), _ptr(rows), l1 - l0, s + 4 * l0, r + 4 * l0,
                                      o + 4 * l0, C.c_void_p(ep), ld, _stream()), 'xr_hashgrid_fwd')
    return enc_t


def hashgrid_bwd(x, denc_t, meta, grad_table, n_dev=None, row0=0, count=None, levels=None, use_workspace=True, live=None,
                 overwrite=False):
    L = _lib.load()
    _ensure_helper(denc_t.device)
    x, xs = _pos_view(x)
    n = x.shape[0] if count is None else count
    s, r, o = meta._args()
    l0, l1 = (0, meta.n_levels) if levels is None else levels
    if not 0 <= l0 < l1 <= meta.n_levels:
        raise _lib.XrError('bad level range %r' % (levels,))
    ld = denc_t.shape[1]
    _ptr(denc_t)
    ws = _ws(x.device, L.xr_hashgrid_bwd_workspace_bytes(n, l1 - l0, r + 4 * l0, o + 4 * l0), 'hgb') if use_workspace else None
    rows = None
    if live is not None:
        if row0:
            raise _lib.XrError('a live-row list addresses rows from 0')
# ... 1141 lines not shown
```

Measured before the change: 36.96 million.

## Compact hit rays in clip kernel and composite only over the hit list

The numsteps clip kernel now uses wave ballots and one atomic per block to build a compacted list of rays with nonzero samples. The training composite kernel walks only that list, while separate workgroups handle background-only rays, so empty rays no longer occupy full 64-lane waves. The cost is an extra memset and atomics in the clip kernel, plus thread-local global state that passes the list into the train step.

```diff
diff --git a/include/xrnerf_mi355.h b/include/xrnerf_mi355.h
--- a/include/xrnerf_mi355.h
+++ b/include/xrnerf_mi355.h
@@ -62,6 +62,10 @@
                        const float* alpha_mask, const float* density_grid_mean, uint32_t n_rays, int rgb_activation,
                        int density_activation, float delta, float scale, float* rgb_output, float* loss_mse_out,
                        float* dloss_doutput, uint32_t* live_seg_count, void* stream);
+int xr_composite_train_hits(const float* network_output, const float* coords, const int32_t* rays_numsteps_compacted,
+                            const uint32_t* hit_list, const uint32_t* hit_count, const float* bg_color, const float* target,
+                            const float* density_grid_mean, uint32_t n_rays, int rgb_activation, int density_activation, float delta,
+                            float scale, float* rgb_output, float* dloss_doutput, uint32_t* live_seg_count, void* stream);
 int xr_train_loss_scalars(const float* rgb, const float* target, const float* alpha_mask, uint32_t n_rays, float delta,
                           float scale, float* loss_mse_out, void* stream);
 int xr_calc_rgb_inference(const float* network_output, const float* coords, const int32_t* rays_numsteps,
@@ -166,6 +170,7 @@
     float* coords; size_t coords_stride;
     float* xyz_planes; uint32_t plane_stride;
     uint32_t *counter2, *n_valid;
+    uint32_t *hit_list, *hit_count;
 } xr_ngp_window;
 int xr_ngp_window_march(const xr_ngp_window* window, uint32_t first_chunk, uint32_t n_chunks, uint32_t batches_ready, uint32_t n_rays,
                         const float* rays_rgb_rows, uint64_t n_table_rays, uint64_t* cur_ray, uint64_t batch_seed, uint64_t batch_call_index,
diff --git a/xrnerf_amd/_lib.py b/xrnerf_amd/_lib.py
--- a/xrnerf_amd/_lib.py
+++ b/xrnerf_amd/_lib.py
@@ -16,7 +16,7 @@
     _fields_ = [(k, C.c_void_p) for k in ('rays_o', 'rays_d', 'target', 'alpha', 'bg', 'img_ids', 'rays_index', 'rays_numsteps',
                                           'numsteps_clipped')] + \
                [('ray_stride', C.c_uint32), ('coords', C.c_void_p), ('coords_stride', C.c_size_t), ('xyz_planes', C.c_void_p),
-                ('plane_stride', C.c_uint32), ('counter2', C.c_void_p), ('n_valid', C.c_void_p)]
+                ('plane_stride', C.c_uint32), ('counter2', C.c_void_p), ('n_valid', C.c_void_p), ('hit_list', C.c_void_p), ('hit_count', C.c_void_p)]
 
 
 class StepSet(C.Structure):
@@ -79,6 +79,7 @@
     'xr_hashgrid_bwd_adam': (_i32, [_vp, _u32, _vp, _u32, _u32, _vp, _vp, _i32, _vp, _vp, _vp, _vp, _sz, _vp, _vp]),
     'xr_train_loss_scalars': (_i32, [_vp, _vp, _vp, _u32, _f, _f, _vp, _vp]),
     'xr_composite_train': (_i32, [_vp, _vp, _vp, _vp, _vp, _vp, _vp, _vp, _u32, _i32, _i32, _f, _f, _vp, _vp, _vp, _vp, _vp]),
+    'xr_composite_train_hits': (_i32, [_vp, _vp, _vp, _vp, _vp, _vp, _vp, _vp, _u32, _i32, _i32, _f, _f, _vp, _vp, _vp, _vp]),
     'xr_calc_rgb_inference': (_i32, [_vp, _vp, _vp, _f, _f, _f, _u32, _i32, _i32, _vp, _vp, _vp]),
     'xr_generate_grid_samples': (_i32, [_vp, _u32, _u32, _u32, _f, _f, _f, _u64, _u64, _vp, _u32, _u32, _vp, _vp]),
     'xr_mark_untrained_density_grid': (_i32, [_vp, _vp, _u32, _u32, _i32, _i32, _vp, _vp]),
diff --git a/xrnerf_amd/csrc/xr_common.h b/xrnerf_amd/csrc/xr_common.h
--- a/xrnerf_amd/csrc/xr_common.h
+++ b/xrnerf_amd/csrc/xr_common.h
@@ -116,5 +116,8 @@
 const XrHelper* xr_internal_helper();
 int xr_internal_hashgrid_bwd_adam_supported(uint32_t n, int n_levels, const float* scale_host, const uint32_t* resolution_host,
                                             const uint32_t* offset_host);
+int xr_internal_clip_numsteps_hits(const int32_t* numsteps_in, const uint32_t* counter2, uint32_t n_rays, uint32_t n_series, uint32_t ray_stride,
+                                   uint32_t max_compacted, int32_t* numsteps_out, uint32_t* n_valid_dev, uint32_t* hits, uint32_t* hit_count, void* stream);
+void xr_internal_composite_hit_list(const uint32_t* hits, const uint32_t* hit_count);
 void xr_internal_defer_mlp_reduce(bool on);
 int xr_internal_mlp_bwd_reduce(const void* workspace, uint32_t n, int n_hidden_density, int n_hidden_color, float* grad_w_density, float* grad_w_color, int overwrite, void* stream);
diff --git a/xrnerf_amd/csrc/xr_misc.hip b/xrnerf_amd/csrc/xr_misc.hip
--- a/xrnerf_amd/csrc/xr_misc.hip
+++ b/xrnerf_amd/csrc/xr_misc.hip
@@ -10,7 +10,7 @@
     va_end(ap);
 }
 extern "C" const char* xr_last_error(void) { return g_err; }
-extern "C" int xr_version(void) { return 123; }
+extern "C" int xr_version(void) { return 124; }
 
 extern "C" void xr_pcg32_host_state(uint64_t seed, uint64_t ncalls, uint64_t* state_host, uint64_t* inc_host) {
     xr_pcg32 r; r.seed(seed, 1u);
diff --git a/xrnerf_amd/csrc/xr_raymarch.hip b/xrnerf_amd/csrc/xr_raymarch.hip
--- a/xrnerf_amd/csrc/xr_raymarch.hip
+++ b/xrnerf_amd/csrc/xr_raymarch.hip
@@ -488,7 +488,8 @@
 __global__ __launch_bounds__(RM_BLOCK) void k2_clip(uint32_t n_rays, uint32_t max_compacted, const int32_t* __restrict__ in,
                                                      const uint32_t* __restrict__ counter2, int32_t* __restrict__ out,
                                                      uint32_t* __restrict__ n_valid, uint32_t chunk_rows, uint32_t n_chunks,
-                                                     uint32_t ray_stride) {
+                                                     uint32_t ray_stride, uint4* __restrict__ hits, uint32_t* __restrict__ hit_count) {
+    __shared__ uint32_t s_wave_hits[RM_BLOCK / 64], s_hit_base;
     const uint32_t i = blockIdx.x * RM_BLOCK + threadIdx.x;
     in += 2 * (size_t)blockIdx.y * ray_stride; out += 2 * (size_t)blockIdx.y * ray_stride;
     counter2 += 2 * blockIdx.y; n_valid += (size_t)(1 + n_chunks) * blockIdx.y;
@@ -498,18 +499,45 @@
         for (uint32_t c = 0; c < n_chunks; ++c)
             n_valid[1 + c] = min(chunk_rows, total - min(total, c * chunk_rows));
     }
-    if (i >= n_rays) return;
-    const uint32_t n = (uint32_t)in[2 * i], base = (uint32_t)in[2 * i + 1];
-    out[2 * i] = (int32_t)min(max_compacted - min(max_compacted, base), n);
-    out[2 * i + 1] = (int32_t)base;
+    uint32_t n = 0, base = 0, nc = 0;
+    if (i < n_rays) {
+        n = (uint32_t)in[2 * i]; base = (uint32_t)in[2 * i + 1];
+        nc = min(max_compacted - min(max_compacted, base), n);
+        out[2 * i] = (int32_t)nc;
+        out[2 * i + 1] = (int32_t)base;
+    }
+    if (!hits) return;
+    const uint32_t lane = threadIdx.x & 63u, wave = threadIdx.x >> 6;
+    const unsigned long long b = __ballot(nc > 0u);
+    if (lane == 0) s_wave_hits[wave] = (uint32_t)__popcll(b);
+    __syncthreads();
+    if (threadIdx.x == 0) {
+        uint32_t tot = 0;
+        for (uint32_t w = 0; w < RM_BLOCK / 64; ++w) tot += s_wave_hits[w];
+        s_hit_base = tot ? atomicAdd(hit_count + blockIdx.y, tot) : 0u;
+    }
+    __syncthreads();
+    if (nc > 0u) {
+        uint32_t o = s_hit_base + (uint32_t)__popcll(b & ((1ull << lane) - 1ull));
+        for (uint32_t w = 0; w < wave; ++w) o += s_wave_hits[w];
+        hits[(size_t)blockIdx.y * ray_stride + o] = make_uint4(i, nc, base, n);
+    }
+}
+int xr_internal_clip_numsteps_hits(const int32_t* numsteps_in, const uint32_t* counter2, uint32_t n_rays, uint32_t n_series, uint32_t ray_stride,
+                                   uint32_t max_compacted, int32_t* numsteps_out, uint32_t* n_valid_dev, uint32_t* hits, uint32_t* hit_count,
+                                   void* stream_) {
+    XR_REQUIRE(numsteps_in && counter2 && numsteps_out && n_valid_dev && n_rays > 0 && n_series >= 1 && n_series <= 65535u && ray_stride >= n_rays, "bad argument");
+    XR_REQUIRE(!hits == !hit_count && (((uintptr_t)hits) & 15) == 0, "a hit list comes with its count and is 16-byte aligned");
+    if (hits) XR_HIP(hipMemsetAsync(hit_count, 0, (size_t)n_series * sizeof(uint32_t), (hipStream_t)stream_));
+    hipLaunchKernelGGL(k2_clip, dim3(xr_div_up(n_rays, RM_BLOCK), n_series), dim3(RM_BLOCK), 0, (hipStream_t)stream_, n_rays, max_compacted,
+                       numsteps_in, counter2, numsteps_out, n_valid_dev, max_compacted, 1u, ray_stride, reinterpret_cast<uint4*>(hits), hit_count);
+    XR_LAUNCH_CHECK();
+    return XR_OK;
 }
 extern "C" int xr_clip_numsteps(const int32_t* numsteps_in, const uint32_t* counter2, uint32_t n_rays, uint32_t n_series, uint32_t ray_stride,
                                        uint32_t max_compacted, int32_t* numsteps_out, uint32_t* n_valid_dev, void* stream_) {
-    XR_REQUIRE(numsteps_in && counter2 && numsteps_out && n_valid_dev && n_rays > 0 && n_series >= 1 && n_series <= 65535u && ray_stride >= n_rays, "bad argument");
-    hipLaunchKernelGGL(k2_clip, dim3(xr_div_up(n_rays, RM_BLOCK), n_series), dim3(RM_BLOCK), 0, (hipStream_t)stream_, n_rays, max_compacted,
-                       numsteps_in, counter2, numsteps_out, n_valid_dev, max_compacted, 1u, ray_stride);
-    XR_LAUNCH_CHECK();
-    return XR_OK;
+    return xr_internal_clip_numsteps_hits(numsteps_in, counter2, n_rays, n_series, ray_stride, max_compacted, numsteps_out, n_valid_dev, nullptr, nullptr,
+                                          stream_);
 }
 
 #define CG 16
@@ -925,6 +953,107 @@
 #define CW_RAYS 4
 #define CW_RC 2
 #define CW_SEGS 8
+struct CwArgs {
+    const float4* __restrict__ raw; const float* __restrict__ coords; const float* __restrict__ bg; const float* __restrict__ target;
+    float* __restrict__ rgb_out; float4* __restrict__ dout;
+    int rgb_act, density_act; float delta, scale, loss_scale, l1, l2;
+};
+__device__ __forceinline__ void cw_load(const CwArgs& A, uint32_t n, uint32_t base, uint32_t lane, float4 (&oc)[CW_RC], float (&dc)[CW_RC]) {
+    const uint32_t chunk = (n + 63) / 64;
+    const uint32_t k0 = min(n, lane * chunk), k1 = min(n, (lane + 1) * chunk), m = k1 - k0;
+    if (chunk <= CW_RC) {
+#pragma unroll
+        for (uint32_t u = 0; u < CW_RC; ++u)
+            if (u < m) { oc[u] = A.raw[base + k0 + u]; dc[u] = A.coords[7 * (size_t)(base + k0 + u) + 3]; }
+    }
+}
+__device__ __forceinline__ void cw_ray(const CwArgs& A, uint32_t i, uint32_t n, uint32_t base, uint32_t n_full, uint32_t lane,
+                                       const float4 (&oc)[CW_RC], const float (&dc)[CW_RC], uint32_t& seg_lo, uint32_t& live_lo, uint32_t& live_hi) {
+    const float4* __restrict__ raw = A.raw; const float* __restrict__ coords = A.coords; float4* __restrict__ dout = A.dout;
+    const int rgb_act = A.rgb_act, density_act = A.density_act;
+    const float delta = A.delta, scale = A.scale, loss_scale = A.loss_scale, l1 = A.l1, l2 = A.l2;
+    const uint32_t chunk = (n + 63) / 64;
+    const uint32_t k0 = min(n, lane * chunk), k1 = min(n, (lane + 1) * chunk), m = k1 - k0;
+    const float br = A.bg[3 * i], bgc = A.bg[3 * i + 1], bb = A.bg[3 * i + 2];
+    const float tr = A.target[3 * i], tg = A.target[3 * i + 1], tb = A.target[3 * i + 2];
+    float T = 1.f, cr = 0.f, cg = 0.f, cb = 0.f;
+    auto pass1 = [&](const float4 o, float dtw, uint32_t) {
+        const float dt = xr_unwarp_dt(dtw);
+        const float alpha = 1.f - __expf(-xr_act_density(o.w, density_act) * dt);
+        const float w = alpha * T;
+        cr += w * xr_act_rgb(o.x, rgb_act); cg += w * xr_act_rgb(o.y, rgb_act); cb += w * xr_act_rgb(o.z, rgb_act);
+        T *= (1.f - alpha);
+    };
+    if (chunk <= CW_RC) {
+#pragma unroll
+        for (uint32_t u = 0; u < CW_RC; ++u) if (u < m) pass1(oc[u], dc[u], 0u);
+    } else {
+        cg_long(raw, coords, base, k0, k1, pass1);
+    }
+    float Tb1, ar1, ag1, ab1, Tg, Cgr, Cgg, Cgb;
+    cg_stitch(lane & 15, T, cr, cg, cb, &Tb1, &ar1, &ag1, &ab1, &Tg, &Cgr, &Cgg, &Cgb);
+    float GT = 1.f, Gr = 0.f, Gg = 0.f, Gb = 0.f, Tb = 1.f, ar = 0.f, ag = 0.f, ab = 0.f;
+#pragma unroll
+    for (int h = 0; h < 4; ++h) {
+        const float th = __shfl(Tg, 16 * h, 64), rh = __shfl(Cgr, 16 * h, 64), gh = __shfl(Cgg, 16 * h, 64), bh = __shfl(Cgb, 16 * h, 64);
+        if ((int)(lane >> 4) == h) { Tb = GT * Tb1; ar = Gr + GT * ar1; ag = Gg + GT * ag1; ab = Gb + GT * ab1; }
+        Gr += GT * rh; Gg += GT * gh; Gb += GT * bh;
+        GT *= th;
+    }
+    const float Tt = GT;
+    float fr = Gr, fg = Gg, fb = Gb;
+    if (n == n_full) { fr += Tt * br; fg += Tt * bgc; fb += Tt * bb; }
+    if (lane == 0) { A.rgb_out[3 * i] = fr; A.rgb_out[3 * i + 1] = fg; A.rgb_out[3 * i + 2] = fb; }
+    float g3[3];
+    {
+        const float d3[3] = {fr - tr, fg - tg, fb - tb};
+#pragma unroll
+        for (int c = 0; c < 3; ++c) g3[c] = fabsf(d3[c]) > delta ? scale * (d3[c] > 0.f ? 1.f : -1.f) : scale * (d3[c] / delta);
+    }
+    const float gr = g3[0], gg = g3[1], gb = g3[2];
+    live_lo = 0; live_hi = 0;
+    seg_lo = (base + k0) / XR_LIVE_SEG;
+    if (k0 < k1) {
+        T = Tb; cr = ar; cg = ag; cb = ab;
+        const uint32_t seg0 = seg_lo;
+        uint32_t lo = 0, hi = 0;
+        auto pass2 = [&](const float4 o, float dtw, uint32_t k) {
+            const float r = xr_act_rgb(o.x, rgb_act), g = xr_act_rgb(o.y, rgb_act), b = xr_act_rgb(o.z, rgb_act);
+            const float dt = xr_unwarp_dt(dtw);
+            const float density = xr_act_density(o.w, density_act);
+            const float alpha = 1.f - __expf(-density * dt);
+            const float w = alpha * T;
+            cr += w * r; cg += w * g; cb += w * b;
+            T *= (1.f - alpha);
+            const float ur = fr - cr, ug = fg - cg, ub = fb - cb;
+            float4 d;
+            d.x = loss_scale * ((w * gr) * xr_dact_rgb(o.x, rgb_act) + fmaxf(0.0f, l2 * o.x));
+            d.y = loss_scale * ((w * gg) * xr_dact_rgb(o.y, rgb_act) + fmaxf(0.0f, l2 * o.y));
+            d.z = loss_scale * ((w * gb) * xr_dact_rgb(o.z, rgb_act) + fmaxf(0.0f, l2 * o.z));
+            const float dot = gr * (T * r - ur) + gg * (T * g - ug) + gb * (T * b - ub);
+            d.w = loss_scale * (xr_dact_density(o.w, density_act) * (dt * dot)) + (o.w < 0.f ? -l1 : 0.0f);
+            dout[base + k] = d;
+            if (d.x != 0.f || d.y != 0.f || d.z != 0.f || d.w != 0.f) {
+                if ((base + k) / XR_LIVE_SEG == seg0) ++lo; else ++hi;
+            }
+        };
+        if (chunk <= CW_RC) {
+#pragma unroll
+            for (uint32_t u = 0; u < CW_RC; ++u) if (u < m) pass2(oc[u], dc[u], k0 + u);
+        } else {
+            cg_long(raw, coords, base, k0, k1, pass2);
+        }
+        live_lo = lo; live_hi = hi;
+    }
+}
+__device__ __forceinline__ CwArgs cw_args(uint32_t n_rays, const float4* raw, const float* coords, const float* bg, const float* target,
+                                          const float* density_grid_mean, int rgb_act, int density_act, float delta, float scale, float* rgb_out,
+                                          float4* dout) {
+    float loss_scale = 128.f; loss_scale /= (float)n_rays;
+    const float l2 = rgb_act == XR_ACT_EXPONENTIAL ? 1e-4f : 0.0f;
+    const float l1 = density_grid_mean[0] < 0.01f ? 1e-4f : 0.0f;
+    return CwArgs{raw, coords, bg, target, rgb_out, dout, rgb_act, density_act, delta, scale, loss_scale, l1, l2};
+}
 __global__ __launch_bounds__(64 * CW_RAYS) void k_composite_train_w(
     uint32_t n_rays, const float4* __restrict__ raw, const float* __restrict__ coords, const int32_t* __restrict__ numsteps,
     const int32_t* __restrict__ numsteps_c, const float* __restrict__ bg, const float* __restrict__ target,
@@ -938,92 +1067,18 @@
         if (threadIdx.x == 0) seg_first = (uint32_t)numsteps_c[2 * i + 1] / XR_LIVE_SEG;
         __syncthreads();
     }
-    float loss_scale = 128.f; loss_scale /= (float)n_rays;
-    const float l2 = rgb_act == XR_ACT_EXPONENTIAL ? 1e-4f : 0.0f;
-    const float l1 = density_grid_mean[0] < 0.01f ? 1e-4f : 0.0f;
+    const CwArgs A = cw_args(n_rays, raw, coords, bg, target, density_grid_mean, rgb_act, density_act, delta, scale, rgb_out, dout);
     uint32_t n = 0, base = 0, n_full = 0;
     if (in) { n = (uint32_t)numsteps_c[2 * i]; base = (uint32_t)numsteps_c[2 * i + 1]; n_full = (uint32_t)numsteps[2 * i]; }
     if (n > 0) {
-        const uint32_t chunk = (n + 63) / 64;
-        const uint32_t k0 = min(n, lane * chunk), k1 = min(n, (lane + 1) * chunk), m = k1 - k0;
         float4 oc[CW_RC]; float dc[CW_RC];
-        if (chunk <= CW_RC) {
-#pragma unroll
-            for (uint32_t u = 0; u < CW_RC; ++u)
-                if (u < m) { oc[u] = raw[base + k0 + u]; dc[u] = coords[7 * (size_t)(base + k0 + u) + 3]; }
-        }
-        const float br = bg[3 * i], bgc = bg[3 * i + 1], bb = bg[3 * i + 2];
-        const float tr = target[3 * i], tg = target[3 * i + 1], tb = target[3 * i + 2];
-        float T = 1.f, cr = 0.f, cg = 0.f, cb = 0.f;
-        auto pass1 = [&](const float4 o, float dtw, uint32_t) {
-            const float dt = xr_unwarp_dt(dtw);
-            const float alpha = 1.f - __expf(-xr_act_density(o.w, density_act) * dt);
-            const float w = alpha * T;
-            cr += w * xr_act_rgb(o.x, rgb_act); cg += w * xr_act_rgb(o.y, rgb_act); cb += w * xr_act_rgb(o.z, rgb_act);
-            T *= (1.f - alpha);
-        };
-        if (chunk <= CW_RC) {
-#pragma unroll
-            for (uint32_t u = 0; u < CW_RC; ++u) if (u < m) pass1(oc[u], dc[u], 0u);
-        } else {
-            cg_long(raw, coords, base, k0, k1, pass1);
-        }
-        float Tb1, ar1, ag1, ab1, Tg, Cgr, Cgg, Cgb;
-        cg_stitch(lane & 15, T, cr, cg, cb, &Tb1, &ar1, &ag1, &ab1, &Tg, &Cgr, &Cgg, &Cgb);
-        float GT = 1.f, Gr = 0.f, Gg = 0.f, Gb = 0.f, Tb = 1.f, ar = 0.f, ag = 0.f, ab = 0.f;
-#pragma unroll
-        for (int h = 0; h < 4; ++h) {
-            const float th = __shfl(Tg, 16 * h, 64), rh = __shfl(Cgr, 16 * h, 64), gh = __shfl(Cgg, 16 * h, 64), bh = __shfl(Cgb, 16 * h, 64);
-            if ((int)(lane >> 4) == h) { Tb = GT * Tb1; ar = Gr + GT * ar1; ag = Gg + GT * ag1; ab = Gb + GT * ab1; }
-            Gr += GT * rh; Gg += GT * gh; Gb += GT * bh;
-            GT *= th;
-        }
-        const float Tt = GT;
-        float fr = Gr, fg = Gg, fb = Gb;
-        if (n == n_full) { fr += Tt * br; fg += Tt * bgc; fb += Tt * bb; }
-        if (lane == 0) { rgb_out[3 * i] = fr; rgb_out[3 * i + 1] = fg; rgb_out[3 * i + 2] = fb; }
-        float g3[3];
-        {
-            const float d3[3] = {fr - tr, fg - tg, fb - tb};
-#pragma unroll
-            for (int c = 0; c < 3; ++c) g3[c] = fabsf(d3[c]) > delta ? scale * (d3[c] > 0.f ? 1.f : -1.f) : scale * (d3[c] / delta);
-        }
-        const float gr = g3[0], gg = g3[1], gb = g3[2];
-        if (k0 < k1) {
-            T = Tb; cr = ar; cg = ag; cb = ab;
-            uint32_t live_lo = 0, live_hi = 0;
-            const uint32_t seg_lo = (base + k0) / XR_LIVE_SEG;
-            auto pass2 = [&](const float4 o, float dtw, uint32_t k) {
-                const float r = xr_act_rgb(o.x, rgb_act), g = xr_act_rgb(o.y, rgb_act), b = xr_act_rgb(o.z, rgb_act);
-                const float dt = xr_unwarp_dt(dtw);
-                const float density = xr_act_density(o.w, density_act);
-                const float alpha = 1.f - __expf(-density * dt);
-                const float w = alpha * T;
-                cr += w * r; cg += w * g; cb += w * b;
-                T *= (1.f - alpha);
-                const float ur = fr - cr, ug = fg - cg, ub = fb - cb;
-                float4 d;
-                d.x = loss_scale * ((w * gr) * xr_dact_rgb(o.x, rgb_act) + fmaxf(0.0f, l2 * o.x));
-                d.y = loss_scale * ((w * gg) * xr_dact_rgb(o.y, rgb_act) + fmaxf(0.0f, l2 * o.y));
-                d.z = loss_scale * ((w * gb) * xr_dact_rgb(o.z, rgb_act) + fmaxf(0.0f, l2 * o.z));
-                const float dot = gr * (T * r - ur) + gg * (T * g - ug) + gb * (T * b - ub);
-                d.w = loss_scale * (xr_dact_density(o.w, density_act) * (dt * dot)) + (o.w < 0.f ? -l1 : 0.0f);
-                dout[base + k] = d;
-                if (d.x != 0.f || d.y != 0.f || d.z != 0.f || d.w != 0.f) {
-                    if ((base + k) / XR_LIVE_SEG == seg_lo) ++live_lo; else ++live_hi;
-                }
-            };
-            if (chunk <= CW_RC) {
-#pragma unroll
-                for (uint32_t u = 0; u < CW_RC; ++u) if (u < m) pass2(oc[u], dc[u], k0 + u);
-            } else {
-                cg_long(raw, coords, base, k0, k1, pass2);
-            }
-            if (live_seg_count) {
-                const uint32_t rel = seg_lo - seg_first;
-                if (live_lo) { if (rel < CW_SEGS) atomicAdd(&seg_hist[rel], live_lo); else atomicAdd(&live_seg_count[seg_lo], live_lo); }
-                if (live_hi) { if (rel + 1 < CW_SEGS) atomicAdd(&seg_hist[rel + 1], live_hi); else atomicAdd(&live_seg_count[seg_lo + 1], live_hi); }
-            }
+        cw_load(A, n, base, lane, oc, dc);
+        uint32_t seg_lo, live_lo, live_hi;
+        cw_ray(A, i, n, base, n_full, lane, oc, dc, seg_lo, live_lo, live_hi);
+        if (live_seg_count) {
+            const uint32_t rel = seg_lo - seg_first;
+            if (live_lo) { if (rel < CW_SEGS) atomicAdd(&seg_hist[rel], live_lo); else atomicAdd(&live_seg_count[seg_lo], live_lo); }
+            if (live_hi) { if (rel + 1 < CW_SEGS) atomicAdd(&seg_hist[rel + 1], live_hi); else atomicAdd(&live_seg_count[seg_lo + 1], live_hi); }
         }
     } else if (in && lane == 0) {
         rgb_out[3 * i] = bg[3 * i]; rgb_out[3 * i + 1] = bg[3 * i + 1]; rgb_out[3 * i + 2] = bg[3 * i + 2];
@@ -1031,6 +1086,77 @@
     if (!live_seg_count) return;
     __syncthreads();
     if (threadIdx.x < CW_SEGS && seg_hist[threadIdx.x]) atomicAdd(&live_seg_count[seg_first + threadIdx.x], seg_hist[threadIdx.x]);
+}
+
+#ifndef CWL_WGS
+#define CWL_WGS 1024u
+#endif
+#define CWL_BG_RAYS (64u * CW_RAYS)
+__global__ __launch_bounds__(64 * CW_RAYS) void k_composite_train_wl(
+    uint32_t n_rays, uint32_t n_list_wgs, const uint4* __restrict__ hits, const uint32_t* __restrict__ hit_count, const float4* __restrict__ raw,
+    const float* __restrict__ coords, const int32_t* __restrict__ numsteps_c, const float* __restrict__ bg, const float* __restrict__ target,
+    const float* __restrict__ density_grid_mean, int rgb_act, int density_act, float delta, float scale,
+    float* __restrict__ rgb_out, float4* __restrict__ dout, uint32_t* __restrict__ live_seg_count) {
+    if (blockIdx.x >= n_list_wgs) {
+        const uint32_t i = (blockIdx.x - n_list_wgs) * CWL_BG_RAYS + threadIdx.x;
+        if (i < n_rays && numsteps_c[2 * i] <= 0) { rgb_out[3 * i] = bg[3 * i]; rgb_out[3 * i + 1] = bg[3 * i + 1]; rgb_out[3 * i + 2] = bg[3 * i + 2]; }
+        return;
+    }
+    const uint32_t lane = threadIdx.x & 63, stride = n_list_wgs * CW_RAYS;
+    const uint32_t count = min(*hit_count, n_rays);
+    const CwArgs A = cw_args(n_rays, raw, coords, bg, target, density_grid_mean, rgb_act, density_act, delta, scale, rgb_out, dout);
+    uint32_t k = blockIdx.x * CW_RAYS + (threadIdx.x >> 6);
+    if (k >= count) return;
+    uint4 e = hits[k], en = k + stride < count ? hits[k + stride] : make_uint4(0u, 0u, 0u, 0u);
+    float4 oc[CW_RC]; float dc[CW_RC];
+    cw_load(A, e.y, e.z, lane, oc, dc);
+    for (;;) {
+        const uint32_t kn = k + stride;
+        const bool more = kn < count;
+        const uint4 enn = kn + stride < count ? hits[kn + stride] : make_uint4(0u, 0u, 0u, 0u);
+        float4 ocn[CW_RC]; float dcn[CW_RC];
+        if (more) cw_load(A, en.y, en.z, lane, ocn, dcn);
+        if (e.x < n_rays && e.y > 0u) {
+            uint32_t seg_lo, live_lo, live_hi;
+            cw_ray(A, e.x, e.y, e.z, e.w, lane, oc, dc, seg_lo, live_lo, live_hi);
+            if (live_seg_count) {
+                const uint32_t s0 = e.z / XR_LIVE_SEG, s1 = (e.z + e.y - 1u) / XR_LIVE_SEG;
+                for (uint32_t sg = s0; sg <= s1; ++sg) {
+                    uint32_t v = (seg_lo == sg ? live_lo : 0u) + (seg_lo + 1u == sg ? live_hi : 0u);
+#pragma unroll
+                    for (int d = 32; d > 0; d >>= 1) v += (uint32_t)__shfl_xor((int)v, d, 64);
+                    if (lane == 0 && v) atomicAdd(&live_seg_count[sg], v);
+                }
+            }
+        }
+        if (!more) break;
+        k = kn; e = en; en = enn;
+#pragma unroll
+        for (uint32_t u = 0; u < CW_RC; ++u) { oc[u] = ocn[u]; dc[u] = dcn[u]; }
+    }
+}
+static thread_local const uint32_t* g_ct_hits = nullptr;
+static thread_local const uint32_t* g_ct_hit_count = nullptr;
+void xr_internal_composite_hit_list(const uint32_t* hits, const uint32_t* hit_count) { g_ct_hits = hits; g_ct_hit_count = hit_count; }
+#ifndef XR_CT_LIST
+#define XR_CT_LIST 1
+#endif
+extern "C" int xr_composite_train_hits(const float* network_output, const float* coords, const int32_t* rays_numsteps_compacted,
+                                        const uint32_t* hit_list, const uint32_t* hit_count, const float* bg_color, const float* target,
+                                        const float* density_grid_mean, uint32_t n_rays, int rgb_activation, int density_activation,
+                                        float delta, float scale, float* rgb_output, float* dloss_doutput, uint32_t* live_seg_count,
+                                        void* stream_) {
+    XR_REQUIRE(network_output && coords && rays_numsteps_compacted && hit_list && hit_count && bg_color && target && density_grid_mean &&
+               rgb_output && dloss_doutput, "null pointer");
+    XR_REQUIRE((((uintptr_t)network_output | (uintptr_t)dloss_doutput | (uintptr_t)hit_list) & 15) == 0, "raw / grad buffers and the hit list must be 16-byte aligned");
+    XR_REQUIRE(n_rays > 0, "n_rays == 0");
+    const uint32_t all_wgs = xr_div_up(n_rays, CW_RAYS), list_wgs = all_wgs < (uint32_t)CWL_WGS ? all_wgs : (uint32_t)CWL_WGS;
+    hipLaunchKernelGGL(k_composite_train_wl, dim3(list_wgs + xr_div_up(n_rays, CWL_BG_RAYS)), dim3(64 * CW_RAYS), 0, (hipStream_t)stream_, n_rays,
+                       list_wgs, reinterpret_cast<const uint4*>(hit_list), hit_count, (const float4*)network_output, coords,
+                       rays_numsteps_compacted, bg_color, target, density_grid_mean, rgb_activation, density_activation, delta, scale,
+                       rgb_output, (float4*)dloss_doutput, live_seg_count);
+    XR_LAUNCH_CHECK();
+    return XR_OK;
 }
 
 #define LS_THREADS XR_AUX_LS_VTHREADS
@@ -1064,6 +1190,9 @@
 #ifndef XR_CT_STAGE
 #define XR_CT_STAGE 1
 #endif
+    if (!loss_mse_out && XR_CT_WAVE && XR_CT_LIST && g_ct_hits && g_ct_hit_count)
+        return xr_composite_train_hits(network_output, coords, rays_numsteps_compacted, g_ct_hits, g_ct_hit_count, bg_color, target, density_grid_mean,
+                                       n_rays, rgb_activation, density_activation, delta, scale, rgb_output, dloss_doutput, live_seg_count, stream_);
     if (!loss_mse_out && XR_CT_WAVE) {
         hipLaunchKernelGGL(k_composite_train_w, dim3(xr_div_up(n_rays, CW_RAYS)), dim3(64 * CW_RAYS), 0, (hipStream_t)stream_, n_rays,
                            (const float4*)network_output, coords, rays_numsteps, rays_numsteps_compacted, bg_color, target,
diff --git a/xrnerf_amd/csrc/xr_step.hip b/xrnerf_amd/csrc/xr_step.hip
--- a/xrnerf_amd/csrc/xr_step.hip
+++ b/xrnerf_amd/csrc/xr_step.hip
@@ -185,8 +185,10 @@
                                 W->xyz_planes ? W->xyz_planes + 3 * (size_t)first_chunk * W->plane_stride : nullptr, W->plane_stride, workspace,
                                 workspace_bytes, stream_);
     if (rc != XR_OK) return rc;
-    rc = xr_clip_numsteps(W->rays_numsteps + 2 * r0, W->counter2 + 2 * first_chunk, n_rays, n_chunks, W->ray_stride, max_compacted,
-                                 W->numsteps_clipped + 2 * r0, W->n_valid + 2 * first_chunk, stream_);
+    XR_REQUIRE(!W->hit_list == !W->hit_count, "a window's hit lists come with their counts");
+    rc = xr_internal_clip_numsteps_hits(W->rays_numsteps + 2 * r0, W->counter2 + 2 * first_chunk, n_rays, n_chunks, W->ray_stride, max_compacted,
+                                        W->numsteps_clipped + 2 * r0, W->n_valid + 2 * first_chunk, W->hit_list ? W->hit_list + 4 * r0 : nullptr,
+                                        W->hit_count ? W->hit_count + first_chunk : nullptr, stream_);
     if (rc != XR_OK) return rc;
     if (counter_host_pinned)
         XR_HIP(hipMemcpyAsync(counter_host_pinned + 2 * first_chunk, W->counter2 + 2 * first_chunk, (size_t)n_chunks * 2 * sizeof(uint32_t),
@@ -226,6 +228,7 @@
         at.ema_momentum = ad.ema_momentum = ac.ema_momentum = ema_momentum[j];
         const float* coords = W.coords + 7 * c * W.coords_stride;
         const size_t table_floats = 2 * (size_t)D.offset_host[D.n_levels];
+        if (W.hit_list && W.hit_count) xr_internal_composite_hit_list(W.hit_list + 4 * r0, W.hit_count + c);
         rc = xr_ngp_train_step(D.table, D.w_density, D.w_color, D.n_hidden_density, D.n_hidden_color, D.pad_value, D.mlp_mode, D.n_levels, D.scale_host,
                                D.resolution_host, D.offset_host, coords, D.n_rows, W.n_valid + 2 * c, W.rays_numsteps + 2 * r0,
                                W.numsteps_clipped + 2 * r0, n_rays, W.bg + 3 * r0, W.target + 3 * r0, W.alpha + r0, D.density_grid_mean, D.rgb_activation,
@@ -235,6 +238,7 @@
                                W.xyz_planes ? W.xyz_planes + 3 * c * W.plane_stride : nullptr, W.plane_stride, X ? nullptr : &at, X ? nullptr : &ad,
                                X ? nullptr : &ac, timed_entry, timed_entry ? timing_events[2 * j] : nullptr,
                                timed_entry ? timing_events[2 * j + 1] : nullptr, D.stream);
+        xr_internal_composite_hit_list(nullptr, nullptr);
         if (rc != XR_OK) return rc;
         if (X) {
             XR_REQUIRE(B.grad_w_color == B.grad_w_density + D.adam_w_density.n, "the two MLP gradients form one bucket");
diff --git a/xrnerf_amd/ops.py b/xrnerf_amd/ops.py
--- a/xrnerf_amd/ops.py
+++ b/xrnerf_amd/ops.py
@@ -305,11 +305,19 @@
 
 
 def composite_train(raw, coords, numsteps, numsteps_c, bg, target, alpha, density_grid_mean, rgb_act, density_act, loss_mse, draw,
-                    delta=0.1, scale=5.0, rgb=None, live_seg=None):
+                    delta=0.1, scale=5.0, rgb=None, live_seg=None, hits=None):
     n = numsteps.shape[0]
     if rgb is None:
         rgb = torch.empty((n, 3), dtype=torch.float32, device=raw.device)
     p_seg = _ptr(live_seg)
+    if hits is not None:
+        if loss_mse is not None:
+            raise _lib.XrError('the launch over a hit list is the wave-per-ray form: no loss accumulator')
+        with _span('xr_composite_train', 0):
+            _lib.check(_lib.load().xr_composite_train_hits(_ptr(raw), _ptr(coords), _ptr(numsteps_c), _ptr(hits[0]), _ptr(hits[1]), _ptr(bg),
+                                                           _ptr(target), _ptr(density_grid_mean), n, int(rgb_act), int(density_act), float(delta),
+                                                           float(scale), _ptr(rgb), _ptr(draw), p_seg, _stream()), 'xr_composite_train_hits')
+        return rgb
     with _span('xr_composite_train', 0):
         _lib.check(_lib.load().xr_composite_train(_ptr(raw), _ptr(coords), _ptr(numsteps), _ptr(numsteps_c), _ptr(bg), _ptr(target),
                                                    _ptr(alpha), _ptr(density_grid_mean), n, int(rgb_act), int(density_act),
@@ -333,6 +341,7 @@
         self.coords = f(W, coords_stride, 7)
         self.xyz = f(W, 3, coords_stride) if planes else None
         self.counter2, self.n_valid = i(W, 2), i(W, 2)
+        self.hit_list, self.hit_count = i(W, ray_stride, 4), i(W)
         self.pinned = torch.zeros((W, 2), dtype=torch.int32).pin_memory() if device.type == 'cuda' else None
         c = _lib.Window()
         vp = lambda t: t.data_ptr() if t is not None else None
@@ -341,6 +350,7 @@
         c.ray_stride, c.coords, c.coords_stride = self.ray_stride, vp(self.coords), self.coords_stride
         c.xyz_planes, c.plane_stride = vp(self.xyz), (self.coords_stride if planes else 0)
         c.counter2, c.n_valid = vp(self.counter2), vp(self.n_valid)
+        c.hit_list, c.hit_count = vp(self.hit_list), vp(self.hit_count)
         self.c = c
 
     def batch(self, c, n):
```

New measurement: 36.93 million. No clear change (-0.1%).
